# YangHai-1218/RADet

Hardware: AMD Instinct MI355X
Metric: images/sec train-step, r50_ycbv_pbr 640x480 bs=4/GPU (higher is better)
Workload: dtype f32

## Files before the change

include/radet_hip.h:

```cpp
#ifndef RADET_HIP_H
#define RADET_HIP_H
#include <stdint.h>

#ifdef __cplusplus
extern "C" {
#endif


typedef struct RadetConvDesc {
    const float* w;
    const float* bias;
    const float* bn_gamma;
    const float* bn_beta;
    const float* bn_mean;
    const float* bn_var;
    float* wf;
    float* wft;
    float* bias_f;
    const float* dwf_slabs;
    const float* dbias_partials;
    float* dw;
    float* dbias;
    float* dgamma;
    float* dbeta;
// ... 8 lines not shown
    float* w_l1;
    float* bias_amax;
    float* w_l1t;
} RadetConvDesc;

#define RADET_AMAX_WORDS 64
typedef struct RadetScales {
    const void* x_amax;
    const void* w_amax;
    void* y_amax;
    const void* x1_amax;
    const void* w1_amax;
    void* y1_amax;
    void* yq;
    void* yq_amax;
    const void* x_true_amax;
    const void* w_l1;
    const void* bias_amax;
    const void* addend_amax;
} RadetScales;

int radet_gather_table_rows(int M);
int radet_build_gather_table(int* table, int B, int KH, int KW, int so, int sr, int off, int div, const int* seg_desc,
                             int nseg, void* stream);
enum {
    RADET_TILE_ID_MASK = 0xFF,
    RADET_TILE_SYMBOL = 0x100,
    RADET_TILE_BK32 = 0x200,
    RADET_TILE_MATH_BF16 = 0x400,
    RADET_TILE_STORE_BF16 = 0x800,
    RADET_TILE_SPLITK = 0x1000,
    RADET_TILE_SPLITK_MASK = 0xF000,
    RADET_TILE_OUT_F32 = 0x10000,
    RADET_TILE_STAGES3 = 0x20000,
    RADET_TILE_STAGES4 = 0x40000,
    RADET_TILE_ROWPAIRS = 0x80000,
    RADET_TILE_STREAMK = 0x100000,
    RADET_TILE_STREAMK_MASK = 0x700000,
    RADET_TILE_X3 = 0x1000000,
    RADET_TILE_P3 = 0x2000000,
    RADET_TILE_H2 = 0x8000000,
    RADET_TILE_MASKQ = 0x10000000
};
int radet_conv2d_igemm(const float* x, const float* w, const float* bias, const float* addend, const float* mask,
                       float* y, const int* gather_table, int M, int Cin, int Cout, int KH, int KW, int relu,
                       int tile_override, float* splitk_ws, size_t splitk_ws_floats, void* stream);
int radet_conv2d_igemm_s(const float* x, const float* w, const float* bias, const float* addend, const float* mask,
                         float* y, const int* gather_table, int M, int Cin, int Cout, int KH, int KW, int relu,
                         int tile_override, float* splitk_ws, size_t splitk_ws_floats, void* stream, const RadetScales* sc);
int radet_conv2d_igemm_pair_s(const float* x0, const float* w0, const float* bias0, const float* addend0,
                              const float* mask0, float* y0, const float* x1, const float* w1, const float* bias1,
                              const float* addend1, const float* mask1, float* y1, const int* gather_table, int M,
                              int Cin, int Cout, int KH, int KW, int relu, int tile_override, float* splitk_ws,
                              size_t splitk_ws_floats, void* stream, const RadetScales* sc);
int radet_conv2d_igemm_taps_s(const float* x, const float* w, const float* addend, const float* mask, float* y,
                              const int* gather_table, const int* out_rows, const int* tap_ids_host, int ntaps, int kt_w,
                              int M, int Cin, int Cout, int tile_override, float* splitk_ws, size_t splitk_ws_floats,
                              void* stream, const RadetScales* sc);
int radet_conv2d_igemm_classes_s(const float* x, const float* w, const float* addend, const float* mask, float* y,
                                 const int* gather_table, const int* out_rows, const int* tap_ids_host,
                                 const int* cls_ntaps, const int* cls_start, int ncls, int kt_w, int M, int Cin, int Cout,
                                 int tile_override, float* splitk_ws, size_t splitk_ws_floats, void* stream,
                                 const RadetScales* sc);
int radet_conv2d_igemm_pair(const float* x0, const float* w0, const float* bias0, const float* addend0,
                            const float* mask0, float* y0, const float* x1, const float* w1, const float* bias1,
                            const float* addend1, const float* mask1, float* y1, const int* gather_table, int M, int Cin,
                            int Cout, int KH, int KW, int relu, int tile_override, float* splitk_ws,
                            size_t splitk_ws_floats, void* stream);
int radet_conv2d_igemm_taps(const float* x, const float* w, const float* addend, const float* mask, float* y,
                            const int* gather_table, const int* out_rows, const int* tap_ids_host, int ntaps, int kt_w,
                            int M, int Cin, int Cout, int tile_override, float* splitk_ws, size_t splitk_ws_floats,
                            void* stream);
int radet_conv2d_igemm_classes(const float* x, const float* w, const float* addend, const float* mask, float* y,
                               const int* gather_table, const int* out_rows, const int* tap_ids_host, const int* cls_ntaps,
                               const int* cls_start, int ncls, int kt_w, int M, int Cin, int Cout, int tile_override,
                               float* splitk_ws, size_t splitk_ws_floats, void* stream);
int radet_pred3x3_patch(const float* x, int Cin, const int* tiles_dev, int ntiles, const float* w0, const float* bias0,
                        float* y0, int c0, const float* w1, const float* bias1, float* y1, int c1, void* stream);
enum {
    RADET_WGRAD_MATH_BF16 = 0x1,
    RADET_WGRAD_STORE_BF16 = 0x2,
    RADET_WGRAD_TILE = 0x10,
    RADET_WGRAD_TILE_MASK = 0x30,
    RADET_WGRAD_ONE_TAP = 0x40,
    RADET_WGRAD_PX32 = 0x80,
    RADET_WGRAD_X3 = 0x100,
    RADET_WGRAD_P3 = 0x200,
    RADET_WGRAD_KDIV4 = 0x400,
    RADET_WGRAD_KDIV2 = 0x800,
    RADET_WGRAD_H2 = 0x1000,
    RADET_WGRAD_DEEP = 0x2000,
    RADET_WGRAD_WINDOWS = 0x4000
};
int radet_conv2d_wgrad_splits(int M, int Cin, int Cout, int KH, int KW);
int radet_conv2d_wgrad(const float* dy, const float* x, float* slabs, float* dbias_partials, const int* gather_table,
                       int M, int Cin, int Cout, int ld_dy, int KH, int KW, int S, int flags, void* stream);
int radet_conv2d_wgrad_s(const float* dy, const float* x, float* slabs, float* dbias_partials, const int* gather_table,
                         int M, int Cin, int Cout, int ld_dy, int KH, int KW, int S, int flags, void* stream,
                         const RadetScales* sc);
typedef struct RadetWgradJob {
    const float* dy;
    const float* x;
    float* slabs;
    float* dbias_partials;
    const int* gather_table;
    int M, Cin, Cout, ld_dy, KH, KW, S;
// ... 302 lines not shown
```

radet_amd/_lib.py:

```python
import ctypes as C
import os

_HERE = os.path.dirname(os.path.abspath(__file__))
LIB_PATH = os.path.join(_HERE, os.environ.get("RADET_LIB", "libradet_hip.so"))

_p = C.c_void_p
_i = C.c_int
_f = C.c_float
_sz = C.c_size_t


class RadetConvDesc(C.Structure):
    _fields_ = [("w", _p), ("bias", _p), ("bn_gamma", _p), ("bn_beta", _p), ("bn_mean", _p), ("bn_var", _p),
                ("wf", _p), ("wft", _p), ("bias_f", _p), ("dwf_slabs", _p), ("dbias_partials", _p),
                ("dw", _p), ("dbias", _p), ("dgamma", _p), ("dbeta", _p),
                ("cout", _i), ("cin", _i), ("kh", _i), ("kw", _i), ("nsplit", _i), ("eps", _f),
                ("wft_ld", _i), ("wft_off", _i), ("w16", _i), ("w_amax", _p), ("wfq", _p), ("w_l1", _p), ("bias_amax", _p),
                ("w_l1t", _p)]


class RadetScales(C.Structure):
    _fields_ = [("x_amax", _p), ("w_amax", _p), ("y_amax", _p), ("x1_amax", _p), ("w1_amax", _p), ("y1_amax", _p),
                ("yq", _p), ("yq_amax", _p), ("x_true_amax", _p), ("w_l1", _p), ("bias_amax", _p), ("addend_amax", _p)]


class RadetWgradJob(C.Structure):
    _fields_ = [("dy", _p), ("x", _p), ("slabs", _p), ("dbias_partials", _p), ("gather_table", _p),
                ("M", _i), ("Cin", _i), ("Cout", _i), ("ld_dy", _i), ("KH", _i), ("KW", _i), ("S", _i)]


class RadetTapeOp(C.Structure):
    _fields_ = [("kind", C.c_int32), ("fn", C.c_int32), ("stream", _p), ("event", _p), ("args", C.c_uint64 * 32)]


SIGNATURES = {
    "radet_gather_table_rows": (_i, [_i]),
    "radet_build_gather_table": (_i, [_p, _i, _i, _i, _i, _i, _i, _i, _p, _i, _p]),
    "radet_conv2d_igemm": (_i, [_p, _p, _p, _p, _p, _p, _p, _i, _i, _i, _i, _i, _i, _i, _p, _sz, _p]),
    "radet_conv2d_igemm_pair": (_i, [_p] * 13 + [_i, _i, _i, _i, _i, _i, _i, _p, _sz, _p]),
    "radet_conv2d_igemm_taps": (_i, [_p, _p, _p, _p, _p, _p, _p, _p, _i, _i, _i, _i, _i, _i, _p, _sz, _p]),
    "radet_conv2d_igemm_classes": (_i, [_p, _p, _p, _p, _p, _p, _p, _p, _p, _p, _i, _i, _i, _i, _i, _i, _p, _sz, _p]),
    "radet_conv2d_igemm_s": (_i, [_p, _p, _p, _p, _p, _p, _p, _i, _i, _i, _i, _i, _i, _i, _p, _sz, _p, _p]),
    "radet_conv2d_igemm_pair_s": (_i, [_p] * 13 + [_i, _i, _i, _i, _i, _i, _i, _p, _sz, _p, _p]),
    "radet_conv2d_igemm_taps_s": (_i, [_p, _p, _p, _p, _p, _p, _p, _p, _i, _i, _i, _i, _i, _i, _p, _sz, _p, _p]),
    "radet_conv2d_igemm_classes_s": (_i, [_p, _p, _p, _p, _p, _p, _p, _p, _p, _p, _i, _i, _i, _i, _i, _i, _p, _sz, _p, _p]),
    "radet_conv2d_wgrad_s": (_i, [_p, _p, _p, _p, _p, _i, _i, _i, _i, _i, _i, _i, _i, _p, _p]),
    "radet_split_pairs": (_i, [_p, _p, _sz, _i, _i, _p, _p, _p]),
    "radet_merge_pairs": (_i, [_p, _p, _sz, _i, _i, _p, _p]),
    "radet_gn_relu_fwd_q": (_i, [_p, _p, _p, _p, _p, _p, _p, _i, _i, _i, _f, _i, _p, _i, _p, _p, _p, _p]),
    "radet_gn_relu_fwd_pair_q": (_i, [_p] * 20 + [_i, _i, _i, _f, _i, _p, _i, _p]),
    "radet_gn_relu_bwd_q": (_i, [_p, _p, _p, _p, _p, _p, _p, _p, _p, _p, _i, _i, _i, _i, _p, _i, _p, _p, _p, _p]),
    "radet_maxpool3x3s2_a": (_i, [_p, _p, _i, _i, _i, _i, _p, _p]),
    "radet_maxpool3x3s2_q": (_i, [_p, _p, _i, _i, _i, _i, _p, _p, _p, _p, _p]),
    "radet_stem_conv_bn_relu_a": (_i, [_p, _p, _p, _p, _i, _i, _i, _p, _p]),
    "radet_upsample_add_a": (_i, [_p, _p, _i, _i, _i, _i, _i, _i, _p, _p]),
    "radet_upsample_add_bwd_a": (_i, [_p, _p, _i, _i, _i, _i, _i, _i, _p, _p]),
    "radet_relu_bwd_a": (_i, [_p, _p, _p, _p, _sz, _p, _p]),
    "radet_absmax": (_i, [_p, _sz, _p, _p]),
    "radet_amax_slot_words": (_i, []),
    "radet_pred3x3_patch": (_i, [_p, _i, _p, _i, _p, _p, _p, _i, _p, _p, _p, _i, _p]),
    "radet_conv2d_wgrad_splits": (_i, [_i, _i, _i, _i, _i]),
    "radet_conv2d_wgrad": (_i, [_p, _p, _p, _p, _p, _i, _i, _i, _i, _i, _i, _i, _i, _p]),
    "radet_conv2d_wgrad_group": (_i, [_p, _i, _i, _p]),
    "radet_fold_weights": (_i, [_p, _i, _p]),
    "radet_unfold_grads": (_i, [_p, _i, _i, _p]),
    "radet_stem_conv_bn_relu": (_i, [_p, _p, _p, _p, _i, _i, _i, _p]),
    "radet_maxpool3x3s2": (_i, [_p, _p, _i, _i, _i, _i, _p]),
    "radet_maxpool3x3s2_bwd_relu": (_i, [_p, _p, _p, _i, _i, _i, _i, _p]),
    "radet_stem_wgrad_splits": (_i, [_i, _i, _i]),
    "radet_stem_wgrad": (_i, [_p, _p, _p, _p, _i, _i, _i, _i, _p]),
    "radet_gn_workspace_floats": (_i, [_i, _p, _i]),
    "radet_gn_relu_fwd": (_i, [_p, _p, _p, _p, _p, _p, _i, _i, _i, _f, _i, _p, _i, _p]),
    "radet_gn_relu_fwd_pair": (_i, [_p] * 12 + [_i, _i, _i, _f, _i, _p, _i, _p]),
    "radet_gn_relu_fwd_pair_h": (_i, [_p] * 12 + [_i, _i, _i, _f, _i, _p, _i, _p]),
    "radet_gn_relu_bwd": (_i, [_p, _p, _p, _p, _p, _p, _p, _p, _p, _i, _i, _i, _i, _p, _i, _p]),
    "radet_upsample_add": (_i, [_p, _p, _i, _i, _i, _i, _i, _i, _p]),
    "radet_upsample_add_bwd": (_i, [_p, _p, _i, _i, _i, _i, _i, _i, _p]),
    "radet_relu_bwd": (_i, [_p, _p, _p, _p, _sz, _p]),
    "radet_nchw_to_nhwc": (_i, [_p, _p, _i, _i, _i, _i, _p]),
    "radet_nhwc_to_nchw": (_i, [_p, _p, _i, _i, _i, _i, _p]),
    "radet_head_loss_ws_ints": (_i, [_i]),
    "radet_head_loss": (_i, [_p, _p, _p, _p, _p, _p, _p, _p, _p, _p, _i, _i, _i, _f, _f, _f, _f, _p, _p, _p, _i, _p,
                             _i, _p, _i, _p, _p, _p, _i, _p, _p]),
    "radet_scale_relu": (_i, [_p, _p, _p, _p, _i, _i, _p]),
    "radet_decode_ws_bytes": (_sz, [_i, _i, _i]),
    "radet_decode_candidates": (_i, [_p, _p, _p, _p, _p, _i, _i, _i, _f, _i, _p, _p, _p, _p, _p, _p, _p, _p, _p]),
    "radet_nms_ws_bytes": (_sz, [_i, _i]),
    "radet_nms": (_i, [_p, _p, _p, _p, _p, _i, _i, _i, _f, _i, _f, _i, _p, _p, _p, _p, _p, _p, _p, _p]),
    "radet_assign_ws_bytes": (_sz, [_i, _i]),
    "radet_assign_points": (_i, [_p, _p, _p, _i, _i, _p, _i, _p, _p, _i, _i, _i, _i, _f, _p, _p, _p, _p, _p]),
    "radet_assign_points_f": (_i, [_p, _p, _p, _i, _i, _p, _i, _p, _p, _i, _i, _i, _i, _f, _p, _p, _p, _p, _p]),
    "radet_resize_linear_u8": (_i, [_p, _p, _p, _p, _p, _i, _i, _i, _p]),
    "radet_resize_linear_f": (_i, [_p, _p, _p, _p, _i, _i, _i, _p]),
    "radet_warp_affine_u8": (_i, [_p, _sz, _p, _sz, _p, _i, _i, _i, _p]),
    "radet_cutout_u8": (_i, [_p, _sz, _p, _i, _p, _i, _i, _i, _i, _p]),
    "radet_cutout_f32": (_i, [_p, _i, _i, _i, _p, _i, _p, _i, _i, _i, _f, _f, _f, _f, _f, _f, _p]),
# ... 112 lines not shown
```

radet_amd/csrc/conv_common.h:

```cpp
#pragma once
#include "common.h"
#include "../../include/radet_hip.h"
#include <stdlib.h>
#include <type_traits>

#define RADET_SPLIT_COUNTERS 16384
#ifndef RADET_P3_DBG
#define RADET_P3_DBG 0
#endif

struct ConvPtrs {
    const float* x;
    const float* w;
    const float* bias;
    const float* addend;
    const float* mask;
    float* y;
    const unsigned* xs;
    const unsigned* ws;
    unsigned* ys;
    _Float16* yq;
    unsigned* yqs;
    const unsigned* xt;
    const unsigned* wl1;
    const unsigned* bs;
    const unsigned* as;
};

struct ConvArgs {
    ConvPtrs p[2];
    int groups;
    const int* rowtab;
    float* partial;
    int* counters;
    const int* out_rows;
    int tap_ids[16];
    int KTw;
    int M, Mp, Cin, Cout, KH, KW;
    int relu;
    int sk, it_per_split;
    int n_full, sk_tail, it_per_tail;
    int io;
    int sk_wgs, sk_base, sk_rem;
    int cls_nt, cls_b[3];
    int dbg;
    int maskq;
};

__device__ __forceinline__ float ld_act(const float* p, size_t o, int io) {
    return io ? (float)reinterpret_cast<const __bf16*>(p)[o] : p[o];
}
__device__ __forceinline__ void st_out(float* p, size_t o, float v, int io) {
    if (io == 1) reinterpret_cast<__bf16*>(p)[o] = (__bf16)v;
    else p[o] = v;
}


typedef const __attribute__((address_space(1))) void* gptr_t;
typedef __attribute__((address_space(3))) void* lptr_t;

#ifndef RADET_BUFLDS
#define RADET_BUFLDS 1
#endif
__device__ __forceinline__ __amdgpu_buffer_rsrc_t radet_rsrc(const void* base) {
    return __builtin_amdgcn_make_buffer_rsrc(const_cast<void*>(base), 0, 0xFFFFFF00u, 0x00020000);
}
#if RADET_BUFLDS
#define radet_lds_load16(base, ok, elem_off, dst) \
    __builtin_amdgcn_raw_ptr_buffer_load_lds(radet_rsrc(base), (dst), 16, \
        (int)((ok) ? (unsigned)((elem_off) * sizeof(*(base))) : 0xFFFFFFFFu), 0, 0, 0)
#else
#define radet_lds_load16(base, ok, elem_off, dst) \
    __builtin_amdgcn_global_load_lds((gptr_t)((ok) ? (const void*)((base) + (elem_off)) : (const void*)(radet_zero_page + (threadIdx.x & 63) * 4)), \
                                     (dst), 16, 0, 0)
#endif

__device__ __forceinline__ void radet_pipe_barrier() {
    asm volatile("s_waitcnt lgkmcnt(0)" ::: "memory");
    __builtin_amdgcn_s_barrier();
    asm volatile("" ::: "memory");
}

__device__ __forceinline__ int find_seg(const RadetSegs& s, int m) {
    int l = 0;
#pragma unroll
    for (int i = 0; i < RADET_MAX_SEG - 1; ++i)
        if (i < s.nseg - 1 && m >= s.s[i].row_end) l = i + 1;
    return l;
}

struct PixCtx {
    int by, bx;
    int Hi, Wi;
    int base;
};

__device__ __forceinline__ PixCtx decode_pixel(const RadetSegs& segs, int m, int M, int so, int off) {
    PixCtx p;
    p.Hi = 0; p.Wi = 0; p.by = 0; p.bx = 0; p.base = 0;
    if (m < M) {
        const int l = find_seg(segs, m);
        const RadetSeg& sg = segs.s[l];
        const int local = m - sg.row_begin;
        const int hw = sg.Ho * sg.Wo;
        const int n = local / hw;
        const int rem = local - n * hw;
        const int oy = rem / sg.Wo;
        const int ox = rem - oy * sg.Wo;
        p.by = oy * so + off;
        p.bx = ox * so + off;
        p.Hi = sg.Hi;
        p.Wi = sg.Wi;
        p.base = sg.in_row_off + n * sg.Hi * sg.Wi;
    }
    return p;
}

__device__ __forceinline__ int gather_row(const PixCtx& p, int r, int q, int sr, int div) {
    int iy = p.by + r * sr, ix = p.bx + q * sr;
    if (div > 1) {
        if ((iy % div) != 0 || (ix % div) != 0) return -1;
        iy /= div;
        ix /= div;
    }
    if (iy < 0 || iy >= p.Hi || ix < 0 || ix >= p.Wi) return -1;
    return p.base + iy * p.Wi + ix;
}

template <int IO>
__device__ __forceinline__ float ld_act_t(const float* p, size_t o) {
    if constexpr (IO != 0) return (float)reinterpret_cast<const __bf16*>(p)[o];
    else return p[o];
}
template <int IO>
__device__ __forceinline__ void st_out_t(float* p, size_t o, float v) {
    if constexpr (IO == 1) reinterpret_cast<__bf16*>(p)[o] = (__bf16)v;
    else p[o] = v;
}

struct EpiArgs {
    float qs, qs2;
    int M, Cout, relu, io;
    int maskq;
    const int* out_rows;
    float* partial;
    int* counters;
    int sk_base, sk_rem;
};
template <class T>
__device__ __forceinline__ T pin_sgpr(T v) {
    asm volatile("" : "+s"(v));
    return v;
}

template <int BM, int BN, int WM, int WN, int IO>
__device__ __forceinline__ void igemm_epilogue(const EpiArgs& a, const ConvPtrs& P,
                                               f32x16 (&acc)[BM / (WM * 32)][BN / (WN * 32)], int m0, int n0, int wm, int wn,
                                               int li, int lh) {
    constexpr int TM = BM / (WM * 32), TN = BN / (WN * 32);
    const bool has_add = P.addend != nullptr, has_mask = P.mask != nullptr, has_rows = a.out_rows != nullptr;
    const bool interior = !has_rows && m0 + BM <= a.M && n0 + BN <= a.Cout;
    float amax = 0.f;
#pragma unroll
    for (int i = 0; i < TM; ++i) {
        size_t obase[16];
        bool rvalid[16];
        if (has_rows) {
            int orow[16];
#pragma unroll
            for (int r = 0; r < 16; ++r) {
                const int row = m0 + (wm * TM + i) * 32 + (r & 3) + 8 * (r >> 2) + 4 * lh;
                orow[r] = a.out_rows[row < a.M ? row : 0];
                rvalid[r] = row < a.M && orow[r] >= 0;
                if (orow[r] < 0) orow[r] = 0;
            }
#pragma unroll
            for (int r = 0; r < 16; ++r) obase[r] = (size_t)orow[r] * a.Cout;
        } else {
#pragma unroll
            for (int r = 0; r < 16; ++r) {
                const int row = m0 + (wm * TM + i) * 32 + (r & 3) + 8 * (r >> 2) + 4 * lh;
                rvalid[r] = row < a.M;
                obase[r] = (size_t)(rvalid[r] ? row : 0) * a.Cout;
            }
        }
#pragma unroll
        for (int j = 0; j < TN; ++j) {
            const int col = n0 + (wn * TN + j) * 32 + li;
            const bool cvalid = col < a.Cout;
            const int cc = cvalid ? col : 0;
            const float bv = P.bias ? P.bias[cc] : 0.f;
            float av[16], mv[16];
            if (has_add) {
#pragma unroll
                for (int r = 0; r < 16; ++r) av[r] = ld_act_t<IO>(P.addend, obase[r] + cc);
            }
            if (has_mask) {
                if (IO == 0 && a.maskq) {
                    const unsigned short* mq = reinterpret_cast<const unsigned short*>(P.mask) + radet_pair_off(cc);
                    unsigned short mh[16], ml[16];
#pragma unroll
                    for (int r = 0; r < 16; ++r) { mh[r] = mq[2 * obase[r]]; ml[r] = mq[2 * obase[r] + 32]; }
#pragma unroll
                    for (int r = 0; r < 16; ++r) {
                        const unsigned sel = (mh[r] & 0x7FFFu) ? mh[r] : ml[r];
                        mv[r] = ((sel & 0x7FFFu) != 0u && (sel & 0x8000u) == 0u) ? 1.f : 0.f;
                    }
                } else {
#pragma unroll
                    for (int r = 0; r < 16; ++r) mv[r] = ld_act_t<IO>(P.mask, obase[r] + cc);
                }
            }
            float out[16];
#pragma unroll
            for (int r = 0; r < 16; ++r) {
                float v = acc[i][j][r] + bv;
                if (has_add) v += av[r];
                if (a.relu) v = fmaxf(v, 0.f);
                if (has_mask) v = mv[r] > 0.f ? v : 0.f;
                out[r] = v;
            }
            if constexpr (IO == 0) {
                if (P.yq) {
                    const bool odd = li & 1;
                    unsigned* const q = reinterpret_cast<unsigned*>(reinterpret_cast<unsigned short*>(P.yq) +
                                                                    radet_pair_off(cc & ~1) + (odd ? 32 : 0));
#pragma unroll
                    for (int r = 0; r < 16; r += 2) {
                        unsigned h, l;
                        radet_split2(out[r], out[r + 1], a.qs, a.qs2, h, l);
                        const unsigned send = odd ? h : l;
                        const unsigned recv = (unsigned)__builtin_amdgcn_mov_dpp((int)send, 0xB1, 0xF, 0xF, true);
                        const unsigned lo_ch = odd ? recv : h, hi_ch = odd ? l : recv;
                        const unsigned w0 = __builtin_amdgcn_perm(hi_ch, lo_ch, 0x05040100u);
                        const unsigned w1 = __builtin_amdgcn_perm(hi_ch, lo_ch, 0x07060302u);
                        if (interior || (cvalid && rvalid[r])) q[obase[r]] = w0;
                        if (interior || (cvalid && rvalid[r + 1])) q[obase[r + 1]] = w1;
                    }
                }
            }
            const bool has_y = P.y != nullptr;
            if (interior) {
                if (has_y) {
#pragma unroll
// ... 43 lines not shown
#pragma unroll
    for (int i = 0; i < TM; ++i)
#pragma unroll
        for (int j = 0; j < TN; ++j) {
            const float4* src = reinterpret_cast<const float4*>(pz + (((wave * TM + i) * TN + j) * 64 + lane) * 16);
#pragma unroll
            for (int q = 0; q < 4; ++q) {
                const float4 v = src[q];
                acc[i][j][4 * q] += v.x; acc[i][j][4 * q + 1] += v.y; acc[i][j][4 * q + 2] += v.z; acc[i][j][4 * q + 3] += v.w;
            }
        }
}

template <class A>
__device__ __forceinline__ int streamk_start(const A& a, int v) { return v * a.sk_base + (v < a.sk_rem ? v : a.sk_rem); }
template <class A>
__device__ __forceinline__ int streamk_owner(const A& a, int it) {
    const int big = (a.sk_base + 1) * a.sk_rem;
    return it < big ? it / (a.sk_base + 1) : a.sk_rem + (it - big) / a.sk_base;
}

template <int BM, int BN, int WM, int WN>
__device__ __forceinline__ bool streamk_publish(const EpiArgs& a, f32x16 (&acc)[BM / (WM * 32)][BN / (WN * 32)],
                                                int tile, int nseg, int nKs, int v, int slot, volatile int* ws) {
    constexpr int TM = BM / (WM * 32), TN = BN / (WN * 32);
    partial_write<BM, BN, WM, WN>(a.partial + (size_t)(2 * v + slot) * BM * BN, acc);
    asm volatile("s_waitcnt vmcnt(0)" ::: "memory");
    __syncthreads();
    if (threadIdx.x == 0)
        ws[0] = __hip_atomic_fetch_add(&a.counters[tile], nseg, __ATOMIC_RELAXED, __HIP_MEMORY_SCOPE_AGENT);
    __syncthreads();
    const bool last = ws[0] + nseg == nKs;
    __syncthreads();
    if (!last) return false;
    __builtin_amdgcn_fence(__ATOMIC_ACQUIRE, "agent");
    if (threadIdx.x == 0)
        __hip_atomic_store(&a.counters[tile], 0, __ATOMIC_RELAXED, __HIP_MEMORY_SCOPE_AGENT);
    __syncthreads();
#pragma unroll
    for (int i = 0; i < TM; ++i)
#pragma unroll
        for (int j = 0; j < TN; ++j)
#pragma unroll
            for (int r = 0; r < 16; ++r) acc[i][j][r] = 0.f;
    const int t0 = tile * nKs;
    const int v0 = streamk_owner(a, t0), v1 = streamk_owner(a, t0 + nKs - 1);
    for (int u = v0; u <= v1; ++u) {
        const int sl = streamk_start(a, u) >= t0 ? 0 : 1;
        partial_add<BM, BN, WM, WN>(a.partial + (size_t)(2 * u + sl) * BM * BN, acc);
    }
    return true;
}

template <int BM, int BN, int WM, int WN>
__device__ __forceinline__ void igemm_store(const EpiArgs& e, const ConvPtrs& P,
                                            f32x16 (&acc)[BM / (WM * 32)][BN / (WN * 32)], int m0, int n0, int nsplit,
                                            int ctile, int z, int wm, int wn, int li, int lh, volatile int* ws) {
    constexpr int TM = BM / (WM * 32), TN = BN / (WN * 32);
    if (nsplit > 1) {
        float* base = e.partial + (size_t)ctile * nsplit * BM * BN;
        partial_write<BM, BN, WM, WN>(base + (size_t)z * BM * BN, acc);
        asm volatile("s_waitcnt vmcnt(0)" ::: "memory");
        __syncthreads();
        if (threadIdx.x == 0)
            ws[0] = __hip_atomic_fetch_add(&e.counters[ctile], 1, __ATOMIC_RELAXED, __HIP_MEMORY_SCOPE_AGENT);
        __syncthreads();
        if (ws[0] != nsplit - 1) return;
        __builtin_amdgcn_fence(__ATOMIC_ACQUIRE, "agent");
        if (threadIdx.x == 0)
            __hip_atomic_store(&e.counters[ctile], 0, __ATOMIC_RELAXED, __HIP_MEMORY_SCOPE_AGENT);
        __syncthreads();
#pragma unroll
        for (int i = 0; i < TM; ++i)
#pragma unroll
            for (int j = 0; j < TN; ++j)
#pragma unroll
                for (int r = 0; r < 16; ++r) acc[i][j][r] = 0.f;
        for (int zz = 0; zz < nsplit; ++zz) partial_add<BM, BN, WM, WN>(base + (size_t)zz * BM * BN, acc);
    }
    if (e.io == 0) igemm_epilogue<BM, BN, WM, WN, 0>(e, P, acc, m0, n0, wm, wn, li, lh);
    else if (e.io == 1) igemm_epilogue<BM, BN, WM, WN, 1>(e, P, acc, m0, n0, wm, wn, li, lh);
    else igemm_epilogue<BM, BN, WM, WN, 2>(e, P, acc, m0, n0, wm, wn, li, lh);
}

typedef float f32x4 __attribute__((ext_vector_type(4)));
template <int OFF>
__device__ __forceinline__ void lds_read128(f32x4& d, unsigned addr) {
    asm volatile("ds_read_b128 %0, %1 offset:%2" : "=v"(d) : "v"(addr), "n"(OFF) : "memory");
}
typedef short s16x4 __attribute__((ext_vector_type(4)));
typedef unsigned u32x2 __attribute__((ext_vector_type(2)));
typedef float f32x2 __attribute__((ext_vector_type(2)));
typedef __bf16 bf16x2 __attribute__((ext_vector_type(2)));
typedef __bf16 bf16x8 __attribute__((ext_vector_type(8)));
__device__ __forceinline__ unsigned cvt_pk_bf16(float lo, float hi) {
    const f32x2 v = {lo, hi};
    return __builtin_bit_cast(unsigned, __builtin_convertvector(v, bf16x2));
}
__device__ __forceinline__ s16x4 cvt_bf16x4(float a, float b, float c, float d) {
    const u32x2 r = {cvt_pk_bf16(a, b), cvt_pk_bf16(c, d)};
    return __builtin_bit_cast(s16x4, r);
}

template <int OFF>
__device__ __forceinline__ void lds_read32(float& d, unsigned addr) {
    asm volatile("ds_read_b32 %0, %1 offset:%2" : "=v"(d) : "v"(addr), "n"(OFF) : "memory");
}
template <int OFF>
__device__ __forceinline__ void lds_read_u16(unsigned& d, unsigned addr) {
    asm volatile("ds_read_u16 %0, %1 offset:%2" : "=v"(d) : "v"(addr), "n"(OFF) : "memory");
}
template <int OFF>
__device__ __forceinline__ void lds_read_i16(int& d, unsigned addr) {
    asm volatile("ds_read_i16 %0, %1 offset:%2" : "=v"(d) : "v"(addr), "n"(OFF) : "memory");
}
template <int N>
__device__ __forceinline__ void vm_wait() {
    asm volatile("s_waitcnt vmcnt(%0)" ::"n"(N) : "memory");
}
template <int I, int N, class F>
__device__ __forceinline__ void static_for(F&& f) {
    if constexpr (I < N) {
        f(std::integral_constant<int, I>{});
        static_for<I + 1, N>(f);
    }
}
typedef short s16x4v_ __attribute__((ext_vector_type(4)));
template <int OFF>
__device__ __forceinline__ void lds_read_tr16(s16x4v_& d, unsigned addr) {
    asm volatile("ds_read_b64_tr_b16 %0, %1 offset:%2" : "=v"(d) : "v"(addr), "n"(OFF) : "memory");
}
template <int N>
__device__ __forceinline__ void lds_wait() {
// ... 4 lines not shown
__device__ __forceinline__ void split3_bf16(const float (&a)[8], bf16x8& hi, bf16x8& mid, bf16x8& lo) {
    typedef float f32x2_ __attribute__((ext_vector_type(2)));
    u32x4_ h, m, l;
#pragma unroll
    for (int q = 0; q < 4; ++q) {
        const f32x2_ a2 = {a[2 * q], a[2 * q + 1]};
        const unsigned ua0 = __float_as_uint(a2.x), ua1 = __float_as_uint(a2.y);
        const f32x2_ h2 = {__uint_as_float(ua0 & 0xFFFF0000u), __uint_as_float(ua1 & 0xFFFF0000u)};
        const f32x2_ r2 = a2 - h2;
        const unsigned ur0 = __float_as_uint(r2.x), ur1 = __float_as_uint(r2.y);
        const f32x2_ m2 = {__uint_as_float(ur0 & 0xFFFF0000u), __uint_as_float(ur1 & 0xFFFF0000u)};
        const f32x2_ l2 = r2 - m2;
        h[q] = __builtin_amdgcn_perm(ua1, ua0, 0x07060302u);
        m[q] = __builtin_amdgcn_perm(ur1, ur0, 0x07060302u);
        l[q] = __builtin_amdgcn_perm(__float_as_uint(l2.y), __float_as_uint(l2.x), 0x07060302u);
    }
    hi = __builtin_bit_cast(bf16x8, h);
    mid = __builtin_bit_cast(bf16x8, m);
    lo = __builtin_bit_cast(bf16x8, l);
}
__device__ __forceinline__ void split3_bf16(const f32x4& f0, const f32x4& f1, bf16x8& hi, bf16x8& mid, bf16x8& lo) {
    const float a[8] = {f0.x, f0.y, f0.z, f0.w, f1.x, f1.y, f1.z, f1.w};
    split3_bf16(a, hi, mid, lo);
}
__device__ __forceinline__ void mfma_x3(f32x16& acc, const bf16x8& ah, const bf16x8& am, const bf16x8& al,
                                        const bf16x8& bh, const bf16x8& bm, const bf16x8& bl) {
    acc = __builtin_amdgcn_mfma_f32_32x32x16_bf16(ah, bh, acc, 0, 0, 0);
    acc = __builtin_amdgcn_mfma_f32_32x32x16_bf16(am, bh, acc, 0, 0, 0);
    acc = __builtin_amdgcn_mfma_f32_32x32x16_bf16(ah, bm, acc, 0, 0, 0);
    acc = __builtin_amdgcn_mfma_f32_32x32x16_bf16(am, bm, acc, 0, 0, 0);
    acc = __builtin_amdgcn_mfma_f32_32x32x16_bf16(al, bh, acc, 0, 0, 0);
    acc = __builtin_amdgcn_mfma_f32_32x32x16_bf16(ah, bl, acc, 0, 0, 0);
}


typedef _Float16 f16x8 __attribute__((ext_vector_type(8)));
struct H2Scale {
    float s, s2, inv;
};
__device__ __forceinline__ H2Scale h2_scale_bits(unsigned amax_bits) {
    const int e = radet_h2_exp(amax_bits);
    H2Scale r;
    r.s = radet_pow2(e); r.s2 = radet_pow2(e + 11); r.inv = radet_pow2(-e);
    return r;
}
__device__ __forceinline__ H2Scale h2_scale(const unsigned* slot) {
    return h2_scale_bits(radet_amax_read(slot));
}
__device__ __forceinline__ unsigned h2_scale_load(const unsigned* slot) { return radet_amax_load(slot); }
__device__ __forceinline__ H2Scale h2_scale_finish(unsigned raw) {
    asm volatile("" : "+v"(raw));
    return h2_scale_bits(radet_amax_reduce(raw));
}
__device__ __forceinline__ void split2_f16(const float (&a)[8], const H2Scale& sc, f16x8& hi, f16x8& lo) {
    u32x4_ h, l;
#pragma unroll
    for (int q = 0; q < 4; ++q) {
        unsigned hq, lq;
        radet_split2(a[2 * q], a[2 * q + 1], sc.s, sc.s2, hq, lq);
        h[q] = hq; l[q] = lq;
    }
    hi = __builtin_bit_cast(f16x8, h);
    lo = __builtin_bit_cast(f16x8, l);
}
__device__ __forceinline__ void split2_f16(const f32x4& f0, const f32x4& f1, const H2Scale& sc, f16x8& hi, f16x8& lo) {
    const float a[8] = {f0.x, f0.y, f0.z, f0.w, f1.x, f1.y, f1.z, f1.w};
    split2_f16(a, sc, hi, lo);
}
__device__ __forceinline__ void mfma_h2(f32x16& acc0, f32x16& acc1, const f16x8& ah, const f16x8& al, const f16x8& bh,
                                        const f16x8& bl) {
    acc0 = __builtin_amdgcn_mfma_f32_32x32x16_f16(ah, bh, acc0, 0, 0, 0);
    acc1 = __builtin_amdgcn_mfma_f32_32x32x16_f16(ah, bl, acc1, 0, 0, 0);
    acc1 = __builtin_amdgcn_mfma_f32_32x32x16_f16(al, bh, acc1, 0, 0, 0);
}
struct PairScaleRaw { unsigned xt, wl1, bs, as; };
__device__ __forceinline__ PairScaleRaw igemm_pair_scale_load(const ConvPtrs& P) {
    PairScaleRaw r;
    r.xt = radet_amax_load(P.xt); r.wl1 = radet_amax_load(P.wl1);
    r.bs = P.bs ? radet_amax_load(P.bs) : 0u;
    r.as = P.as ? radet_amax_load(P.as) : 0u;
    return r;
}
__device__ __forceinline__ void igemm_pair_scale(const ConvPtrs& P, PairScaleRaw r, bool store, float& qs, float& qs2) {
    asm volatile("" : "+v"(r.xt), "+v"(r.wl1), "+v"(r.bs), "+v"(r.as));
    float bound = __uint_as_float(radet_amax_reduce(r.xt)) * __uint_as_float(radet_amax_reduce(r.wl1));
    bound += __uint_as_float(radet_amax_reduce(r.bs));
    bound += __uint_as_float(radet_amax_reduce(r.as));
    bound *= 1.0001f;
    const unsigned bits = __float_as_uint(bound);
    if (store && threadIdx.x == 0) radet_amax_store(P.yqs, bits);
    const int e = radet_h2_exp(bits);
    qs = radet_pow2(e);
    qs2 = radet_pow2(e + 11);
}

__device__ __forceinline__ void h2_combine(f32x16& acc0, const f32x16& acc1, float inv_a, float inv_b) {
#pragma unroll
    for (int r = 0; r < 16; ++r) acc0[r] = (fmaf(acc1[r], 1.0f / 2048.0f, acc0[r]) * inv_a) * inv_b;
}

struct TileWord {
    int id;
    int splitk;
    int stages;
    int streamk;
    bool symbol, bk32, math_bf16, store_bf16, out_f32, rowpairs, x3, p3, h2, maskq;
// ... 31 lines not shown
```

radet_amd/csrc/conv_igemm.hip:

```cpp
#include "common.h"
#include "../../include/radet_hip.h"
#include <stdlib.h>
#include <type_traits>

#include "conv_common.h"

#include "conv_igemm_kernel.h"
#include "conv_wgrad_kernel.h"

struct PredTile { int base_row, H, W, yx; };
struct PredArgs {
    const float* x;
    const float* w[2];
    const float* bias[2];
    float* y[2];
    int c[2];
    const PredTile* tiles;
    int Cin;
};

__global__ __launch_bounds__(512) void pred3x3_patch_kernel(const PredArgs a) {
    constexpr int TH = 8, TW = 16, PW = TW + 2, PP = (TH + 2) * PW;
    constexpr int PROWS = 192, WROWS = 9 * 32;
    constexpr int A_BYTES = PROWS * 64, BUF_BYTES = (PROWS + WROWS) * 64;
// ... 888 lines not shown
                      const RadetScales* sc) {
    const TileWord tw = decode_tile(tile_override);
    const bool h16 = tw.store_bf16;
    const bool p3 = tw.p3 && !h16;
    if (h16 || p3) {
        if (Cin % 32 != 0) return RADET_ERR_ARG;
        Cin /= 2;
    }
    if (Cin % 16 != 0 || Cin <= 0 || Cout <= 0 || M <= 0 || KH * KW > 16 ||
        (gather_table == nullptr && (KH * KW != 1 || out_rows != nullptr || cls != nullptr)))
        return RADET_ERR_ARG;
    ConvArgs a;
    a.io = h16 ? (tw.out_f32 ? 2 : 1) : 0;
    a.out_rows = out_rows;
    for (int t = 0; t < 16; ++t) a.tap_ids[t] = tap_ids ? (t < KH * KW ? tap_ids[t] : 0) : t;
    a.cls_nt = 0; a.cls_b[0] = a.cls_b[1] = a.cls_b[2] = 0x7fffffff;
    if (cls != nullptr) {
        for (int t = 0; t < 16; ++t) a.tap_ids[t] = tap_ids[t];
        for (int c = 0; c < cls[0]; ++c) {
            a.cls_nt |= cls[1 + c] << (4 * c);
            if (c > 0) a.cls_b[c - 1] = cls[5 + c];
        }
    }
    a.KTw = kt_w > 0 ? kt_w : KH * KW;
    { static const int dbg = getenv("RADET_DBG_IGEMM") ? atoi(getenv("RADET_DBG_IGEMM")) : 0; a.dbg = dbg; }
    a.maskq = tw.maskq && mask != nullptr;
    if (a.maskq && (h16 || Cout % 32 != 0 || second != nullptr)) return RADET_ERR_ARG;
    if (y == nullptr && (sc == nullptr || sc->yq == nullptr)) return RADET_ERR_ARG;
    a.p[0].x = x; a.p[0].w = w; a.p[0].bias = bias; a.p[0].addend = addend; a.p[0].mask = mask; a.p[0].y = y;
    a.p[0].xs = sc ? (const unsigned*)sc->x_amax : nullptr;
    a.p[0].ws = sc ? (const unsigned*)sc->w_amax : nullptr;
    a.p[0].ys = sc ? (unsigned*)sc->y_amax : nullptr;
    a.p[0].yq = sc ? (_Float16*)sc->yq : nullptr;
    a.p[0].yqs = sc ? (unsigned*)sc->yq_amax : nullptr;
    a.p[0].xt = sc ? (const unsigned*)sc->x_true_amax : nullptr;
    a.p[0].wl1 = sc ? (const unsigned*)sc->w_l1 : nullptr;
    a.p[0].bs = (sc && bias) ? (const unsigned*)sc->bias_amax : nullptr;
    a.p[0].as = (sc && addend) ? (const unsigned*)sc->addend_amax : nullptr;
    if (a.p[0].yq != nullptr) {
        if (h16 || Cout % 32 != 0 || a.p[0].yqs == nullptr || a.p[0].xt == nullptr || a.p[0].wl1 == nullptr ||
            (bias && a.p[0].bs == nullptr) || (addend && a.p[0].as == nullptr) || second != nullptr)
            return RADET_ERR_ARG;
    }
    a.p[1] = a.p[0];
    a.groups = 1;
    if (second != nullptr) {
        a.p[1] = *second;
        a.p[1].yq = nullptr; a.p[1].yqs = nullptr; a.p[1].xt = a.p[1].wl1 = a.p[1].bs = a.p[1].as = nullptr;
        a.p[1].xs = sc ? (const unsigned*)sc->x1_amax : nullptr;
        a.p[1].ws = sc ? (const unsigned*)sc->w1_amax : nullptr;
        a.p[1].ys = sc ? (unsigned*)sc->y1_amax : nullptr;
        a.groups = 2;
    }
    a.rowtab = gather_table;
    a.Cin = Cin; a.Cout = Cout; a.KH = KH; a.KW = KW;
    a.relu = relu;
    a.M = M;
    a.Mp = radet_gather_table_rows(M);
    hipStream_t st = (hipStream_t)stream;
    const int sym = tw.symbol ? TAG_SYMBOL : 0;
    int tag = sym | (h16 ? TAG_H16 : (tw.math_bf16 ? TAG_BF16_MATH : 0));
    int bk = tw.bk32 ? 32 : 16;
    if (Cin % 32 != 0) bk = 16;
    const bool x3 = tw.x3 && !h16 && !p3 && !tw.math_bf16 && Cin % 32 == 0;
    if (x3) { bk = 32; tag |= TAG_X3; }
    if (p3) { tag = TAG_P3 | sym; bk = 16; }
    const bool h2 = tw.h2 && (x3 || p3);
    if (h2) {
        for (int g = 0; g < a.groups; ++g)
            if (a.p[g].xs == nullptr || a.p[g].ws == nullptr) return RADET_ERR_ARG;
        tag |= TAG_H2;
    }
    int choice = tw.id;
    if (p3 && h2 && tw.rowpairs && (choice == 5 || choice == 6)) {
        Cin *= 2;
        a.Cin = Cin;
        if (Cin % 32 != 0) return RADET_ERR_ARG;
        tag |= TAG_PAIRS; bk = 32;
    }
    if (choice == 7 && p3 && h2) {
        Cin *= 2;
        a.Cin = Cin;
        if (Cin % 64 != 0 || tw.streamk || a.groups != 1) return RADET_ERR_ARG;
        tag = TAG_X3 | TAG_KDIV | TAG_H2 | TAG_PAIRS; bk = 64;
    } else
    if (choice == 7 || choice == 8) {
        const int kbk = choice == 7 ? 64 : 32;
        if (!x3 || Cin % kbk != 0 || tw.streamk) return RADET_ERR_ARG;
        tag |= TAG_KDIV; bk = kbk;
    } else
    if (choice > 4 && !p3) return RADET_ERR_ARG;
    if (choice == 6 && cls != nullptr) return RADET_ERR_ARG;
    if (choice <= 0) {
        if (Cout <= 32) choice = 4;
        else {
            const double s1 = tile_score(a.M, Cout, 128, 128, 1.00);
            const double s2 = tile_score(a.M, Cout, 128, 64, 0.96);
            const double s3 = tile_score(a.M, Cout, 64, 64, 0.90);
            choice = 1;
            double best = s1;
            if (s2 > best) { best = s2; choice = 2; }
            if (s3 > best) { best = s3; choice = 3; }
        }
    }
    const int nK = KH * KW * (Cin / bk);
    int sk = 1;
// ... 237 lines not shown
```

radet_amd/csrc/conv_igemm_kernel.h:

```cpp
#pragma once
#include "conv_common.h"
static __device__ __attribute__((aligned(16))) float radet_zero_page[512];

constexpr int TAG_SYMBOL = 1;
constexpr int TAG_BF16_MATH = 2;
constexpr int TAG_H16 = 4;
constexpr int TAG_X3 = 8;
constexpr int TAG_P3 = 16;
constexpr int TAG_KDIV = 32;
constexpr int TAG_H2 = 64;
constexpr int TAG_PAIRS = 128;
template <int BM, int BN, int WM, int WN, int TAG, int BK, int NSTG = 2, bool SK = false>
__global__ __launch_bounds__(WM * WN * 64) void conv_igemmg_kernel(const ConvArgs a) {
    constexpr int NW = WM * WN;
    constexpr int F4 = BK / 4;
    constexpr int RPI = 64 / F4;
    constexpr int RPB = 64 / BK;
    constexpr int TM = BM / (WM * 32), TN = BN / (WN * 32);
    constexpr int A_INSTR = BM / RPI, B_INSTR = BN / RPI;
    constexpr int A_PW = (A_INSTR + NW - 1) / NW, B_PW = (B_INSTR + NW - 1) / NW;
    constexpr int NS = ((TAG & TAG_PAIRS) && (TAG & TAG_P3)) ? 2 : BK / 8;
    constexpr bool BF16 = (TAG & TAG_BF16_MATH) != 0;
    constexpr bool H16 = (TAG & TAG_H16) != 0;
    constexpr bool X3 = (TAG & TAG_X3) != 0;
    constexpr bool P3 = (TAG & TAG_P3) != 0;
    constexpr bool H2 = (TAG & TAG_H2) != 0;
    static_assert(!H2 || X3 || P3, "fp16 hi / lo arithmetic: in-register split (TAG_X3) or plane pairs (TAG_P3)");
    constexpr bool RI = P3 && (TAG & TAG_PAIRS) != 0;
    static_assert(!RI || (H2 && BK == 32), "row-interleaved pairs: fp16 hi / lo planes, 128-byte tile rows");
    constexpr int NPLC = P3 ? (H2 ? 2 : 3) : 1;
    constexpr int NPL = RI ? 1 : NPLC;
    constexpr bool KW = (TAG & TAG_KDIV) != 0;
    constexpr bool PQ = (TAG & TAG_PAIRS) != 0 && (TAG & TAG_KDIV) != 0;
    static_assert(!PQ || (KW && H2 && BK == 64), "pair operands in the K-divided tile: 64-channel stages");
    constexpr int KD = KW ? BK / 16 : 1;
    constexpr int WNK = NW / KD;
    constexpr int TMA = KW ? BM / 32 : TM, TNA = KW ? BN / (32 * WNK) : TN;
    static_assert(!KW || (X3 && !SK && NW == 4 && KD * WNK == NW && TM == 1 && TN == 1 && TMA * TNA == KD && NSTG >= 2 && NSTG <= 4),
                  "K-divided tile: one 32 x 32 block per wave after the reduction");
    static_assert(NW == 4 || NW == 8, "4 or 8 waves");
    static_assert(!P3 || BK == 16 || RI, "plane rows are laid out in 32-channel groups: one group per K stage");
    __shared__ __attribute__((aligned(16))) float As[NSTG][NPL * BM * BK];
    __shared__ __attribute__((aligned(16))) float Bs[NSTG][NPL * BN * BK];

    radet_kernarg_warm<sizeof(ConvArgs)>();
    const int tid = threadIdx.x;
    const int lane = tid & 63, wave = __builtin_amdgcn_readfirstlane(tid >> 6);
    const int wm = wave / WN, wn = wave % WN;
    const int li = lane & 31, lh = lane >> 5;
    const int xld = NPL * a.Cin;

    const int tilesN = (a.Cout + BN - 1) / BN;
    const int tilesG = ((a.M + BM - 1) / BM) * tilesN;
    const int KT = a.KH * a.KW;
    const int cpt = a.Cin / BK;
    constexpr bool streamk = SK;
    const int vwg = streamk ? ((int)blockIdx.x & 7) * (a.sk_wgs >> 3) + ((int)blockIdx.x >> 3) : 0;
    int cur = streamk ? streamk_start(a, vwg) : 0;
    const int end_it = streamk ? cur + a.sk_base + (vwg < a.sk_rem ? 1 : 0) : 1;
    const int first_tile = cur / (KT * cpt);
  do {
    const bool tail = !streamk && (int)blockIdx.x >= a.n_full;
    const int tail_slot = tail ? (int)blockIdx.x - a.n_full : 0;
    int id = streamk ? cur / (KT * cpt)
                     : (tail ? a.n_full + tail_slot / a.sk_tail : (a.cls_nt ? (int)blockIdx.x : xcd_remap(blockIdx.x, a.n_full)));
    const int sk_tile = id;
    const int grp = id >= tilesG ? 1 : 0;
    id -= grp * tilesG;
    ConvPtrs P = a.p[grp];
    P.y = pin_sgpr(P.y); P.bias = pin_sgpr(P.bias); P.addend = pin_sgpr(P.addend); P.mask = pin_sgpr(P.mask);
    EpiArgs epi;
    epi.M = pin_sgpr(a.M); epi.Cout = pin_sgpr(a.Cout); epi.relu = pin_sgpr(a.relu); epi.io = pin_sgpr(a.io);
    epi.out_rows = pin_sgpr(a.out_rows); epi.maskq = pin_sgpr(a.maskq);
    epi.partial = pin_sgpr(a.partial); epi.counters = pin_sgpr(a.counters);
    epi.sk_base = pin_sgpr(a.sk_base); epi.sk_rem = pin_sgpr(a.sk_rem);
    epi.qs = 1.f; epi.qs2 = 2048.f;
    unsigned raw_xs = 0u, raw_ws = 0u;
    if constexpr ((TAG & TAG_H2) != 0) { raw_xs = h2_scale_load(P.xs); raw_ws = h2_scale_load(P.ws); }
    PairScaleRaw raw_q = {0u, 0u, 0u, 0u};
    const bool pair_copy = P.yq != nullptr;
    if (pair_copy) raw_q = igemm_pair_scale_load(P);
    const bool pair_store = id == 0 && (int)blockIdx.y == 0 && !SK;
    const int nsplit = pin_sgpr(tail ? a.sk_tail : a.sk);
    const int ctile = pin_sgpr(tail ? tail_slot / a.sk_tail : sk_tile);
    const int zsplit = pin_sgpr(tail ? tail_slot % a.sk_tail : (int)blockIdx.y);
    const int m0 = (id / tilesN) * BM;
    const int n0 = (id % tilesN) * BN;
    int KTt = KT, tbase = 0;
    if (!streamk && a.cls_nt) {
        const int cls = (m0 >= a.cls_b[0] ? 1 : 0) + (m0 >= a.cls_b[1] ? 1 : 0) + (m0 >= a.cls_b[2] ? 1 : 0);
        KTt = (a.cls_nt >> (4 * cls)) & 15;
        tbase = 4 * cls;
    }

    const int per = tail ? a.it_per_tail : a.it_per_split;
    const int it0 = streamk ? cur - sk_tile * KT * cpt : (tail ? tail_slot % a.sk_tail : (int)blockIdx.y) * per;
    int nK = KTt * cpt - it0;
    if (streamk) {
        if (nK > end_it - cur) nK = end_it - cur;
    } else if (nK > per) {
        nK = per;
    }

    const int lrow = lane / F4;
    const bool cmaj = P3 && (!RADET_P3_DBG || !(a.dbg & 8));
    int ld_tap = cmaj ? it0 % KTt : it0 / cpt, ld_c0 = cmaj ? (it0 / KTt) * BK : (it0 - ld_tap * cpt) * BK;
    int arow[A_PW], akq[A_PW];
    const float* wp[B_PW];
#pragma unroll
    for (int k = 0; k < A_PW; ++k) {
        const int r = (wave + NW * k) * RPI + lrow;
        akq[k] = 4 * ((lane % F4) ^ ((r / RPB) % F4));
    }
    {
        int araw[A_PW];
        if (a.rowtab) {
            const int* const tab = a.rowtab + (size_t)(nK > 0 ? ld_tap : 0) * a.Mp;
#pragma unroll
            for (int k = 0; k < A_PW; ++k) {
                const int m = m0 + (wave + NW * k) * RPI + lrow;
                araw[k] = tab[m < a.Mp ? m : a.Mp - 1];
            }
        } else {
#pragma unroll
            for (int k = 0; k < A_PW; ++k) {
                const int m = m0 + (wave + NW * k) * RPI + lrow;
                araw[k] = m < a.M ? m : -1;
            }
        }
#pragma unroll
        for (int k = 0; k < A_PW; ++k) arow[k] = (nK > 0 && (A_INSTR % NW == 0 || wave + NW * k < A_INSTR)) ? araw[k] : -1;
    }
#pragma unroll
    for (int k = 0; k < B_PW; ++k) {
        const int r = (wave + NW * k) * RPI + lrow;
        const int n = n0 + r;
        wp[k] = (wave + NW * k < B_INSTR && n < a.Cout)
                    ? P.w + (size_t)n * a.KTw * xld + 4 * ((lane % F4) ^ ((r / RPB) % F4)) : nullptr;
    }
    constexpr bool A_FULL = A_INSTR % NW == 0, B_FULL = B_INSTR % NW == 0;
    int wtap = nK > 0 ? a.tap_ids[tbase + ld_tap] : 0;
    constexpr int NPIECE = NPL * (A_PW + B_PW);
    const float* abase[A_PW];
    const float* wbase[B_PW];
    unsigned amask[A_PW], wmask[B_PW];
    constexpr bool BMASK = P3 || KW;
    constexpr bool BL = RADET_BUFLDS != 0;
    __amdgpu_buffer_rsrc_t rs_x, rs_w;
    unsigned aoffb[A_PW], woffb[B_PW];
    if constexpr (BL) {
        rs_x = radet_rsrc(P.x);
        rs_w = radet_rsrc(P.w);
    }
    int pc0 = 0, pwt = 0;
    auto set_abase = [&]() {
        pc0 = ld_c0; pwt = wtap;
        if constexpr (BL) {
#pragma unroll
            for (int k = 0; k < A_PW; ++k) {
                amask[k] = arow[k] >= 0 ? 0xFFFFFFFFu : 0u;
                aoffb[k] = ((unsigned)(arow[k] & (int)amask[k]) * (unsigned)xld + (unsigned)akq[k]) * 4u;
            }
        } else
        if constexpr (BMASK) {
#pragma unroll
            for (int k = 0; k < A_PW; ++k) {
                amask[k] = arow[k] >= 0 ? 0xFFFFFFFFu : 0u;
                const unsigned long long real = (unsigned long long)(P.x + (size_t)(arow[k] & (int)amask[k]) * xld + akq[k]);
                const unsigned long long zero = (unsigned long long)(radet_zero_page + lane * 4);
                const unsigned long long m = (unsigned long long)(long long)(int)amask[k];
                abase[k] = (const float*)((real & m) | (zero & ~m));
            }
        }
    };
    if constexpr (BMASK || BL) {
#pragma unroll
        for (int k = 0; k < B_PW; ++k) {
            wmask[k] = wp[k] ? 0xFFFFFFFFu : 0u;
            wbase[k] = wp[k] ? wp[k] : radet_zero_page + lane * 4;
            if constexpr (BL) woffb[k] = wp[k] ? (unsigned)((const char*)wp[k] - (const char*)P.w) : 0u;
        }
    }
    set_abase();
    auto issue_piece = [&](int buf, auto qc) {
        constexpr int q = decltype(qc)::value;
        if constexpr (q < NPL * A_PW) {
            constexpr int k = q / NPL, p = q % NPL;
            const int ins = wave + NW * k;
            if (A_FULL || ins < A_INSTR) {
                if constexpr (BL) {
                    const unsigned voff = (aoffb[k] + 4u * (unsigned)(NPL * pc0 + p * BK)) | ~amask[k];
                    __builtin_amdgcn_raw_ptr_buffer_load_lds(rs_x, (lptr_t)(&As[buf][p * BM * BK + ins * 256]), 16, (int)voff, 0, 0, 0);
                } else {
                const float* src;
                if constexpr (BMASK) src = abase[k] + ((unsigned)(NPL * pc0 + p * BK) & amask[k]);
                else src = arow[k] >= 0 ? P.x + (size_t)arow[k] * xld + NPL * pc0 + akq[k] + p * BK : radet_zero_page + lane * 4;
                __builtin_amdgcn_global_load_lds((gptr_t)src, (lptr_t)(&As[buf][p * BM * BK + ins * 256]), 16, 0, 0);
                }
            }
        } else {
            constexpr int k = (q - NPL * A_PW) / NPL, p = (q - NPL * A_PW) % NPL;
            const int ins = wave + NW * k;
            if (B_FULL || ins < B_INSTR) {
                if constexpr (BL) {
                    const unsigned voff = (woffb[k] + 4u * (unsigned)(pwt * xld + NPL * pc0 + p * BK)) | ~wmask[k];
                    __builtin_amdgcn_raw_ptr_buffer_load_lds(rs_w, (lptr_t)(&Bs[buf][p * BN * BK + ins * 256]), 16, (int)voff, 0, 0, 0);
                } else {
                const float* src;
                if constexpr (BMASK) src = wbase[k] + ((unsigned)(pwt * xld + NPL * pc0 + p * BK) & wmask[k]);
                else src = wp[k] ? wp[k] + pwt * xld + NPL * pc0 + p * BK : radet_zero_page + lane * 4;
                __builtin_amdgcn_global_load_lds((gptr_t)src, (lptr_t)(&Bs[buf][p * BN * BK + ins * 256]), 16, 0, 0);
                }
            }
        }
    };
    auto advance_stage = [&]() {
        if (cmaj) {
            if (++ld_tap == KTt) { ld_tap = 0; ld_c0 += BK; }
            wtap = a.tap_ids[tbase + ld_tap];
            if (a.rowtab) {
#pragma unroll
                for (int k = 0; k < A_PW; ++k)
                    if (A_FULL || wave + NW * k < A_INSTR)
                        arow[k] = a.rowtab[(size_t)ld_tap * a.Mp + m0 + (wave + NW * k) * RPI + lrow];
            }
            return;
        }
        ld_c0 += BK;
        if (ld_c0 == a.Cin) {
            ld_c0 = 0;
            ++ld_tap;
            if (ld_tap < KTt) {
                wtap = a.tap_ids[tbase + ld_tap];
#pragma unroll
                for (int k = 0; k < A_PW; ++k)
                    if (A_FULL || wave + NW * k < A_INSTR)
                        arow[k] = a.rowtab[(size_t)ld_tap * a.Mp + m0 + (wave + NW * k) * RPI + lrow];
            }
        }
    };
    auto issue_stage = [&](int buf) {
        set_abase();
        static_for<0, NPIECE>([&](auto qc) { issue_piece(buf, qc); });
        advance_stage();
    };

    f32x16 acc[TMA][TNA];
    f32x16 acc1[H2 ? TMA : 1][H2 ? TNA : 1];
#pragma unroll
    for (int i = 0; i < TMA; ++i)
#pragma unroll
        for (int j = 0; j < TNA; ++j)
#pragma unroll
            for (int r = 0; r < 16; ++r) acc[i][j][r] = 0.f;
    if constexpr (H2) {
#pragma unroll
        for (int i = 0; i < TMA; ++i)
#pragma unroll
            for (int j = 0; j < TNA; ++j)
#pragma unroll
                for (int r = 0; r < 16; ++r) acc1[i][j][r] = 0.f;
    }
    H2Scale sx = {1.f, 1.f, 1.f}, sw = {1.f, 1.f, 1.f};

    constexpr int LOADS = (A_FULL && B_FULL) ? NPL * (A_PW + B_PW) : 0;
    if (nK > 0) issue_stage(0);
    if (NSTG >= 3 && nK >= NSTG - 1) {
        issue_stage(1);
        if constexpr (NSTG >= 4) issue_stage(2);
        asm volatile("s_waitcnt vmcnt(%0)" ::"n"(LOADS * (NSTG - 2)) : "memory");
    } else {
        if (NSTG >= 3 && nK > 1) issue_stage(1);
        asm volatile("s_waitcnt vmcnt(0)" ::: "memory");
    }
    __syncthreads();
    if constexpr (H2) { sx = h2_scale_finish(raw_xs); sw = h2_scale_finish(raw_ws); }
    if (pair_copy) {
        float qs, qs2;
        igemm_pair_scale(P, raw_q, pair_store, qs, qs2);
        epi.qs = pin_sgpr(qs); epi.qs2 = pin_sgpr(qs2);
    }

    const int rswz = (li / RPB) % F4;
    unsigned aaddr[NS], baddr[NS];
    unsigned aaddr_lo[RI ? NS : 1], baddr_lo[RI ? NS : 1];
    {
        const unsigned a_lds = (unsigned)(size_t)(lptr_t)(&As[0][0]) + (unsigned)((wm * TM * 32 + li) * BK * 4);
        const unsigned b_lds = (unsigned)(size_t)(lptr_t)(&Bs[0][0]) + (unsigned)((wn * TN * 32 + li) * BK * 4);
#pragma unroll
        for (int s = 0; s < NS; ++s) {
            aaddr[s] = a_lds + 16u * (unsigned)((2 * s + lh) ^ rswz);
            baddr[s] = b_lds + 16u * (unsigned)((2 * s + lh) ^ rswz);
            if constexpr (RI) {
                aaddr_lo[s] = a_lds + 16u * (unsigned)((4 + 2 * s + lh) ^ rswz);
                baddr_lo[s] = b_lds + 16u * (unsigned)((4 + 2 * s + lh) ^ rswz);
            }
        }
    }
    auto stage = [&](auto bufc, int it) {
        constexpr int BUF = decltype(bufc)::value;
        constexpr int AO = BUF * BM * BK * 4, BO = BUF * BN * BK * 4, RO = 32 * BK * 4;
        if (it + NSTG - 1 < nK) issue_stage((BUF + NSTG - 1) % NSTG);
        f32x4 af[X3 ? NS : 2][TM], bf[X3 ? NS : 2][TN];
        auto read_s = [&](int s, int pp) {
            lds_read128<AO>(af[pp][0], aaddr[s]);
            if constexpr (TM > 1) lds_read128<AO + RO>(af[pp][TM - 1], aaddr[s]);
            lds_read128<BO>(bf[pp][0], baddr[s]);
            if constexpr (TN > 1) lds_read128<BO + RO>(bf[pp][TN - 1], baddr[s]);
        };
        if constexpr (X3) {
#pragma unroll
            for (int s = 0; s < NS; ++s) read_s(s, s);
            static_for<0, NS / 2>([&](auto gc) {
                constexpr int g = decltype(gc)::value;
                lds_wait<(NS - 2 * g - 2) * (TM + TN)>();
#pragma unroll
                for (int i = 0; i < TM; ++i) asm volatile("" : "+v"(af[2 * g][i]), "+v"(af[2 * g + 1][i]));
#pragma unroll
                for (int j = 0; j < TN; ++j) asm volatile("" : "+v"(bf[2 * g][j]), "+v"(bf[2 * g + 1][j]));
                if constexpr (H2) {
                    f16x8 ah[TM], al[TM], bh[TN], bl[TN];
#pragma unroll
                    for (int i = 0; i < TM; ++i) split2_f16(af[2 * g][i], af[2 * g + 1][i], sx, ah[i], al[i]);
#pragma unroll
                    for (int j = 0; j < TN; ++j) split2_f16(bf[2 * g][j], bf[2 * g + 1][j], sw, bh[j], bl[j]);
#pragma unroll
                    for (int i = 0; i < TM; ++i)
#pragma unroll
                        for (int j = 0; j < TN; ++j) mfma_h2(acc[i][j], acc1[i][j], ah[i], al[i], bh[j], bl[j]);
                } else {
                bf16x8 ah[TM], am[TM], al[TM], bh[TN], bm[TN], bl[TN];
#pragma unroll
                for (int i = 0; i < TM; ++i) split3_bf16(af[2 * g][i], af[2 * g + 1][i], ah[i], am[i], al[i]);
#pragma unroll
                for (int j = 0; j < TN; ++j) split3_bf16(bf[2 * g][j], bf[2 * g + 1][j], bh[j], bm[j], bl[j]);
#pragma unroll
                for (int i = 0; i < TM; ++i)
#pragma unroll
                    for (int j = 0; j < TN; ++j) mfma_x3(acc[i][j], ah[i], am[i], al[i], bh[j], bm[j], bl[j]);
                }
                __builtin_amdgcn_sched_barrier(0);
            });
        } else {
        read_s(0, 0);
#pragma unroll
        for (int s = 0; s < NS; ++s) {
            const int pp = s & 1;
            if (s + 1 < NS) {
                read_s(s + 1, pp ^ 1);
                lds_wait<TM + TN>();
            } else {
                lds_wait<0>();
            }
#pragma unroll
            for (int i = 0; i < TM; ++i) asm volatile("" : "+v"(af[pp][i]));
#pragma unroll
            for (int j = 0; j < TN; ++j) asm volatile("" : "+v"(bf[pp][j]));
            if constexpr (H16) {
#pragma unroll
                for (int i = 0; i < TM; ++i)
#pragma unroll
                    for (int j = 0; j < TN; ++j)
                        acc[i][j] = __builtin_amdgcn_mfma_f32_32x32x16_bf16(__builtin_bit_cast(bf16x8, af[pp][i]),
                                                                            __builtin_bit_cast(bf16x8, bf[pp][j]), acc[i][j], 0, 0, 0);
            } else if constexpr (BF16) {
                s16x4 ab[TM], bb[TN];
#pragma unroll
                for (int i = 0; i < TM; ++i) ab[i] = cvt_bf16x4(af[pp][i].x, af[pp][i].y, af[pp][i].z, af[pp][i].w);
#pragma unroll
                for (int j = 0; j < TN; ++j) bb[j] = cvt_bf16x4(bf[pp][j].x, bf[pp][j].y, bf[pp][j].z, bf[pp][j].w);
#pragma unroll
                for (int i = 0; i < TM; ++i)
#pragma unroll
                    for (int j = 0; j < TN; ++j)
                        acc[i][j] = __builtin_amdgcn_mfma_f32_32x32x8bf16_1k(ab[i], bb[j], acc[i][j], 0, 0, 0);
            } else {
#pragma unroll
                for (int i = 0; i < TM; ++i)
// ... 6 lines not shown
                    }
            }
            __builtin_amdgcn_sched_barrier(0);
        }
        }
        if (NSTG >= 3 && it + NSTG - 1 < nK) asm volatile("s_waitcnt vmcnt(%0)" ::"n"(LOADS * (NSTG - 2)) : "memory");
        else asm volatile("s_waitcnt vmcnt(0)" ::: "memory");
        radet_pipe_barrier();
    };
    if constexpr (KW) {
        const int kg = wave % KD, nh = wave / KD;
        const unsigned ka = (unsigned)(size_t)(lptr_t)(&As[0][0]) + (unsigned)(li * BK * 4);
        const unsigned kb = (unsigned)(size_t)(lptr_t)(&Bs[0][0]) + (unsigned)((nh * TNA * 32 + li) * BK * 4);
        unsigned kaa[2], kba[2];
#pragma unroll
        for (int h = 0; h < 2; ++h) {
            const int slot = PQ ? (8 * (kg >> 1) + 4 * h + 2 * (kg & 1) + lh) : (4 * kg + 2 * h + lh);
            kaa[h] = ka + 16u * (unsigned)(slot ^ rswz);
            kba[h] = kb + 16u * (unsigned)(slot ^ rswz);
        }
        f32x4 fa[2][2][TMA], fb[2][2][TNA];
        constexpr int NRD = 2 * (TMA + TNA);
        auto read_one = [&](int buf, auto ppc, auto rc) {
            constexpr int PP = decltype(ppc)::value, r = decltype(rc)::value;
            constexpr int RO = 32 * BK * 4;
            constexpr int h = r / (TMA + TNA), e = r % (TMA + TNA);
            if constexpr (e < TMA) lds_read128<e * RO>(fa[PP][h][e], kaa[h] + (unsigned)(buf * (BM * BK * 4)));
            else lds_read128<(e - TMA) * RO>(fb[PP][h][e - TMA], kba[h] + (unsigned)(buf * (BN * BK * 4)));
        };
        auto pin = [&](auto ppc) {
            constexpr int PP = decltype(ppc)::value;
            (void)fa; (void)fb;
#pragma unroll
            for (int h = 0; h < 2; ++h) {
#pragma unroll
                for (int i = 0; i < TMA; ++i) asm volatile("" : "+v"(fa[PP][h][i]));
#pragma unroll
                for (int j = 0; j < TNA; ++j) asm volatile("" : "+v"(fb[PP][h][j]));
            }
        };
        auto stage_kw = [&](int buf, auto ppc, int it) {
            constexpr int PP = decltype(ppc)::value;
            if (it + NSTG - 1 < nK) issue_stage(buf + NSTG - 1 >= NSTG ? buf - 1 : buf + NSTG - 1);
            lds_wait<0>();
            pin(ppc);
            if constexpr (H2) {
                f16x8 ah[TMA], al[TMA], bh[TNA], bl[TNA];
                if constexpr (PQ) {
#pragma unroll
                    for (int i = 0; i < TMA; ++i) { ah[i] = __builtin_bit_cast(f16x8, fa[PP][0][i]); al[i] = __builtin_bit_cast(f16x8, fa[PP][1][i]); }
#pragma unroll
                    for (int j = 0; j < TNA; ++j) { bh[j] = __builtin_bit_cast(f16x8, fb[PP][0][j]); bl[j] = __builtin_bit_cast(f16x8, fb[PP][1][j]); }
                } else {
#pragma unroll
                for (int i = 0; i < TMA; ++i) split2_f16(fa[PP][0][i], fa[PP][1][i], sx, ah[i], al[i]);
#pragma unroll
                for (int j = 0; j < TNA; ++j) split2_f16(fb[PP][0][j], fb[PP][1][j], sw, bh[j], bl[j]);
                }
#pragma unroll
                for (int i = 0; i < TMA; ++i)
#pragma unroll
                    for (int j = 0; j < TNA; ++j) mfma_h2(acc[i][j], acc1[i][j], ah[i], al[i], bh[j], bl[j]);
            } else {
            bf16x8 ah[TMA], am[TMA], al[TMA], bh[TNA], bm[TNA], bl[TNA];
#pragma unroll
            for (int i = 0; i < TMA; ++i) split3_bf16(fa[PP][0][i], fa[PP][1][i], ah[i], am[i], al[i]);
#pragma unroll
            for (int j = 0; j < TNA; ++j) split3_bf16(fb[PP][0][j], fb[PP][1][j], bh[j], bm[j], bl[j]);
#pragma unroll
            for (int i = 0; i < TMA; ++i)
#pragma unroll
                for (int j = 0; j < TNA; ++j) mfma_x3(acc[i][j], ah[i], am[i], al[i], bh[j], bm[j], bl[j]);
            }
            __builtin_amdgcn_sched_barrier(0);
            if (NSTG >= 3 && it + NSTG - 1 < nK) asm volatile("s_waitcnt vmcnt(%0)" ::"n"(LOADS * (NSTG - 2)) : "memory");
            else asm volatile("s_waitcnt vmcnt(0)" ::: "memory");
            radet_pipe_barrier();
        };
        static_assert(NSTG == 2 || LOADS > 0, "deep K-divided pipelines count on every wave owning the same loads per stage");
        int buf = 0;
        auto next_buf = [&]() { buf = buf + 1 == NSTG ? 0 : buf + 1; };
        if (nK > 0) static_for<0, NRD>([&](auto rc) { read_one(0, std::integral_constant<int, 0>{}, rc); });
        for (int it = 0; it < nK; it += 2) {
            stage_kw(buf, std::integral_constant<int, 0>{}, it);
            next_buf();
            if (it + 1 < nK) {
                static_for<0, NRD>([&](auto rc) { read_one(buf, std::integral_constant<int, 1>{}, rc); });
                stage_kw(buf, std::integral_constant<int, 1>{}, it + 1);
                next_buf();
                if (it + 2 < nK) static_for<0, NRD>([&](auto rc) { read_one(buf, std::integral_constant<int, 0>{}, rc); });
            }
        }
    } else if constexpr (P3) {
        f32x4 fa[2][NPLC][TM], fb[2][NPLC][TN];
        constexpr int NRD = NPLC * (TM + TN);
        constexpr int NT = H2 ? 3 : 6;
        auto read_one = [&](auto bufc, auto sc, auto ppc, auto rc) {
            constexpr int BUF = decltype(bufc)::value, s = decltype(sc)::value, pp = decltype(ppc)::value, r = decltype(rc)::value;
            constexpr int AO = BUF * NPL * BM * BK * 4, BO = BUF * NPL * BN * BK * 4, RO = 32 * BK * 4;
            constexpr int pl = r / (TM + TN), e = (H2 && pl == 1) ? (r % (TM + TN) + TM) % (TM + TN) : r % (TM + TN);
            if constexpr (RI) {
                if constexpr (e < TM) lds_read128<e * RO>(fa[pp][pl][e], (pl ? aaddr_lo[s] : aaddr[s]) + (unsigned)AO);
                else lds_read128<(e - TM) * RO>(fb[pp][pl][e - TM], (pl ? baddr_lo[s] : baddr[s]) + (unsigned)BO);
            } else
            if constexpr (e < TM) lds_read128<pl * BM * BK * 4 + e * RO>(fa[pp][pl][e], aaddr[s] + (unsigned)AO);
            else lds_read128<pl * BN * BK * 4 + (e - TM) * RO>(fb[pp][pl][e - TM], baddr[s] + (unsigned)BO);
        };
        auto slice = [&](auto ppc, auto rbufc, auto rsc, bool do_read, auto ldc, int ld_buf, bool do_load) {
            constexpr int PP = decltype(ppc)::value;
            constexpr bool LD = decltype(ldc)::value;
// ... 45 lines not shown
                    if (do_read)
                        static_for<t * NRD / (NT - 1), (t + 1) * NRD / (NT - 1)>([&](auto rc) { read_one(rbufc, rsc, std::integral_constant<int, PP ^ 1>{}, rc); });
                }
                __builtin_amdgcn_sched_barrier(0);
            });
        };
        auto stage_p3 = [&](auto bufc, int it) {
            constexpr int BUF = decltype(bufc)::value;
            static_for<0, NS>([&](auto sc) {
                constexpr int s = decltype(sc)::value;
                constexpr int PP = s & 1;
                if constexpr (H2 && s + 1 < NS) lds_wait<NRD / 2>(); else lds_wait<0>();
                if constexpr (s + 1 < NS) {
                    slice(std::integral_constant<int, PP>{}, bufc, std::integral_constant<int, s + 1>{},
                          !RADET_P3_DBG || !(a.dbg & 4), std::false_type{}, 0, false);
                } else {
                    if (NSTG >= 3 && it + NSTG - 1 < nK) asm volatile("s_waitcnt vmcnt(%0)" ::"n"(LOADS * (NSTG - 2)) : "memory");
                    else asm volatile("s_waitcnt vmcnt(0)" ::: "memory");
                    radet_pipe_barrier();
                    slice(std::integral_constant<int, PP>{}, std::integral_constant<int, (BUF + 1) % NSTG>{},
                          std::integral_constant<int, 0>{}, it + 1 < nK && (!RADET_P3_DBG || !(a.dbg & 4)), std::true_type{}, BUF,
                          it + NSTG < nK && (!RADET_P3_DBG || !(a.dbg & 1)));
                }
            });
        };
        static_assert(NS % 2 == 0, "fragment double buffer: compile-time slice parity");
        if (nK > 0) {
            if (NSTG - 1 < nK) issue_stage(NSTG - 1);
            static_for<0, NRD>([&](auto rc) {
                read_one(std::integral_constant<int, 0>{}, std::integral_constant<int, 0>{}, std::integral_constant<int, 0>{}, rc);
            });
        }
        for (int it = 0; it < nK; it += NSTG) {
            stage_p3(std::integral_constant<int, 0>{}, it);
            if (it + 1 < nK) stage_p3(std::integral_constant<int, 1>{}, it + 1);
            if constexpr (NSTG >= 3)
                if (it + 2 < nK) stage_p3(std::integral_constant<int, 2>{}, it + 2);
            if constexpr (NSTG >= 4)
                if (it + 3 < nK) stage_p3(std::integral_constant<int, 3>{}, it + 3);
        }
    } else
    for (int it = 0; it < nK; it += NSTG) {
        stage(std::integral_constant<int, 0>{}, it);
        if (it + 1 < nK) stage(std::integral_constant<int, 1>{}, it + 1);
        if constexpr (NSTG >= 3)
            if (it + 2 < nK) stage(std::integral_constant<int, 2>{}, it + 2);
        if constexpr (NSTG >= 4)
            if (it + 3 < nK) stage(std::integral_constant<int, 3>{}, it + 3);
    }
    if constexpr (H2) {
#pragma unroll
        for (int i = 0; i < TMA; ++i)
#pragma unroll
            for (int j = 0; j < TNA; ++j) h2_combine(acc[i][j], acc1[i][j], sx.inv, sw.inv);
    }
    if constexpr (SK) {
        cur += nK;
        bool fin = nK == KT * cpt;
        if (!fin)
            fin = streamk_publish<BM, BN, WM, WN>(epi, acc, sk_tile, nK, KT * cpt, vwg, sk_tile == first_tile ? 0 : 1,
                                                  reinterpret_cast<volatile int*>(&As[0][0]));
        if (fin) igemm_store<BM, BN, WM, WN>(epi, P, acc, m0, n0, 1, 0, 0, wm, wn, li, lh, nullptr);
    } else if constexpr (KW) {
        constexpr int SLOTS_A = NSTG * BM * BK / 1024, SLOTS_B = NSTG * BN * BK / 1024;
        static_assert(NW * (KD - 1) <= SLOTS_A + SLOTS_B, "partial blocks fit the stage buffers");
        const int kg = wave % KD, nh = wave / KD;
        float* const pa = &As[0][0];
        float* const pb = &Bs[0][0];
        auto slot_ptr = [&](int sender_wave, int blk) {
            const int sk_ = sender_wave % KD;
            const int slot = sender_wave * (KD - 1) + blk - (blk > sk_ ? 1 : 0);
            return reinterpret_cast<f32x4*>(slot < SLOTS_A ? pa + slot * 1024 : pb + (slot - SLOTS_A) * 1024) + lane;
        };
        f32x16 out[1][1];
        static_for<0, KD>([&](auto bc) {
            constexpr int b = decltype(bc)::value;
            const f32x16& v = acc[b / TNA][b % TNA];
            if (kg == b) {
                out[0][0] = v;
            } else {
                f32x4* d = slot_ptr(wave, b);
#pragma unroll
                for (int q = 0; q < 4; ++q) d[q * 64] = f32x4{v[4 * q], v[4 * q + 1], v[4 * q + 2], v[4 * q + 3]};
            }
        });
        __syncthreads();
#pragma unroll
        for (int sg = 0; sg < KD; ++sg) {
            if (sg != kg) {
                const f32x4* d = slot_ptr(nh * KD + sg, kg);
#pragma unroll
                for (int q = 0; q < 4; ++q) {
                    const f32x4 t = d[q * 64];
                    out[0][0][4 * q] += t.x; out[0][0][4 * q + 1] += t.y; out[0][0][4 * q + 2] += t.z; out[0][0][4 * q + 3] += t.w;
                }
            }
        }
        __syncthreads();
        igemm_store<BM, BN, WM, WN>(epi, P, out, m0, n0, nsplit, ctile, zsplit, kg / TNA, nh * TNA + kg % TNA, li, lh,
                                    reinterpret_cast<volatile int*>(&As[0][0]));
        cur = end_it;
    } else {
        igemm_store<BM, BN, WM, WN>(epi, P, acc, m0, n0, nsplit, ctile, zsplit, wm, wn, li, lh,
                                    reinterpret_cast<volatile int*>(&As[0][0]));
        cur = end_it;
    }
  } while (SK && cur < end_it);
}


template <int BM, int BN>
static int igemm_plan(ConvArgs& a, int tag, int bk, size_t ws_floats, int skw, bool no_tail_split) {
    const int sk_in = a.sk;
    const int T = a.groups * ((a.M + BM - 1) / BM) * ((a.Cout + BN - 1) / BN);
    a.sk_wgs = a.sk_base = a.sk_rem = 0;
    if (skw > 0 && a.partial != nullptr && tag == 0 && BM * BN <= 128 * 64) {
        const long I = (long)T * a.KH * a.KW * (a.Cin / bk);
        const int G = 256 * skw;
        if (I >= G && T <= RADET_SPLIT_COUNTERS && (size_t)G * 2 * BM * BN <= ws_floats && T % G != 0) {
            a.sk = 1;
            a.it_per_split = a.KH * a.KW * (a.Cin / bk);
            a.sk_wgs = G;
            a.sk_base = (int)(I / G);
            a.sk_rem = (int)(I % G);
        }
    }
    while (a.sk > 1 && ((size_t)T * a.sk * BM * BN > ws_floats || T > RADET_SPLIT_COUNTERS)) --a.sk;
    if (a.sk != sk_in) {
        const int nKs0 = a.KH * a.KW * (a.Cin / bk);
        a.it_per_split = (nKs0 + a.sk - 1) / a.sk;
    }
    a.n_full = T; a.sk_tail = 1; a.it_per_tail = a.it_per_split;
    const int nKs = a.KH * a.KW * (a.Cin / bk);
    const int rem = T % 256;
    if (a.sk_wgs == 0 && a.cls_nt == 0 && a.sk == 1 && a.partial != nullptr && T > 256 && rem > 0 && rem <= 160 && nKs * bk >= 512 &&
        !no_tail_split) {
        int skt = 256 / rem;
        if (skt > 8) skt = 8;
        if (skt > nKs / 8) skt = nKs / 8;
        while (skt > 1 && ((size_t)rem * skt * BM * BN > ws_floats || rem > RADET_SPLIT_COUNTERS)) --skt;
        if (skt >= 2) {
            a.n_full = T - rem;
            a.sk_tail = skt;
            a.it_per_tail = (nKs + skt - 1) / skt;
        }
    }
    return a.sk_wgs > 0 ? a.sk_wgs : a.n_full + (T - a.n_full) * a.sk_tail;
}
```

radet_amd/csrc/tape_thunks.c:

```c
#include <stdint.h>
#include <stddef.h>
#include <string.h>
#include "radet_hip.h"

static float f32(uint64_t w) { uint32_t u = (uint32_t)w; float f; memcpy(&f, &u, 4); return f; }

static int t_radet_absmax(const uint64_t* a) { return radet_absmax((void*)(uintptr_t)a[0], (size_t)a[1], (void*)(uintptr_t)a[2], (void*)(uintptr_t)a[3]); }
static int t_radet_adamw_step(const uint64_t* a) { return radet_adamw_step((void*)(uintptr_t)a[0], (void*)(uintptr_t)a[1], (void*)(uintptr_t)a[2], (void*)(uintptr_t)a[3], (size_t)a[4], f32(a[5]), f32(a[6]), f32(a[7]), f32(a[8]), f32(a[9]), (int)(int64_t)a[10], f32(a[11]), f32(a[12]), (void*)(uintptr_t)a[13], (int)(int64_t)a[14], (void*)(uintptr_t)a[15], (void*)(uintptr_t)a[16]); }
static int t_radet_adamw_step_runs(const uint64_t* a) { return radet_adamw_step_runs((void*)(uintptr_t)a[0], (void*)(uintptr_t)a[1], (void*)(uintptr_t)a[2], (void*)(uintptr_t)a[3], (size_t)a[4], f32(a[5]), f32(a[6]), f32(a[7]), f32(a[8]), f32(a[9]), (int)(int64_t)a[10], f32(a[11]), f32(a[12]), (void*)(uintptr_t)a[13], (int)(int64_t)a[14], (void*)(uintptr_t)a[15], (void*)(uintptr_t)a[16], (int)(int64_t)a[17], (void*)(uintptr_t)a[18]); }
static int t_radet_amax_slot_words(const uint64_t* a) { (void)a; return radet_amax_slot_words(); }
static int t_radet_assign_points(const uint64_t* a) { return radet_assign_points((void*)(uintptr_t)a[0], (void*)(uintptr_t)a[1], (void*)(uintptr_t)a[2], (int)(int64_t)a[3], (int)(int64_t)a[4], (void*)(uintptr_t)a[5], (int)(int64_t)a[6], (void*)(uintptr_t)a[7], (void*)(uintptr_t)a[8], (int)(int64_t)a[9], (int)(int64_t)a[10], (int)(int64_t)a[11], (int)(int64_t)a[12], f32(a[13]), (void*)(uintptr_t)a[14], (void*)(uintptr_t)a[15], (void*)(uintptr_t)a[16], (void*)(uintptr_t)a[17], (void*)(uintptr_t)a[18]); }
static int t_radet_assign_points_f(const uint64_t* a) { return radet_assign_points_f((void*)(uintptr_t)a[0], (void*)(uintptr_t)a[1], (void*)(uintptr_t)a[2], (int)(int64_t)a[3], (int)(int64_t)a[4], (void*)(uintptr_t)a[5], (int)(int64_t)a[6], (void*)(uintptr_t)a[7], (void*)(uintptr_t)a[8], (int)(int64_t)a[9], (int)(int64_t)a[10], (int)(int64_t)a[11], (int)(int64_t)a[12], f32(a[13]), (void*)(uintptr_t)a[14], (void*)(uintptr_t)a[15], (void*)(uintptr_t)a[16], (void*)(uintptr_t)a[17], (void*)(uintptr_t)a[18]); }
static int t_radet_augment_box(const uint64_t* a) { return radet_augment_box((void*)(uintptr_t)a[0], (void*)(uintptr_t)a[1], (void*)(uintptr_t)a[2], (size_t)a[3], (int)(int64_t)a[4], (int)(int64_t)a[5], (int)(int64_t)a[6], (void*)(uintptr_t)a[7]); }
static int t_radet_augment_finish(const uint64_t* a) { return radet_augment_finish((void*)(uintptr_t)a[0], (void*)(uintptr_t)a[1], (void*)(uintptr_t)a[2], (void*)(uintptr_t)a[3], (int)(int64_t)a[4], (int)(int64_t)a[5], (int)(int64_t)a[6], f32(a[7]), f32(a[8]), f32(a[9]), f32(a[10]), f32(a[11]), f32(a[12]), (void*)(uintptr_t)a[13]); }
static int t_radet_augment_hsv_noise(const uint64_t* a) { return radet_augment_hsv_noise((void*)(uintptr_t)a[0], (void*)(uintptr_t)a[1], (void*)(uintptr_t)a[2], (int)(int64_t)a[3], (int)(int64_t)a[4], (void*)(uintptr_t)a[5]); }
static int t_radet_augment_merge_hblur(const uint64_t* a) { return radet_augment_merge_hblur((void*)(uintptr_t)a[0], (void*)(uintptr_t)a[1], (void*)(uintptr_t)a[2], (void*)(uintptr_t)a[3], (int)(int64_t)a[4], (int)(int64_t)a[5], (int)(int64_t)a[6], (void*)(uintptr_t)a[7]); }
static int t_radet_augment_sharp(const uint64_t* a) { return radet_augment_sharp((void*)(uintptr_t)a[0], (void*)(uintptr_t)a[1], (void*)(uintptr_t)a[2], (void*)(uintptr_t)a[3], (int)(int64_t)a[4], (int)(int64_t)a[5], (void*)(uintptr_t)a[6]); }
static int t_radet_augment_vblur(const uint64_t* a) { return radet_augment_vblur((void*)(uintptr_t)a[0], (void*)(uintptr_t)a[1], (void*)(uintptr_t)a[2], (int)(int64_t)a[3], (int)(int64_t)a[4], (int)(int64_t)a[5], (void*)(uintptr_t)a[6]); }
static int t_radet_bbox_overlaps(const uint64_t* a) { return radet_bbox_overlaps((void*)(uintptr_t)a[0], (void*)(uintptr_t)a[1], (void*)(uintptr_t)a[2], (int)(int64_t)a[3], (int)(int64_t)a[4], (int)(int64_t)a[5], (int)(int64_t)a[6], (int)(int64_t)a[7], f32(a[8]), (void*)(uintptr_t)a[9]); }
static int t_radet_bce_logits_loss(const uint64_t* a) { return radet_bce_logits_loss((void*)(uintptr_t)a[0], (void*)(uintptr_t)a[1], (void*)(uintptr_t)a[2], (int)(int64_t)a[3], (size_t)a[4], (int)(int64_t)a[5], (void*)(uintptr_t)a[6], f32(a[7]), (void*)(uintptr_t)a[8], (void*)(uintptr_t)a[9]); }
static int t_radet_bce_logits_loss_bwd(const uint64_t* a) { return radet_bce_logits_loss_bwd((void*)(uintptr_t)a[0], (void*)(uintptr_t)a[1], (void*)(uintptr_t)a[2], (int)(int64_t)a[3], (size_t)a[4], (int)(int64_t)a[5], (void*)(uintptr_t)a[6], (void*)(uintptr_t)a[7], (void*)(uintptr_t)a[8], f32(a[9]), (void*)(uintptr_t)a[10], (void*)(uintptr_t)a[11]); }
static int t_radet_box_loss(const uint64_t* a) { return radet_box_loss((int)(int64_t)a[0], (void*)(uintptr_t)a[1], (void*)(uintptr_t)a[2], (void*)(uintptr_t)a[3], (size_t)a[4], f32(a[5]), f32(a[6]), (void*)(uintptr_t)a[7], f32(a[8]), (void*)(uintptr_t)a[9], (void*)(uintptr_t)a[10]); }
static int t_radet_box_loss_bwd(const uint64_t* a) { return radet_box_loss_bwd((int)(int64_t)a[0], (void*)(uintptr_t)a[1], (void*)(uintptr_t)a[2], (void*)(uintptr_t)a[3], (size_t)a[4], f32(a[5]), f32(a[6]), (void*)(uintptr_t)a[7], (void*)(uintptr_t)a[8], (void*)(uintptr_t)a[9], f32(a[10]), (void*)(uintptr_t)a[11], (void*)(uintptr_t)a[12]); }
static int t_radet_build_gather_table(const uint64_t* a) { return radet_build_gather_table((void*)(uintptr_t)a[0], (int)(int64_t)a[1], (int)(int64_t)a[2], (int)(int64_t)a[3], (int)(int64_t)a[4], (int)(int64_t)a[5], (int)(int64_t)a[6], (int)(int64_t)a[7], (void*)(uintptr_t)a[8], (int)(int64_t)a[9], (void*)(uintptr_t)a[10]); }
static int t_radet_coco_accumulate(const uint64_t* a) { return radet_coco_accumulate((void*)(uintptr_t)a[0], (void*)(uintptr_t)a[1], (void*)(uintptr_t)a[2], (void*)(uintptr_t)a[3], (void*)(uintptr_t)a[4], (void*)(uintptr_t)a[5], (void*)(uintptr_t)a[6], (void*)(uintptr_t)a[7], (int)(int64_t)a[8], (int)(int64_t)a[9], (int)(int64_t)a[10], (int)(int64_t)a[11], (int)(int64_t)a[12], (void*)(uintptr_t)a[13], (void*)(uintptr_t)a[14], (void*)(uintptr_t)a[15], (void*)(uintptr_t)a[16]); }
static int t_radet_coco_match(const uint64_t* a) { return radet_coco_match((void*)(uintptr_t)a[0], (void*)(uintptr_t)a[1], (void*)(uintptr_t)a[2], (void*)(uintptr_t)a[3], (void*)(uintptr_t)a[4], (void*)(uintptr_t)a[5], (int)(int64_t)a[6], (int)(int64_t)a[7], (void*)(uintptr_t)a[8], (int)(int64_t)a[9], (void*)(uintptr_t)a[10], (int)(int64_t)a[11], (void*)(uintptr_t)a[12], (void*)(uintptr_t)a[13], (void*)(uintptr_t)a[14], (void*)(uintptr_t)a[15], (void*)(uintptr_t)a[16]); }
static int t_radet_conv2d_igemm(const uint64_t* a) { return radet_conv2d_igemm((void*)(uintptr_t)a[0], (void*)(uintptr_t)a[1], (void*)(uintptr_t)a[2], (void*)(uintptr_t)a[3], (void*)(uintptr_t)a[4], (void*)(uintptr_t)a[5], (void*)(uintptr_t)a[6], (int)(int64_t)a[7], (int)(int64_t)a[8], (int)(int64_t)a[9], (int)(int64_t)a[10], (int)(int64_t)a[11], (int)(int64_t)a[12], (int)(int64_t)a[13], (void*)(uintptr_t)a[14], (size_t)a[15], (void*)(uintptr_t)a[16]); }
static int t_radet_conv2d_igemm_classes(const uint64_t* a) { return radet_conv2d_igemm_classes((void*)(uintptr_t)a[0], (void*)(uintptr_t)a[1], (void*)(uintptr_t)a[2], (void*)(uintptr_t)a[3], (void*)(uintptr_t)a[4], (void*)(uintptr_t)a[5], (void*)(uintptr_t)a[6], (void*)(uintptr_t)a[7], (void*)(uintptr_t)a[8], (void*)(uintptr_t)a[9], (int)(int64_t)a[10], (int)(int64_t)a[11], (int)(int64_t)a[12], (int)(int64_t)a[13], (int)(int64_t)a[14], (int)(int64_t)a[15], (void*)(uintptr_t)a[16], (size_t)a[17], (void*)(uintptr_t)a[18]); }
static int t_radet_conv2d_igemm_classes_s(const uint64_t* a) { return radet_conv2d_igemm_classes_s((void*)(uintptr_t)a[0], (void*)(uintptr_t)a[1], (void*)(uintptr_t)a[2], (void*)(uintptr_t)a[3], (void*)(uintptr_t)a[4], (void*)(uintptr_t)a[5], (void*)(uintptr_t)a[6], (void*)(uintptr_t)a[7], (void*)(uintptr_t)a[8], (void*)(uintptr_t)a[9], (int)(int64_t)a[10], (int)(int64_t)a[11], (int)(int64_t)a[12], (int)(int64_t)a[13], (int)(int64_t)a[14], (int)(int64_t)a[15], (void*)(uintptr_t)a[16], (size_t)a[17], (void*)(uintptr_t)a[18], (void*)(uintptr_t)a[19]); }
static int t_radet_conv2d_igemm_pair(const uint64_t* a) { return radet_conv2d_igemm_pair((void*)(uintptr_t)a[0], (void*)(uintptr_t)a[1], (void*)(uintptr_t)a[2], (void*)(uintptr_t)a[3], (void*)(uintptr_t)a[4], (void*)(uintptr_t)a[5], (void*)(uintptr_t)a[6], (void*)(uintptr_t)a[7], (void*)(uintptr_t)a[8], (void*)(uintptr_t)a[9], (void*)(uintptr_t)a[10], (void*)(uintptr_t)a[11], (void*)(uintptr_t)a[12], (int)(int64_t)a[13], (int)(int64_t)a[14], (int)(int64_t)a[15], (int)(int64_t)a[16], (int)(int64_t)a[17], (int)(int64_t)a[18], (int)(int64_t)a[19], (void*)(uintptr_t)a[20], (size_t)a[21], (void*)(uintptr_t)a[22]); }
static int t_radet_conv2d_igemm_pair_s(const uint64_t* a) { return radet_conv2d_igemm_pair_s((void*)(uintptr_t)a[0], (void*)(uintptr_t)a[1], (void*)(uintptr_t)a[2], (void*)(uintptr_t)a[3], (void*)(uintptr_t)a[4], (void*)(uintptr_t)a[5], (void*)(uintptr_t)a[6], (void*)(uintptr_t)a[7], (void*)(uintptr_t)a[8], (void*)(uintptr_t)a[9], (void*)(uintptr_t)a[10], (void*)(uintptr_t)a[11], (void*)(uintptr_t)a[12], (int)(int64_t)a[13], (int)(int64_t)a[14], (int)(int64_t)a[15], (int)(int64_t)a[16], (int)(int64_t)a[17], (int)(int64_t)a[18], (int)(int64_t)a[19], (void*)(uintptr_t)a[20], (size_t)a[21], (void*)(uintptr_t)a[22], (void*)(uintptr_t)a[23]); }
static int t_radet_conv2d_igemm_s(const uint64_t* a) { return radet_conv2d_igemm_s((void*)(uintptr_t)a[0], (void*)(uintptr_t)a[1], (void*)(uintptr_t)a[2], (void*)(uintptr_t)a[3], (void*)(uintptr_t)a[4], (void*)(uintptr_t)a[5], (void*)(uintptr_t)a[6], (int)(int64_t)a[7], (int)(int64_t)a[8], (int)(int64_t)a[9], (int)(int64_t)a[10], (int)(int64_t)a[11], (int)(int64_t)a[12], (int)(int64_t)a[13], (void*)(uintptr_t)a[14], (size_t)a[15], (void*)(uintptr_t)a[16], (void*)(uintptr_t)a[17]); }
static int t_radet_conv2d_igemm_taps(const uint64_t* a) { return radet_conv2d_igemm_taps((void*)(uintptr_t)a[0], (void*)(uintptr_t)a[1], (void*)(uintptr_t)a[2], (void*)(uintptr_t)a[3], (void*)(uintptr_t)a[4], (void*)(uintptr_t)a[5], (void*)(uintptr_t)a[6], (void*)(uintptr_t)a[7], (int)(int64_t)a[8], (int)(int64_t)a[9], (int)(int64_t)a[10], (int)(int64_t)a[11], (int)(int64_t)a[12], (int)(int64_t)a[13], (void*)(uintptr_t)a[14], (size_t)a[15], (void*)(uintptr_t)a[16]); }
static int t_radet_conv2d_igemm_taps_s(const uint64_t* a) { return radet_conv2d_igemm_taps_s((void*)(uintptr_t)a[0], (void*)(uintptr_t)a[1], (void*)(uintptr_t)a[2], (void*)(uintptr_t)a[3], (void*)(uintptr_t)a[4], (void*)(uintptr_t)a[5], (void*)(uintptr_t)a[6], (void*)(uintptr_t)a[7], (int)(int64_t)a[8], (int)(int64_t)a[9], (int)(int64_t)a[10], (int)(int64_t)a[11], (int)(int64_t)a[12], (int)(int64_t)a[13], (void*)(uintptr_t)a[14], (size_t)a[15], (void*)(uintptr_t)a[16], (void*)(uintptr_t)a[17]); }
static int t_radet_conv2d_wgrad(const uint64_t* a) { return radet_conv2d_wgrad((void*)(uintptr_t)a[0], (void*)(uintptr_t)a[1], (void*)(uintptr_t)a[2], (void*)(uintptr_t)a[3], (void*)(uintptr_t)a[4], (int)(int64_t)a[5], (int)(int64_t)a[6], (int)(int64_t)a[7], (int)(int64_t)a[8], (int)(int64_t)a[9], (int)(int64_t)a[10], (int)(int64_t)a[11], (int)(int64_t)a[12], (void*)(uintptr_t)a[13]); }
static int t_radet_conv2d_wgrad_group(const uint64_t* a) { return radet_conv2d_wgrad_group((void*)(uintptr_t)a[0], (int)(int64_t)a[1], (int)(int64_t)a[2], (void*)(uintptr_t)a[3]); }
static int t_radet_conv2d_wgrad_s(const uint64_t* a) { return radet_conv2d_wgrad_s((void*)(uintptr_t)a[0], (void*)(uintptr_t)a[1], (void*)(uintptr_t)a[2], (void*)(uintptr_t)a[3], (void*)(uintptr_t)a[4], (int)(int64_t)a[5], (int)(int64_t)a[6], (int)(int64_t)a[7], (int)(int64_t)a[8], (int)(int64_t)a[9], (int)(int64_t)a[10], (int)(int64_t)a[11], (int)(int64_t)a[12], (void*)(uintptr_t)a[13], (void*)(uintptr_t)a[14]); }
static int t_radet_conv2d_wgrad_splits(const uint64_t* a) { return radet_conv2d_wgrad_splits((int)(int64_t)a[0], (int)(int64_t)a[1], (int)(int64_t)a[2], (int)(int64_t)a[3], (int)(int64_t)a[4]); }
static int t_radet_convert_rows(const uint64_t* a) { return radet_convert_rows((void*)(uintptr_t)a[0], (void*)(uintptr_t)a[1], (size_t)a[2], (int)(int64_t)a[3], (int)(int64_t)a[4], (int)(int64_t)a[5], (int)(int64_t)a[6], (int)(int64_t)a[7], (int)(int64_t)a[8], (void*)(uintptr_t)a[9]); }
static int t_radet_copy_d2d(const uint64_t* a) { return radet_copy_d2d((void*)(uintptr_t)a[0], (void*)(uintptr_t)a[1], (size_t)a[2], (void*)(uintptr_t)a[3]); }
static int t_radet_copy_segments(const uint64_t* a) { return radet_copy_segments((void*)(uintptr_t)a[0], (int)(int64_t)a[1], (int)(int64_t)a[2], (void*)(uintptr_t)a[3]); }
static int t_radet_crop_canvases(const uint64_t* a) { return radet_crop_canvases((void*)(uintptr_t)a[0], (size_t)a[1], (void*)(uintptr_t)a[2], (void*)(uintptr_t)a[3], (int)(int64_t)a[4], (void*)(uintptr_t)a[5], (int)(int64_t)a[6], (int)(int64_t)a[7], (void*)(uintptr_t)a[8], (size_t)a[9], (void*)(uintptr_t)a[10]); }
static int t_radet_cutout_f32(const uint64_t* a) { return radet_cutout_f32((void*)(uintptr_t)a[0], (int)(int64_t)a[1], (int)(int64_t)a[2], (int)(int64_t)a[3], (void*)(uintptr_t)a[4], (int)(int64_t)a[5], (void*)(uintptr_t)a[6], (int)(int64_t)a[7], (int)(int64_t)a[8], (int)(int64_t)a[9], f32(a[10]), f32(a[11]), f32(a[12]), f32(a[13]), f32(a[14]), f32(a[15]), (void*)(uintptr_t)a[16]); }
static int t_radet_cutout_u8(const uint64_t* a) { return radet_cutout_u8((void*)(uintptr_t)a[0], (size_t)a[1], (void*)(uintptr_t)a[2], (int)(int64_t)a[3], (void*)(uintptr_t)a[4], (int)(int64_t)a[5], (int)(int64_t)a[6], (int)(int64_t)a[7], (int)(int64_t)a[8], (void*)(uintptr_t)a[9]); }
static int t_radet_decode_candidates(const uint64_t* a) { return radet_decode_candidates((void*)(uintptr_t)a[0], (void*)(uintptr_t)a[1], (void*)(uintptr_t)a[2], (void*)(uintptr_t)a[3], (void*)(uintptr_t)a[4], (int)(int64_t)a[5], (int)(int64_t)a[6], (int)(int64_t)a[7], f32(a[8]), (int)(int64_t)a[9], (void*)(uintptr_t)a[10], (void*)(uintptr_t)a[11], (void*)(uintptr_t)a[12], (void*)(uintptr_t)a[13], (void*)(uintptr_t)a[14], (void*)(uintptr_t)a[15], (void*)(uintptr_t)a[16], (void*)(uintptr_t)a[17], (void*)(uintptr_t)a[18]); }
static int t_radet_fill_zero(const uint64_t* a) { return radet_fill_zero((void*)(uintptr_t)a[0], (size_t)a[1], (void*)(uintptr_t)a[2]); }
static int t_radet_fold_weights(const uint64_t* a) { return radet_fold_weights((void*)(uintptr_t)a[0], (int)(int64_t)a[1], (void*)(uintptr_t)a[2]); }
static int t_radet_gather_table_rows(const uint64_t* a) { return radet_gather_table_rows((int)(int64_t)a[0]); }
static int t_radet_gaussian_blur9_u8(const uint64_t* a) { return radet_gaussian_blur9_u8((void*)(uintptr_t)a[0], (void*)(uintptr_t)a[1], (void*)(uintptr_t)a[2], (void*)(uintptr_t)a[3], (void*)(uintptr_t)a[4], (int)(int64_t)a[5], (int)(int64_t)a[6], (void*)(uintptr_t)a[7]); }
static int t_radet_gdt(const uint64_t* a) { return radet_gdt((void*)(uintptr_t)a[0], (void*)(uintptr_t)a[1], (int)(int64_t)a[2], (void*)(uintptr_t)a[3], (void*)(uintptr_t)a[4], (void*)(uintptr_t)a[5], (void*)(uintptr_t)a[6], (void*)(uintptr_t)a[7]); }
static int t_radet_giou_loss(const uint64_t* a) { return radet_giou_loss((void*)(uintptr_t)a[0], (void*)(uintptr_t)a[1], (void*)(uintptr_t)a[2], (size_t)a[3], f32(a[4]), (void*)(uintptr_t)a[5], f32(a[6]), (void*)(uintptr_t)a[7], (void*)(uintptr_t)a[8]); }
static int t_radet_giou_loss_bwd(const uint64_t* a) { return radet_giou_loss_bwd((void*)(uintptr_t)a[0], (void*)(uintptr_t)a[1], (void*)(uintptr_t)a[2], (size_t)a[3], f32(a[4]), (void*)(uintptr_t)a[5], (void*)(uintptr_t)a[6], (void*)(uintptr_t)a[7], f32(a[8]), (void*)(uintptr_t)a[9], (void*)(uintptr_t)a[10]); }
static int t_radet_gn_relu_bwd(const uint64_t* a) { return radet_gn_relu_bwd((void*)(uintptr_t)a[0], (void*)(uintptr_t)a[1], (void*)(uintptr_t)a[2], (void*)(uintptr_t)a[3], (void*)(uintptr_t)a[4], (void*)(uintptr_t)a[5], (void*)(uintptr_t)a[6], (void*)(uintptr_t)a[7], (void*)(uintptr_t)a[8], (int)(int64_t)a[9], (int)(int64_t)a[10], (int)(int64_t)a[11], (int)(int64_t)a[12], (void*)(uintptr_t)a[13], (int)(int64_t)a[14], (void*)(uintptr_t)a[15]); }
static int t_radet_gn_relu_bwd_h(const uint64_t* a) { return radet_gn_relu_bwd_h((void*)(uintptr_t)a[0], (void*)(uintptr_t)a[1], (void*)(uintptr_t)a[2], (void*)(uintptr_t)a[3], (void*)(uintptr_t)a[4], (void*)(uintptr_t)a[5], (void*)(uintptr_t)a[6], (void*)(uintptr_t)a[7], (void*)(uintptr_t)a[8], (int)(int64_t)a[9], (int)(int64_t)a[10], (int)(int64_t)a[11], (int)(int64_t)a[12], (void*)(uintptr_t)a[13], (int)(int64_t)a[14], (void*)(uintptr_t)a[15]); }
static int t_radet_gn_relu_bwd_p(const uint64_t* a) { return radet_gn_relu_bwd_p((void*)(uintptr_t)a[0], (void*)(uintptr_t)a[1], (void*)(uintptr_t)a[2], (void*)(uintptr_t)a[3], (void*)(uintptr_t)a[4], (void*)(uintptr_t)a[5], (void*)(uintptr_t)a[6], (void*)(uintptr_t)a[7], (void*)(uintptr_t)a[8], (void*)(uintptr_t)a[9], (int)(int64_t)a[10], (int)(int64_t)a[11], (int)(int64_t)a[12], (int)(int64_t)a[13], (void*)(uintptr_t)a[14], (int)(int64_t)a[15], (void*)(uintptr_t)a[16]); }
static int t_radet_gn_relu_bwd_q(const uint64_t* a) { return radet_gn_relu_bwd_q((void*)(uintptr_t)a[0], (void*)(uintptr_t)a[1], (void*)(uintptr_t)a[2], (void*)(uintptr_t)a[3], (void*)(uintptr_t)a[4], (void*)(uintptr_t)a[5], (void*)(uintptr_t)a[6], (void*)(uintptr_t)a[7], (void*)(uintptr_t)a[8], (void*)(uintptr_t)a[9], (int)(int64_t)a[10], (int)(int64_t)a[11], (int)(int64_t)a[12], (int)(int64_t)a[13], (void*)(uintptr_t)a[14], (int)(int64_t)a[15], (void*)(uintptr_t)a[16], (void*)(uintptr_t)a[17], (void*)(uintptr_t)a[18], (void*)(uintptr_t)a[19]); }
static int t_radet_gn_relu_fwd(const uint64_t* a) { return radet_gn_relu_fwd((void*)(uintptr_t)a[0], (void*)(uintptr_t)a[1], (void*)(uintptr_t)a[2], (void*)(uintptr_t)a[3], (void*)(uintptr_t)a[4], (void*)(uintptr_t)a[5], (int)(int64_t)a[6], (int)(int64_t)a[7], (int)(int64_t)a[8], f32(a[9]), (int)(int64_t)a[10], (void*)(uintptr_t)a[11], (int)(int64_t)a[12], (void*)(uintptr_t)a[13]); }
static int t_radet_gn_relu_fwd_h(const uint64_t* a) { return radet_gn_relu_fwd_h((void*)(uintptr_t)a[0], (void*)(uintptr_t)a[1], (void*)(uintptr_t)a[2], (void*)(uintptr_t)a[3], (void*)(uintptr_t)a[4], (void*)(uintptr_t)a[5], (int)(int64_t)a[6], (int)(int64_t)a[7], (int)(int64_t)a[8], f32(a[9]), (int)(int64_t)a[10], (void*)(uintptr_t)a[11], (int)(int64_t)a[12], (void*)(uintptr_t)a[13]); }
static int t_radet_gn_relu_fwd_p(const uint64_t* a) { return radet_gn_relu_fwd_p((void*)(uintptr_t)a[0], (void*)(uintptr_t)a[1], (void*)(uintptr_t)a[2], (void*)(uintptr_t)a[3], (void*)(uintptr_t)a[4], (void*)(uintptr_t)a[5], (void*)(uintptr_t)a[6], (int)(int64_t)a[7], (int)(int64_t)a[8], (int)(int64_t)a[9], f32(a[10]), (int)(int64_t)a[11], (void*)(uintptr_t)a[12], (int)(int64_t)a[13], (void*)(uintptr_t)a[14]); }
static int t_radet_gn_relu_fwd_pair(const uint64_t* a) { return radet_gn_relu_fwd_pair((void*)(uintptr_t)a[0], (void*)(uintptr_t)a[1], (void*)(uintptr_t)a[2], (void*)(uintptr_t)a[3], (void*)(uintptr_t)a[4], (void*)(uintptr_t)a[5], (void*)(uintptr_t)a[6], (void*)(uintptr_t)a[7], (void*)(uintptr_t)a[8], (void*)(uintptr_t)a[9], (void*)(uintptr_t)a[10], (void*)(uintptr_t)a[11], (int)(int64_t)a[12], (int)(int64_t)a[13], (int)(int64_t)a[14], f32(a[15]), (int)(int64_t)a[16], (void*)(uintptr_t)a[17], (int)(int64_t)a[18], (void*)(uintptr_t)a[19]); }
static int t_radet_gn_relu_fwd_pair_h(const uint64_t* a) { return radet_gn_relu_fwd_pair_h((void*)(uintptr_t)a[0], (void*)(uintptr_t)a[1], (void*)(uintptr_t)a[2], (void*)(uintptr_t)a[3], (void*)(uintptr_t)a[4], (void*)(uintptr_t)a[5], (void*)(uintptr_t)a[6], (void*)(uintptr_t)a[7], (void*)(uintptr_t)a[8], (void*)(uintptr_t)a[9], (void*)(uintptr_t)a[10], (void*)(uintptr_t)a[11], (int)(int64_t)a[12], (int)(int64_t)a[13], (int)(int64_t)a[14], f32(a[15]), (int)(int64_t)a[16], (void*)(uintptr_t)a[17], (int)(int64_t)a[18], (void*)(uintptr_t)a[19]); }
static int t_radet_gn_relu_fwd_pair_p(const uint64_t* a) { return radet_gn_relu_fwd_pair_p((void*)(uintptr_t)a[0], (void*)(uintptr_t)a[1], (void*)(uintptr_t)a[2], (void*)(uintptr_t)a[3], (void*)(uintptr_t)a[4], (void*)(uintptr_t)a[5], (void*)(uintptr_t)a[6], (void*)(uintptr_t)a[7], (void*)(uintptr_t)a[8], (void*)(uintptr_t)a[9], (void*)(uintptr_t)a[10], (void*)(uintptr_t)a[11], (void*)(uintptr_t)a[12], (void*)(uintptr_t)a[13], (int)(int64_t)a[14], (int)(int64_t)a[15], (int)(int64_t)a[16], f32(a[17]), (int)(int64_t)a[18], (void*)(uintptr_t)a[19], (int)(int64_t)a[20], (void*)(uintptr_t)a[21]); }
static int t_radet_gn_relu_fwd_pair_q(const uint64_t* a) { return radet_gn_relu_fwd_pair_q((void*)(uintptr_t)a[0], (void*)(uintptr_t)a[1], (void*)(uintptr_t)a[2], (void*)(uintptr_t)a[3], (void*)(uintptr_t)a[4], (void*)(uintptr_t)a[5], (void*)(uintptr_t)a[6], (void*)(uintptr_t)a[7], (void*)(uintptr_t)a[8], (void*)(uintptr_t)a[9], (void*)(uintptr_t)a[10], (void*)(uintptr_t)a[11], (void*)(uintptr_t)a[12], (void*)(uintptr_t)a[13], (void*)(uintptr_t)a[14], (void*)(uintptr_t)a[15], (void*)(uintptr_t)a[16], (void*)(uintptr_t)a[17], (void*)(uintptr_t)a[18], (void*)(uintptr_t)a[19], (int)(int64_t)a[20], (int)(int64_t)a[21], (int)(int64_t)a[22], f32(a[23]), (int)(int64_t)a[24], (void*)(uintptr_t)a[25], (int)(int64_t)a[26], (void*)(uintptr_t)a[27]); }
static int t_radet_gn_relu_fwd_q(const uint64_t* a) { return radet_gn_relu_fwd_q((void*)(uintptr_t)a[0], (void*)(uintptr_t)a[1], (void*)(uintptr_t)a[2], (void*)(uintptr_t)a[3], (void*)(uintptr_t)a[4], (void*)(uintptr_t)a[5], (void*)(uintptr_t)a[6], (int)(int64_t)a[7], (int)(int64_t)a[8], (int)(int64_t)a[9], f32(a[10]), (int)(int64_t)a[11], (void*)(uintptr_t)a[12], (int)(int64_t)a[13], (void*)(uintptr_t)a[14], (void*)(uintptr_t)a[15], (void*)(uintptr_t)a[16], (void*)(uintptr_t)a[17]); }
static int t_radet_gn_workspace_floats(const uint64_t* a) { return radet_gn_workspace_floats((int)(int64_t)a[0], (void*)(uintptr_t)a[1], (int)(int64_t)a[2]); }
static int t_radet_grad_accumulate(const uint64_t* a) { return radet_grad_accumulate((void*)(uintptr_t)a[0], (void*)(uintptr_t)a[1], (size_t)a[2], (int)(int64_t)a[3], (void*)(uintptr_t)a[4]); }
static int t_radet_grid_anchors(const uint64_t* a) { return radet_grid_anchors((void*)(uintptr_t)a[0], (void*)(uintptr_t)a[1], (int)(int64_t)a[2], (int)(int64_t)a[3], (void*)(uintptr_t)a[4]); }
static int t_radet_head_loss(const uint64_t* a) { return radet_head_loss((void*)(uintptr_t)a[0], (void*)(uintptr_t)a[1], (void*)(uintptr_t)a[2], (void*)(uintptr_t)a[3], (void*)(uintptr_t)a[4], (void*)(uintptr_t)a[5], (void*)(uintptr_t)a[6], (void*)(uintptr_t)a[7], (void*)(uintptr_t)a[8], (void*)(uintptr_t)a[9], (int)(int64_t)a[10], (int)(int64_t)a[11], (int)(int64_t)a[12], f32(a[13]), f32(a[14]), f32(a[15]), f32(a[16]), (void*)(uintptr_t)a[17], (void*)(uintptr_t)a[18], (void*)(uintptr_t)a[19], (int)(int64_t)a[20], (void*)(uintptr_t)a[21], (int)(int64_t)a[22], (void*)(uintptr_t)a[23], (int)(int64_t)a[24], (void*)(uintptr_t)a[25], (void*)(uintptr_t)a[26], (void*)(uintptr_t)a[27], (int)(int64_t)a[28], (void*)(uintptr_t)a[29], (void*)(uintptr_t)a[30]); }
static int t_radet_head_loss_ws_ints(const uint64_t* a) { return radet_head_loss_ws_ints((int)(int64_t)a[0]); }
static int t_radet_jpeg_decode(const uint64_t* a) { return radet_jpeg_decode((void*)(uintptr_t)a[0], (void*)(uintptr_t)a[1], (int)(int64_t)a[2], (void*)(uintptr_t)a[3], (int)(int64_t)a[4], (void*)(uintptr_t)a[5], (void*)(uintptr_t)a[6], (void*)(uintptr_t)a[7], (int)(int64_t)a[8], (void*)(uintptr_t)a[9], (void*)(uintptr_t)a[10], (void*)(uintptr_t)a[11], (void*)(uintptr_t)a[12], (int)(int64_t)a[13], (int)(int64_t)a[14], (int)(int64_t)a[15], (void*)(uintptr_t)a[16]); }
static int t_radet_jpeg_index(const uint64_t* a) { return radet_jpeg_index((void*)(uintptr_t)a[0], (int)(int64_t)a[1], (int)(int64_t)a[2], (int)(int64_t)a[3], (void*)(uintptr_t)a[4], (void*)(uintptr_t)a[5], (int)(int64_t)a[6], (int)(int64_t)a[7], (int)(int64_t)a[8], (void*)(uintptr_t)a[9], (int)(int64_t)a[10]); }
static int t_radet_loss_finalize(const uint64_t* a) { return radet_loss_finalize((void*)(uintptr_t)a[0], (int)(int64_t)a[1], (void*)(uintptr_t)a[2], f32(a[3]), (void*)(uintptr_t)a[4], (void*)(uintptr_t)a[5]); }
static int t_radet_loss_partials(const uint64_t* a) { return radet_loss_partials((size_t)a[0]); }
static int t_radet_mask_max(const uint64_t* a) { return radet_mask_max((void*)(uintptr_t)a[0], (void*)(uintptr_t)a[1], (int)(int64_t)a[2], (size_t)a[3], (void*)(uintptr_t)a[4]); }
static int t_radet_mask_transform(const uint64_t* a) { return radet_mask_transform((void*)(uintptr_t)a[0], (void*)(uintptr_t)a[1], (void*)(uintptr_t)a[2], (void*)(uintptr_t)a[3], (int)(int64_t)a[4], (int)(int64_t)a[5], (int)(int64_t)a[6], (int)(int64_t)a[7], (int)(int64_t)a[8], (int)(int64_t)a[9], (int)(int64_t)a[10], (int)(int64_t)a[11], (int)(int64_t)a[12], (void*)(uintptr_t)a[13]); }
static int t_radet_maxpool3x3s2(const uint64_t* a) { return radet_maxpool3x3s2((void*)(uintptr_t)a[0], (void*)(uintptr_t)a[1], (int)(int64_t)a[2], (int)(int64_t)a[3], (int)(int64_t)a[4], (int)(int64_t)a[5], (void*)(uintptr_t)a[6]); }
static int t_radet_maxpool3x3s2_a(const uint64_t* a) { return radet_maxpool3x3s2_a((void*)(uintptr_t)a[0], (void*)(uintptr_t)a[1], (int)(int64_t)a[2], (int)(int64_t)a[3], (int)(int64_t)a[4], (int)(int64_t)a[5], (void*)(uintptr_t)a[6], (void*)(uintptr_t)a[7]); }
static int t_radet_maxpool3x3s2_bwd_relu(const uint64_t* a) { return radet_maxpool3x3s2_bwd_relu((void*)(uintptr_t)a[0], (void*)(uintptr_t)a[1], (void*)(uintptr_t)a[2], (int)(int64_t)a[3], (int)(int64_t)a[4], (int)(int64_t)a[5], (int)(int64_t)a[6], (void*)(uintptr_t)a[7]); }
static int t_radet_maxpool3x3s2_h(const uint64_t* a) { return radet_maxpool3x3s2_h((void*)(uintptr_t)a[0], (void*)(uintptr_t)a[1], (int)(int64_t)a[2], (int)(int64_t)a[3], (int)(int64_t)a[4], (int)(int64_t)a[5], (void*)(uintptr_t)a[6]); }
static int t_radet_maxpool3x3s2_q(const uint64_t* a) { return radet_maxpool3x3s2_q((void*)(uintptr_t)a[0], (void*)(uintptr_t)a[1], (int)(int64_t)a[2], (int)(int64_t)a[3], (int)(int64_t)a[4], (int)(int64_t)a[5], (void*)(uintptr_t)a[6], (void*)(uintptr_t)a[7], (void*)(uintptr_t)a[8], (void*)(uintptr_t)a[9], (void*)(uintptr_t)a[10]); }
static int t_radet_mbd(const uint64_t* a) { return radet_mbd((void*)(uintptr_t)a[0], (void*)(uintptr_t)a[1], (int)(int64_t)a[2], (void*)(uintptr_t)a[3], (void*)(uintptr_t)a[4], f32(a[5]), (int)(int64_t)a[6], (int)(int64_t)a[7], (void*)(uintptr_t)a[8], (size_t)a[9], (void*)(uintptr_t)a[10], (void*)(uintptr_t)a[11]); }
static int t_radet_merge_pairs(const uint64_t* a) { return radet_merge_pairs((void*)(uintptr_t)a[0], (void*)(uintptr_t)a[1], (size_t)a[2], (int)(int64_t)a[3], (int)(int64_t)a[4], (void*)(uintptr_t)a[5], (void*)(uintptr_t)a[6]); }
// ... 11 lines not shown
static int t_radet_resize_linear_u8(const uint64_t* a) { return radet_resize_linear_u8((void*)(uintptr_t)a[0], (void*)(uintptr_t)a[1], (void*)(uintptr_t)a[2], (void*)(uintptr_t)a[3], (void*)(uintptr_t)a[4], (int)(int64_t)a[5], (int)(int64_t)a[6], (int)(int64_t)a[7], (void*)(uintptr_t)a[8]); }
static int t_radet_rle_masks(const uint64_t* a) { return radet_rle_masks((void*)(uintptr_t)a[0], (int)(int64_t)a[1], (void*)(uintptr_t)a[2], (int)(int64_t)a[3], (void*)(uintptr_t)a[4], (void*)(uintptr_t)a[5], (int)(int64_t)a[6], (void*)(uintptr_t)a[7], (void*)(uintptr_t)a[8], (int)(int64_t)a[9], (int)(int64_t)a[10], (int)(int64_t)a[11], (int)(int64_t)a[12], (int)(int64_t)a[13], (void*)(uintptr_t)a[14]); }
static int t_radet_scale_relu(const uint64_t* a) { return radet_scale_relu((void*)(uintptr_t)a[0], (void*)(uintptr_t)a[1], (void*)(uintptr_t)a[2], (void*)(uintptr_t)a[3], (int)(int64_t)a[4], (int)(int64_t)a[5], (void*)(uintptr_t)a[6]); }
static int t_radet_sgd_step(const uint64_t* a) { return radet_sgd_step((void*)(uintptr_t)a[0], (void*)(uintptr_t)a[1], (void*)(uintptr_t)a[2], (size_t)a[3], f32(a[4]), f32(a[5]), f32(a[6]), f32(a[7]), (int)(int64_t)a[8], (int)(int64_t)a[9], f32(a[10]), f32(a[11]), (void*)(uintptr_t)a[12], (int)(int64_t)a[13], (void*)(uintptr_t)a[14], (void*)(uintptr_t)a[15], (int)(int64_t)a[16], (void*)(uintptr_t)a[17]); }
static int t_radet_sigmoid_focal_loss(const uint64_t* a) { return radet_sigmoid_focal_loss((void*)(uintptr_t)a[0], (void*)(uintptr_t)a[1], (void*)(uintptr_t)a[2], (int)(int64_t)a[3], (size_t)a[4], (int)(int64_t)a[5], f32(a[6]), f32(a[7]), (void*)(uintptr_t)a[8], f32(a[9]), (void*)(uintptr_t)a[10], (void*)(uintptr_t)a[11]); }
static int t_radet_sigmoid_focal_loss_bwd(const uint64_t* a) { return radet_sigmoid_focal_loss_bwd((void*)(uintptr_t)a[0], (void*)(uintptr_t)a[1], (void*)(uintptr_t)a[2], (int)(int64_t)a[3], (size_t)a[4], (int)(int64_t)a[5], f32(a[6]), f32(a[7]), (void*)(uintptr_t)a[8], (void*)(uintptr_t)a[9], (void*)(uintptr_t)a[10], f32(a[11]), (void*)(uintptr_t)a[12], (void*)(uintptr_t)a[13]); }
static int t_radet_sobel_edge(const uint64_t* a) { return radet_sobel_edge((void*)(uintptr_t)a[0], (void*)(uintptr_t)a[1], (void*)(uintptr_t)a[2], (void*)(uintptr_t)a[3], (void*)(uintptr_t)a[4], (int)(int64_t)a[5], (int)(int64_t)a[6], (void*)(uintptr_t)a[7]); }
static int t_radet_split_pairs(const uint64_t* a) { return radet_split_pairs((void*)(uintptr_t)a[0], (void*)(uintptr_t)a[1], (size_t)a[2], (int)(int64_t)a[3], (int)(int64_t)a[4], (void*)(uintptr_t)a[5], (void*)(uintptr_t)a[6], (void*)(uintptr_t)a[7]); }
static int t_radet_split_planes(const uint64_t* a) { return radet_split_planes((void*)(uintptr_t)a[0], (void*)(uintptr_t)a[1], (size_t)a[2], (int)(int64_t)a[3], (int)(int64_t)a[4], (void*)(uintptr_t)a[5]); }
static int t_radet_sqnorm_partials(const uint64_t* a) { return radet_sqnorm_partials((void*)(uintptr_t)a[0], (size_t)a[1], (void*)(uintptr_t)a[2], (int)(int64_t)a[3], (void*)(uintptr_t)a[4]); }
static int t_radet_stem_conv_bn_relu(const uint64_t* a) { return radet_stem_conv_bn_relu((void*)(uintptr_t)a[0], (void*)(uintptr_t)a[1], (void*)(uintptr_t)a[2], (void*)(uintptr_t)a[3], (int)(int64_t)a[4], (int)(int64_t)a[5], (int)(int64_t)a[6], (void*)(uintptr_t)a[7]); }
static int t_radet_stem_conv_bn_relu_a(const uint64_t* a) { return radet_stem_conv_bn_relu_a((void*)(uintptr_t)a[0], (void*)(uintptr_t)a[1], (void*)(uintptr_t)a[2], (void*)(uintptr_t)a[3], (int)(int64_t)a[4], (int)(int64_t)a[5], (int)(int64_t)a[6], (void*)(uintptr_t)a[7], (void*)(uintptr_t)a[8]); }
static int t_radet_stem_conv_bn_relu_h(const uint64_t* a) { return radet_stem_conv_bn_relu_h((void*)(uintptr_t)a[0], (void*)(uintptr_t)a[1], (void*)(uintptr_t)a[2], (void*)(uintptr_t)a[3], (int)(int64_t)a[4], (int)(int64_t)a[5], (int)(int64_t)a[6], (void*)(uintptr_t)a[7]); }
static int t_radet_stem_wgrad(const uint64_t* a) { return radet_stem_wgrad((void*)(uintptr_t)a[0], (void*)(uintptr_t)a[1], (void*)(uintptr_t)a[2], (void*)(uintptr_t)a[3], (int)(int64_t)a[4], (int)(int64_t)a[5], (int)(int64_t)a[6], (int)(int64_t)a[7], (void*)(uintptr_t)a[8]); }
static int t_radet_stem_wgrad_splits(const uint64_t* a) { return radet_stem_wgrad_splits((int)(int64_t)a[0], (int)(int64_t)a[1], (int)(int64_t)a[2]); }
static int t_radet_stream_create_cumask(const uint64_t* a) { return radet_stream_create_cumask((void*)(uintptr_t)a[0], (int)(int64_t)a[1], (void*)(uintptr_t)a[2]); }
static int t_radet_tblr_decode(const uint64_t* a) { return radet_tblr_decode((void*)(uintptr_t)a[0], (void*)(uintptr_t)a[1], (void*)(uintptr_t)a[2], (int)(int64_t)a[3], (void*)(uintptr_t)a[4], (int)(int64_t)a[5], f32(a[6]), f32(a[7]), (int)(int64_t)a[8], (void*)(uintptr_t)a[9]); }
static int t_radet_tblr_encode(const uint64_t* a) { return radet_tblr_encode((void*)(uintptr_t)a[0], (void*)(uintptr_t)a[1], (void*)(uintptr_t)a[2], (int)(int64_t)a[3], (void*)(uintptr_t)a[4], (int)(int64_t)a[5], (void*)(uintptr_t)a[6]); }
static int t_radet_threshold_compact(const uint64_t* a) { return radet_threshold_compact((void*)(uintptr_t)a[0], (size_t)a[1], f32(a[2]), (void*)(uintptr_t)a[3], (void*)(uintptr_t)a[4], (void*)(uintptr_t)a[5]); }
static int t_radet_unfold_grads(const uint64_t* a) { return radet_unfold_grads((void*)(uintptr_t)a[0], (int)(int64_t)a[1], (int)(int64_t)a[2], (void*)(uintptr_t)a[3]); }
static int t_radet_upsample_add(const uint64_t* a) { return radet_upsample_add((void*)(uintptr_t)a[0], (void*)(uintptr_t)a[1], (int)(int64_t)a[2], (int)(int64_t)a[3], (int)(int64_t)a[4], (int)(int64_t)a[5], (int)(int64_t)a[6], (int)(int64_t)a[7], (void*)(uintptr_t)a[8]); }
static int t_radet_upsample_add_a(const uint64_t* a) { return radet_upsample_add_a((void*)(uintptr_t)a[0], (void*)(uintptr_t)a[1], (int)(int64_t)a[2], (int)(int64_t)a[3], (int)(int64_t)a[4], (int)(int64_t)a[5], (int)(int64_t)a[6], (int)(int64_t)a[7], (void*)(uintptr_t)a[8], (void*)(uintptr_t)a[9]); }
static int t_radet_upsample_add_bwd(const uint64_t* a) { return radet_upsample_add_bwd((void*)(uintptr_t)a[0], (void*)(uintptr_t)a[1], (int)(int64_t)a[2], (int)(int64_t)a[3], (int)(int64_t)a[4], (int)(int64_t)a[5], (int)(int64_t)a[6], (int)(int64_t)a[7], (void*)(uintptr_t)a[8]); }
static int t_radet_upsample_add_bwd_a(const uint64_t* a) { return radet_upsample_add_bwd_a((void*)(uintptr_t)a[0], (void*)(uintptr_t)a[1], (int)(int64_t)a[2], (int)(int64_t)a[3], (int)(int64_t)a[4], (int)(int64_t)a[5], (int)(int64_t)a[6], (int)(int64_t)a[7], (void*)(uintptr_t)a[8], (void*)(uintptr_t)a[9]); }
static int t_radet_upsample_add_bwd_h(const uint64_t* a) { return radet_upsample_add_bwd_h((void*)(uintptr_t)a[0], (void*)(uintptr_t)a[1], (int)(int64_t)a[2], (int)(int64_t)a[3], (int)(int64_t)a[4], (int)(int64_t)a[5], (int)(int64_t)a[6], (int)(int64_t)a[7], (void*)(uintptr_t)a[8]); }
static int t_radet_upsample_add_h(const uint64_t* a) { return radet_upsample_add_h((void*)(uintptr_t)a[0], (void*)(uintptr_t)a[1], (int)(int64_t)a[2], (int)(int64_t)a[3], (int)(int64_t)a[4], (int)(int64_t)a[5], (int)(int64_t)a[6], (int)(int64_t)a[7], (void*)(uintptr_t)a[8]); }
static int t_radet_warp_affine_u8(const uint64_t* a) { return radet_warp_affine_u8((void*)(uintptr_t)a[0], (size_t)a[1], (void*)(uintptr_t)a[2], (size_t)a[3], (void*)(uintptr_t)a[4], (int)(int64_t)a[5], (int)(int64_t)a[6], (int)(int64_t)a[7], (void*)(uintptr_t)a[8]); }

typedef int (*radet_thunk_fn)(const uint64_t*);
const struct RadetTapeThunk { const char* name; radet_thunk_fn fn; int nargs; } radet_tape_thunks[] = {
    {"radet_absmax", t_radet_absmax, 4},
    {"radet_adamw_step", t_radet_adamw_step, 17},
    {"radet_adamw_step_runs", t_radet_adamw_step_runs, 19},
    {"radet_amax_slot_words", t_radet_amax_slot_words, 0},
    {"radet_assign_points", t_radet_assign_points, 19},
    {"radet_assign_points_f", t_radet_assign_points_f, 19},
    {"radet_augment_box", t_radet_augment_box, 8},
    {"radet_augment_finish", t_radet_augment_finish, 14},
    {"radet_augment_hsv_noise", t_radet_augment_hsv_noise, 6},
    {"radet_augment_merge_hblur", t_radet_augment_merge_hblur, 8},
    {"radet_augment_sharp", t_radet_augment_sharp, 7},
    {"radet_augment_vblur", t_radet_augment_vblur, 7},
    {"radet_bbox_overlaps", t_radet_bbox_overlaps, 10},
    {"radet_bce_logits_loss", t_radet_bce_logits_loss, 10},
    {"radet_bce_logits_loss_bwd", t_radet_bce_logits_loss_bwd, 12},
    {"radet_box_loss", t_radet_box_loss, 11},
    {"radet_box_loss_bwd", t_radet_box_loss_bwd, 13},
    {"radet_build_gather_table", t_radet_build_gather_table, 11},
    {"radet_coco_accumulate", t_radet_coco_accumulate, 17},
    {"radet_coco_match", t_radet_coco_match, 17},
    {"radet_conv2d_igemm", t_radet_conv2d_igemm, 17},
    {"radet_conv2d_igemm_classes", t_radet_conv2d_igemm_classes, 19},
    {"radet_conv2d_igemm_classes_s", t_radet_conv2d_igemm_classes_s, 20},
    {"radet_conv2d_igemm_pair", t_radet_conv2d_igemm_pair, 23},
    {"radet_conv2d_igemm_pair_s", t_radet_conv2d_igemm_pair_s, 24},
    {"radet_conv2d_igemm_s", t_radet_conv2d_igemm_s, 18},
    {"radet_conv2d_igemm_taps", t_radet_conv2d_igemm_taps, 17},
    {"radet_conv2d_igemm_taps_s", t_radet_conv2d_igemm_taps_s, 18},
    {"radet_conv2d_wgrad", t_radet_conv2d_wgrad, 14},
    {"radet_conv2d_wgrad_group", t_radet_conv2d_wgrad_group, 4},
    {"radet_conv2d_wgrad_s", t_radet_conv2d_wgrad_s, 15},
    {"radet_conv2d_wgrad_splits", t_radet_conv2d_wgrad_splits, 5},
    {"radet_convert_rows", t_radet_convert_rows, 10},
    {"radet_copy_d2d", t_radet_copy_d2d, 4},
    {"radet_copy_segments", t_radet_copy_segments, 4},
    {"radet_crop_canvases", t_radet_crop_canvases, 11},
    {"radet_cutout_f32", t_radet_cutout_f32, 17},
    {"radet_cutout_u8", t_radet_cutout_u8, 10},
    {"radet_decode_candidates", t_radet_decode_candidates, 19},
    {"radet_fill_zero", t_radet_fill_zero, 3},
    {"radet_fold_weights", t_radet_fold_weights, 3},
    {"radet_gather_table_rows", t_radet_gather_table_rows, 1},
    {"radet_gaussian_blur9_u8", t_radet_gaussian_blur9_u8, 8},
    {"radet_gdt", t_radet_gdt, 8},
    {"radet_giou_loss", t_radet_giou_loss, 9},
    {"radet_giou_loss_bwd", t_radet_giou_loss_bwd, 11},
    {"radet_gn_relu_bwd", t_radet_gn_relu_bwd, 16},
    {"radet_gn_relu_bwd_h", t_radet_gn_relu_bwd_h, 16},
    {"radet_gn_relu_bwd_p", t_radet_gn_relu_bwd_p, 17},
    {"radet_gn_relu_bwd_q", t_radet_gn_relu_bwd_q, 20},
    {"radet_gn_relu_fwd", t_radet_gn_relu_fwd, 14},
    {"radet_gn_relu_fwd_h", t_radet_gn_relu_fwd_h, 14},
    {"radet_gn_relu_fwd_p", t_radet_gn_relu_fwd_p, 15},
    {"radet_gn_relu_fwd_pair", t_radet_gn_relu_fwd_pair, 20},
    {"radet_gn_relu_fwd_pair_h", t_radet_gn_relu_fwd_pair_h, 20},
    {"radet_gn_relu_fwd_pair_p", t_radet_gn_relu_fwd_pair_p, 22},
    {"radet_gn_relu_fwd_pair_q", t_radet_gn_relu_fwd_pair_q, 28},
    {"radet_gn_relu_fwd_q", t_radet_gn_relu_fwd_q, 18},
    {"radet_gn_workspace_floats", t_radet_gn_workspace_floats, 3},
    {"radet_grad_accumulate", t_radet_grad_accumulate, 5},
    {"radet_grid_anchors", t_radet_grid_anchors, 5},
    {"radet_head_loss", t_radet_head_loss, 31},
    {"radet_head_loss_ws_ints", t_radet_head_loss_ws_ints, 1},
    {"radet_jpeg_decode", t_radet_jpeg_decode, 17},
    {"radet_jpeg_index", t_radet_jpeg_index, 11},
    {"radet_loss_finalize", t_radet_loss_finalize, 6},
    {"radet_loss_partials", t_radet_loss_partials, 1},
    {"radet_mask_max", t_radet_mask_max, 5},
    {"radet_mask_transform", t_radet_mask_transform, 14},
    {"radet_maxpool3x3s2", t_radet_maxpool3x3s2, 7},
    {"radet_maxpool3x3s2_a", t_radet_maxpool3x3s2_a, 8},
    {"radet_maxpool3x3s2_bwd_relu", t_radet_maxpool3x3s2_bwd_relu, 8},
    {"radet_maxpool3x3s2_h", t_radet_maxpool3x3s2_h, 7},
    {"radet_maxpool3x3s2_q", t_radet_maxpool3x3s2_q, 11},
    {"radet_mbd", t_radet_mbd, 12},
    {"radet_merge_pairs", t_radet_merge_pairs, 7},
    {"radet_merge_planes", t_radet_merge_planes, 6},
    {"radet_nchw_to_nhwc", t_radet_nchw_to_nhwc, 7},
    {"radet_nhwc_to_nchw", t_radet_nhwc_to_nchw, 7},
    {"radet_nms", t_radet_nms, 20},
    {"radet_paste_maps", t_radet_paste_maps, 9},
    {"radet_pred3x3_patch", t_radet_pred3x3_patch, 13},
    {"radet_preprocess_frames", t_radet_preprocess_frames, 12},
    {"radet_relu_bwd", t_radet_relu_bwd, 6},
    {"radet_relu_bwd_a", t_radet_relu_bwd_a, 7},
    {"radet_relu_bwd_h", t_radet_relu_bwd_h, 6},
    {"radet_resize_linear_f", t_radet_resize_linear_f, 8},
    {"radet_resize_linear_u8", t_radet_resize_linear_u8, 9},
    {"radet_rle_masks", t_radet_rle_masks, 15},
    {"radet_scale_relu", t_radet_scale_relu, 7},
    {"radet_sgd_step", t_radet_sgd_step, 18},
    {"radet_sigmoid_focal_loss", t_radet_sigmoid_focal_loss, 12},
    {"radet_sigmoid_focal_loss_bwd", t_radet_sigmoid_focal_loss_bwd, 14},
    {"radet_sobel_edge", t_radet_sobel_edge, 8},
    {"radet_split_pairs", t_radet_split_pairs, 8},
    {"radet_split_planes", t_radet_split_planes, 6},
    {"radet_sqnorm_partials", t_radet_sqnorm_partials, 5},
    {"radet_stem_conv_bn_relu", t_radet_stem_conv_bn_relu, 8},
    {"radet_stem_conv_bn_relu_a", t_radet_stem_conv_bn_relu_a, 9},
    {"radet_stem_conv_bn_relu_h", t_radet_stem_conv_bn_relu_h, 8},
    {"radet_stem_wgrad", t_radet_stem_wgrad, 9},
    {"radet_stem_wgrad_splits", t_radet_stem_wgrad_splits, 3},
    {"radet_stream_create_cumask", t_radet_stream_create_cumask, 3},
    {"radet_tblr_decode", t_radet_tblr_decode, 10},
    {"radet_tblr_encode", t_radet_tblr_encode, 7},
    {"radet_threshold_compact", t_radet_threshold_compact, 6},
    {"radet_unfold_grads", t_radet_unfold_grads, 4},
    {"radet_upsample_add", t_radet_upsample_add, 9},
    {"radet_upsample_add_a", t_radet_upsample_add_a, 10},
    {"radet_upsample_add_bwd", t_radet_upsample_add_bwd, 9},
    {"radet_upsample_add_bwd_a", t_radet_upsample_add_bwd_a, 10},
    {"radet_upsample_add_bwd_h", t_radet_upsample_add_bwd_h, 9},
    {"radet_upsample_add_h", t_radet_upsample_add_h, 9},
    {"radet_warp_affine_u8", t_radet_warp_affine_u8, 9},
};
const int radet_tape_nthunks = 114;
```

radet_amd/engine.py:

```python
import contextlib
import ctypes as C
import os

import torch

from . import _lib
from . import kernels as K
from .kernels import ConvGeom, Levels

ARCH = {50: (3, 4, 6, 3), 101: (3, 4, 23, 3)}


def conv_out_hw(h, w, k, s, p):
    return (h + 2 * p - k) // s + 1, (w + 2 * p - k) // s + 1


class _StemSplits:

    def __init__(self, nsplit):
        self.nsplit = nsplit


class Conv:

    def __init__(self, name, cin, cout, k, stride, pad, bn=None, bias=False, trainable=True, dgrad=True):
        self.name, self.cin, self.cout, self.k, self.stride, self.pad = name, cin, cout, k, stride, pad
        self.bn, self.bias, self.trainable, self.need_dgrad = bn, bias, trainable, dgrad
        self.wft_ld, self.wft_off, self.wft_shared = 0, 0, None
        self.grouped = False
        self.geom = None
        self.wf = self.wft = self.bias_f = self.slabs = self.dbias_partials = None

    @property
    def wsize(self):
        return self.cout * self.cin * self.k * self.k


class Engine:
    def __init__(self, params, grads, depth=50, num_classes=21, frozen_stages=1, strides=(8, 16, 32, 64, 128),
                 stacked_convs=4, feat=256, math=None, watch=None):
        math = math or os.environ.get("RADET_MATH", "fp32")
        assert math in ("fp32", "fp32-mfma", "bf16", "bf16-storage"), math
        self.watch = watch or {}
        self._watched = {}
        self.math = 1 if math == "bf16" else 0
        self.h16 = math == "bf16-storage"
        x3mode = os.environ.get("RADET_X3", "h2")
        self.x3 = math == "fp32" and x3mode != "0"
        self.h2 = self.x3 and x3mode not in ("bf16", "b3")
        self.pairs = self.h2 and os.environ.get("RADET_PAIRS", "0") == "1"
        self.po = self.h2 and not self.pairs and os.environ.get("RADET_PAIRS_ONLY", "0") == "1"
        self.po_max_planes = int(os.environ.get("RADET_PAIRS_ONLY_MAX", "512"))
        self.pairs_from = int(os.environ.get("RADET_PAIRS_FROM", "2"))
        if self.x3 and "RADET_TOWER_MODE" not in os.environ:
            self.tower_mode = "pairbwd"
        self.p3 = self.x3 and self.tower_mode == "pairbwd" and feat % 32 == 0 and os.environ.get("RADET_P3", "1") != "0"
        self.math_name = math
        self.act_dtype = torch.bfloat16 if self.h16 else torch.float32
        self.p, self.g = params, grads
        self.depth, self.num_classes, self.frozen_stages = depth, num_classes, frozen_stages
        self.strides, self.stacked_convs, self.feat = tuple(strides), stacked_convs, feat
        self.dev = next(iter(params.values())).device
        self.convs = []
        self._build_layers()
        self._alloc_folded()
        self.geo_key = None
        self.table = None

    TOWER_TAG = K.SYMBOL | K.BK32 | 3
    TOWER_TAG_FWD = K.SYMBOL | K.BK32 | 2

    tower_stages = K.STAGES3 if os.environ.get("RADET_TOWER_STAGES3", "0") == "1" else 0
    tower_tile = int(os.environ.get("RADET_TOWER_TILE", "6"))
    if os.environ.get("RADET_TOWER_ROWPAIRS", "0") == "1":
        tower_tile |= K.ROWPAIRS

    def _ttile(self, c, bwd=False, tag=True, pair=True):
        fp32 = not self.math and not self.h16
        if self.p3:
            return (6 if pair else 5) | (K.SYMBOL if tag else 0) | self.tower_stages
        if fp32 and self.x3:
            t = K.BK32 | 1
        elif bwd:
            t = (self.TOWER_TAG & ~K.SYMBOL) if fp32 else (self.tower_bwd_tile_h16 or c.geom.bwd_tile)
        else:
            t = (self.TOWER_TAG_FWD & ~K.SYMBOL) | (K.STAGES3 if fp32 else 0)
            if not fp32 and self.tower_fwd_tile_h16:
                t = self.tower_fwd_tile_h16
        return t | (K.SYMBOL if tag else 0)
    tower_fwd_tile_h16 = int(os.environ.get("RADET_TOWER_FWD_TILE", "0"), 0)
    tower_bwd_tile_h16 = int(os.environ.get("RADET_TOWER_BWD_TILE", str(K.BK32 | 1)), 0)
    tower_events = None
    _pfx_ready = None

    def _tower_launch(self, fn, *args, **kw):
        ev = self.tower_events
        if ev is None:
            return fn(*args, **kw)
        s, e = torch.cuda.Event(enable_timing=True), torch.cuda.Event(enable_timing=True)
        s.record()
        fn(*args, **kw)
        e.record()
        ev.append((s, e))

    def tower_gemm_flops(self):
        return 2.0 * self.R * self.feat * 9 * self.feat

    def _add(self, conv):
        self.convs.append(conv)
        return conv

    def _build_layers(self):
        fs = self.frozen_stages
        if fs < 0 and self.h16:
            raise NotImplementedError("ResNet(frozen_stages=-1) (trainable stem) with bf16 storage is not implemented on MI355X: "
                                      "every RADet config freezes the stem (frozen_stages >= 0; the BOP configs use 1)")
        self.stem = self._add(Conv("backbone.conv1", 3, 64, 7, 2, 3, bn="backbone.bn1", trainable=fs < 0, dgrad=False))
        self.stages = []
        inpl = 64
        for li, nb in enumerate(ARCH[self.depth]):
            planes = 64 * 2 ** li
            train = (li + 1) > fs
            blocks = []
            for b in range(nb):
                pfx = f"backbone.layer{li + 1}.{b}"
                stride = 2 if (b == 0 and li > 0) else 1
                in_dgrad = train and not (b == 0 and li <= fs)
                blk = dict(
                    c1=self._add(Conv(pfx + ".conv1", inpl, planes, 1, 1, 0, bn=pfx + ".bn1", trainable=train, dgrad=in_dgrad)),
                    c2=self._add(Conv(pfx + ".conv2", planes, planes, 3, stride, 1, bn=pfx + ".bn2", trainable=train, dgrad=train)),
                    c3=self._add(Conv(pfx + ".conv3", planes, planes * 4, 1, 1, 0, bn=pfx + ".bn3", trainable=train, dgrad=train)),
                    ds=None, stride=stride, train=train,
                    po=self.po and stride == 1 and planes % 32 == 0 and planes <= self.po_max_planes)
                if b == 0:
                    blk["ds"] = self._add(Conv(pfx + ".downsample.0", inpl, planes * 4, 1, stride, 0, bn=pfx + ".downsample.1",
                                               trainable=train, dgrad=in_dgrad))
                inpl = planes * 4
                blocks.append(blk)
            self.stages.append(blocks)
        f = self.feat
        self.lat = [self._add(Conv(f"neck.lateral_convs.{i}.conv", c, f, 1, 1, 0, bias=True)) for i, c in enumerate((512, 1024, 2048))]
        self.fpn = [self._add(Conv(f"neck.fpn_convs.{i}.conv", f, f, 3, 1 if i < 3 else 2, 1, bias=True)) for i in range(5)]
        self.cls_tower = [self._add(Conv(f"bbox_head.cls_convs.{i}.conv", f, f, 3, 1, 1)) for i in range(self.stacked_convs)]
        self.reg_tower = [self._add(Conv(f"bbox_head.reg_convs.{i}.conv", f, f, 3, 1, 1)) for i in range(self.stacked_convs)]
        self.pred_cls = self._add(Conv("bbox_head.atss_cls", f, self.num_classes, 3, 1, 1, bias=True))
        self.pred_reg = self._add(Conv("bbox_head.atss_reg", f, 4, 3, 1, 1, bias=True))
        self.pred_iou = self._add(Conv("bbox_head.atss_centerness", f, 1, 3, 1, 1, bias=True))
        kq = 32 if self.h16 else 16
        self.cls_pad = ((self.num_classes + kq - 1) // kq) * kq
        self.ri_pad = kq
        self.iou_col = 8 if self.h16 else 4
        self.pred_cls.wft_ld, self.pred_cls.wft_off = self.cls_pad, 0
        self.pred_reg.wft_ld, self.pred_reg.wft_off = self.ri_pad, 0
        self.pred_iou.wft_ld, self.pred_iou.wft_off = self.ri_pad, self.iou_col
        self.pred_iou.wft_shared = self.pred_reg

    def _alloc_folded(self):
        dev = self.dev
        n_wf = sum(c.wsize for c in self.convs)
        n_b = sum(c.cout for c in self.convs)
        self.wf_arena = torch.zeros(n_wf, device=dev, dtype=self.act_dtype)
        self.stem_wf = torch.zeros(self.convs[0].wsize, device=dev)
        self.bias_arena = torch.zeros(n_b, device=dev)
        n_wft = 0
        for c in self.convs:
            if c.need_dgrad and c.wft_shared is None:
                ld = c.wft_ld or c.cout
                n_wft += c.cin * c.k * c.k * ld
        self.wft_arena = torch.zeros(n_wft, device=dev, dtype=self.act_dtype)
        self.w_amax = K.new_amax(dev, len(self.convs))
        self.w_l1 = K.new_amax(dev, len(self.convs)) if (self.pairs or self.po) else None
        self.b_amax = K.new_amax(dev, len(self.convs)) if (self.pairs or self.po) else None
        self.w_l1t = K.new_amax(dev, len(self.convs)) if self.po else None
        self._w_amax_keys = []
        o_w = o_b = o_t = 0
        towers = (self.cls_tower + self.reg_tower) if self.p3 else []
        po_c1 = [blk["c1"] for st in self.stages for blk in st if blk["po"]]
        po_c2 = [blk["c2"] for st in self.stages for blk in st if blk["po"]]
        po_c3 = [blk["c3"] for st in self.stages for blk in st if blk["po"] and blk["train"]]
        towers = towers + po_c2
        pkind = "h2" if self.h2 else "b3"
        for ci, c in enumerate(self.convs):
            c.w_amax = self.w_amax[ci]
            c.wfq = None
            c.wmeta = (self.w_l1[ci], self.b_amax[ci] if (c.bn or c.bias) else None) if (self.pairs or c in po_c1) else None
            c.wmeta_t = (self.w_l1t[ci], None) if c in po_c3 else None
            c.w16 = (3 if self.h2 else 2) if c in towers else (1 if (self.h16 and c is not self.convs[0]) else 0)
            c.wf = self.wf_arena[o_w:o_w + c.wsize] if c is not self.convs[0] else self.stem_wf
            o_w += c.wsize
# ... 85 lines not shown
            if only:
                q = K.Planes(rows, ch, device=dev, kind="h2")
                if prefix:
                    assert n_pfx[0] < self.amax_pfx[0].shape[0], "frozen prefix: more buffers than amax slots"
                    q.true_amax = self.amax_pfx[0][n_pfx[0]]
                    n_pfx[0] += 1
                    self._pfx_shapes[name] = (rows, ch, "pairs-only", False)
                    self._pfx_sets[0][name] = q
                else:
                    q.true_amax = slot()
                self.buf[name] = q
                return q
            t = torch.empty(rows, ch, device=dev, dtype=dtype or self.act_dtype)
            self.buf[name] = t
            if prefix:
                self._pfx_shapes[name] = (rows, ch, t.dtype, twin and self.pairs)
                self._pfx_sets[0][name] = t
            sl_ = None
            if self.h2 and t.dtype == torch.float32:
                if prefix:
                    assert n_pfx[0] < self.amax_pfx[0].shape[0], "frozen prefix: more buffers than amax slots"
                    sl_ = self.amax_pfx[0][n_pfx[0]]
                    n_pfx[0] += 1
                else:
                    sl_ = slot()
                self._amax_keys.append(K.register_amax(t, sl_, by_storage=True))
            if twin and self.pairs and ch % 32 == 0:
                q = K.Planes(rows, ch, device=dev, kind="h2")
                q.true_amax = sl_
                self.buf[name + "@q"] = q
                if prefix:
                    self._pfx_sets[0][name + "@q"] = q
            return t

        frozen_prefix = not self.stem.trainable
        new("stem", B * h1 * w1, 64, prefix=frozen_prefix)
        new("pool", B * h2 * w2, 64, prefix=frozen_prefix, twin=self.pairs_from <= 1)
        if self.stem.trainable:
            new("d_pool", B * h2 * w2, 64)
            new("d_stem", B * h1 * w1, 64)
            self.stem.geom = _StemSplits(K.stem_wgrad_splits(B, H, W))
        lv = Levels([(h2, w2)], B)
        for li, blocks in enumerate(self.stages):
            for b, blk in enumerate(blocks):
                pfx = f"l{li + 1}.{b}"
                blk["lin"] = lv
                fz = frozen_prefix and not blk["train"] and all(not bb["train"] for st in self.stages[:li] for bb in st)
                blk["c1"].geom = ConvGeom(lv, blk["c1"].cin, blk["c1"].cout, 1, 1, 0)
                blk["c2"].geom = ConvGeom(lv, blk["c2"].cin, blk["c2"].cout, 3, blk["stride"], 1)
                lo = blk["c2"].geom.lout
                blk["c3"].geom = ConvGeom(lo, blk["c3"].cin, blk["c3"].cout, 1, 1, 0)
                if blk["ds"] is not None:
                    blk["ds"].geom = ConvGeom(lv, blk["ds"].cin, blk["ds"].cout, 1, blk["stride"], 0)
                    new(pfx + ".idt", lo.rows, blk["ds"].cout, prefix=fz)
                blk["lout"] = lo
                tw = li + 1 >= self.pairs_from
                new(pfx + ".o1", lv.rows, blk["c1"].cout, prefix=fz, twin=tw, only=blk["po"])
                new(pfx + ".o2", lo.rows, blk["c2"].cout, prefix=fz, twin=tw)
                new(pfx + ".out", lo.rows, blk["c3"].cout, prefix=fz, twin=tw or (li + 2 == self.pairs_from and b == len(blocks) - 1))
                if blk["train"]:
                    new(pfx + ".d_o1", lv.rows, blk["c1"].cout)
                    new(pfx + ".d_o2", lo.rows, blk["c2"].cout, only=blk["po"])
                    new(pfx + ".d_pre", lo.rows, blk["c3"].cout)
                lv = lo
        c_lv = [self.stages[i][-1]["lout"] for i in (1, 2, 3)]
        f = self.feat
        for i in range(3):
            self.lat[i].geom = ConvGeom(c_lv[i], self.lat[i].cin, f, 1, 1, 0)
            new(f"lat{i}", c_lv[i].rows, f)
            new(f"d_lat{i}", c_lv[i].rows, f)
            new(f"d_c{i}", c_lv[i].rows, self.lat[i].cin)
        hw = [c_lv[i].hw[0] for i in range(3)]
        hw.append(conv_out_hw(*hw[-1], 3, 2, 1))
        hw.append(conv_out_hw(*hw[-1], 3, 2, 1))
        self.plv = Levels(hw, B)
        if self.x3:
            K._pred_tiles(self.plv)
        for i in range(3):
            self.fpn[i].geom = ConvGeom(c_lv[i], f, f, 3, 1, 1)
        self.fpn[3].geom = ConvGeom(self.plv.sub(2), f, f, 3, 2, 1)
        self.fpn[4].geom = ConvGeom(self.plv.sub(3), f, f, 3, 2, 1)
        R = self.plv.rows
        self.R = R
        new("P", R, f)
        new("dP", R, f)
        for lvl in (2, 3):
            r0, r1 = self.plv.level_rows(lvl)
            new(f"dP_tmp{lvl}", r1 - r0, f)
        pkind = "h2" if self.h2 else "b3"
        if self.p3:
            self.buf["Pp"] = K.Planes(R, f, device=dev, kind=pkind)
        for t in ("cls", "reg"):
            for i in range(self.stacked_convs):
                new(f"{t}.z{i}", R, f)
                if self.p3 and i < self.stacked_convs - 1:
                    self.buf[f"{t}.y{i}"] = K.Planes(R, f, device=dev, kind=pkind)
                else:
                    new(f"{t}.y{i}", R, f)
                if self.h2:
                    self.buf[f"{t}.zhat{i}"] = slot(aux=True)
                self.buf[f"{t}.stats{i}"] = torch.empty(len(hw) * B * 64, device=dev)
            new(f"{t}.dy", R, f)
            for nm in (f"{t}.dz0", f"{t}.dz1"):
                if self.p3:
                    self.buf[nm] = K.Planes(R, f, device=dev, kind=pkind)
                else:
                    new(nm, R, f)
# ... 9 lines not shown
        new("iou", R, 1, torch.float32)
        self.buf["dcls"] = torch.zeros(R, self.cls_pad, device=dev)
        self.buf["dregiou"] = torch.zeros(R, 16, device=dev)
        if self.h2:
            for nm in ("dcls", "dregiou"):
                self._amax_keys.append(K.register_amax(self.buf[nm], slot(), by_storage=True))
        if self.h16:
            self.buf["dcls16"] = torch.zeros(R, self.cls_pad, device=dev, dtype=torch.bfloat16)
            self.buf["dregiou16"] = torch.zeros(R, self.ri_pad, device=dev, dtype=torch.bfloat16)
        self.gn_ws = torch.empty(K.gn_ws_floats(self.plv), device=dev)
        self.gn_ws2 = torch.empty(K.gn_ws_floats(self.plv), device=dev)
        self.ldesc, self.nlvl = K.level_desc(self.plv, self.strides)
        self.loss_ws = torch.zeros(K.head_loss_ws_ints(R), dtype=torch.int32, device=dev)
        self.losses = torch.zeros(3, device=dev)
        self.dscales = torch.zeros(len(hw), device=dev)
        for c in self.convs:
            if c.geom is not None:
                c.geom.math = self.math
                c.geom.h16 = self.h16
                c.geom.x3 = self.x3
                c.geom.h2 = self.h2
                c.geom.pairs = c.wfq is not None or (self.po and c.w16 == 3 and c.name.startswith("backbone."))
        tune = os.environ.get("RADET_AUTOTUNE", "1") != "0"
        self._plan_wgrad_groups()
        if tune:
            K.load_tune_cache()
            for c in self.convs:
                if c.trainable and c.geom is not None and c.cout > 64 and c.cin > 64 and not c.grouped \
                        and c not in self.cls_tower and c not in self.reg_tower:
                    K.autotune_wgrad(c.geom)
        for c in self.convs:
            if c.geom is not None and hasattr(c.geom, "wgrad_pair_flags") and c not in self.cls_tower + self.reg_tower:
                c.geom.wgrad_pair_flags = K.WG_ONE_TAP | (c.geom.wgrad_flags & K.WG_TILE_MASK)
        n_slab = sum(c.geom.nsplit * c.wsize for c in self.convs if c.trainable)
        n_bp = sum(c.geom.nsplit * c.cout for c in self.convs if c.trainable)
        self.slab_arena = torch.empty(n_slab, device=dev)
        self.bp_arena = torch.zeros(n_bp, device=dev)
        o_s = o_b = 0
        for c in self.convs:
            if c.trainable:
                n = c.geom.nsplit * c.wsize
                c.slabs = self.slab_arena[o_s:o_s + n]
                o_s += n
                n = c.geom.nsplit * c.cout
                c.dbias_partials = self.bp_arena[o_b:o_b + n]
                o_b += n
        self._build_table()
        if tune:
            towers = self.cls_tower + self.reg_tower
            for c in self.convs:
                if c is not self.stem and c.geom is not None and (self.math or c not in towers):
                    K.autotune(c.geom, need_dgrad=c.need_dgrad)
            K.save_tune_cache()

    wgrad_group = os.environ.get("RADET_WGRAD_GROUP", "0") == "1"
    wgrad_group_tile = int(os.environ.get("RADET_WGRAD_GROUP_TILE", "128"))
    wgrad_group_slots = int(os.environ.get("RADET_WGRAD_GROUP_SLOTS", "512"))
    wgrad_flush_blocks = int(os.environ.get("RADET_WGRAD_FLUSH_BLOCKS", "0"))

    def _plan_wgrad_groups(self):
        for c in self.convs:
            c.grouped = False
        self._pending_wgrad = []
        if not self.wgrad_group or self.h16:
            return
        t = self.wgrad_group_tile
        fb = self.wgrad_flush_blocks
        groups = []
        for blocks in self.stages:
            rev = list(reversed(blocks))
            step = fb if fb > 0 else len(rev)
            for i in range(0, len(rev), step):
                groups.append([c for blk in rev[i:i + step] for c in (blk["c1"], blk["c2"], blk["c3"], blk["ds"])
                               if c is not None and c.trainable])
        groups.append(list(self.lat) + list(self.fpn))
        for grp in groups:
            grp = [c for c in grp if c.cout % t == 0 and c.cin % t == 0]
            if not grp:
                continue
            for c, s in zip(grp, K.group_splits([c.geom for c in grp], tile=t, slots=self.wgrad_group_slots)):
                c.grouped = True
                c.geom.nsplit = s

    def flush_wgrads(self):
        jobs, self._pending_wgrad = self._pending_wgrad, []
        if not jobs:
            return
        if not self.use_streams:
            K.conv_wgrad_group(jobs, tile=self.wgrad_group_tile, math=self.math)
            return
        side = self._side()
        self._fork(side)
        with torch.cuda.stream(side):
            K.conv_wgrad_group(jobs, tile=self.wgrad_group_tile, math=self.math)

    def _build_table(self):
        n = len(self.convs)
        arr = (_lib.RadetConvDesc * n)()

        def ptr(t):
            return None if t is None else C.c_void_p(t.data_ptr())

        for d, c in zip(arr, self.convs):
            p, g = self.p, self.g
            d.w = ptr(p[c.name + ".weight"])
            d.bias = ptr(p.get(c.name + ".bias")) if c.bias else None
# ... 74 lines not shown
    def _part_version(self, lo, hi):
        if os.environ.get("RADET_FOLD_EVERY_CALL"):
            return (object(),)
        key = (lo, hi)
        watched = self._watched.get(key)
        if watched is None:
            watched = []
            for c in self.convs[lo:hi]:
                names = [c.name + ".weight"] + ([c.name + ".bias"] if c.bias else [])
                if c.bn:
                    names += [c.bn + sfx for sfx in (".weight", ".bias", ".running_mean", ".running_var")]
                for k in names:
                    if k in self.p:
                        watched += list(self.watch.get(k, (self.p[k],)))
            self._watched[key] = watched
        return (tuple(t._version for t in watched), tuple(t.data_ptr() for t in watched), self.h16, self.math)

    def params_changed(self):
        self._param_epoch += 1

    def invalidate_fold(self):
        self._folded = (None, None)

    def _await_fold(self):
        if self._fold_event is not None:
            K.ev_wait(self._fold_event)
            self._fold_event = None

    def unfold(self):
        K.unfold_grads(self.table, len(self.convs), self.max_cout)

    def _block_forward(self, blk, pfx, x, b, xq=None):
        blk["x"] = x
        o1, o2, out = b[pfx + ".o1"], b[pfx + ".o2"], b[pfx + ".out"]
        c1, c2, c3, ds = blk["c1"], blk["c2"], blk["c3"], blk["ds"]
        if xq is not None and c1.wfq is not None and c2.wfq is not None and c3.wfq is not None and (ds is None or ds.wfq is not None):
            o1q, o2q, outq = b[pfx + ".o1@q"], b[pfx + ".o2@q"], b.get(pfx + ".out@q")
            K.conv_fwd(c1.geom, xq, c1.wfq, c1.bias_f, o1, relu=True, tile=c1.geom.fwd_tile_q, yq=o1q, wmeta=c1.wmeta)
            K.conv_fwd(c2.geom, o1q, c2.wfq, c2.bias_f, o2, relu=True, tile=c2.geom.fwd_tile_q, yq=o2q, wmeta=c2.wmeta)
            if ds is not None:
                idt = b[pfx + ".idt"]
                K.conv_fwd(ds.geom, xq, ds.wfq, ds.bias_f, idt, tile=ds.geom.fwd_tile_q)
            else:
                idt = x
            K.conv_fwd(c3.geom, o2q, c3.wfq, c3.bias_f, out, addend=idt, relu=True, tile=c3.geom.fwd_tile_q, yq=outq,
                       wmeta=c3.wmeta)
            return out
        if blk["po"]:
            K.conv_fwd(c1.geom, x, c1.wf, c1.bias_f, None, relu=True, yq=o1, wmeta=c1.wmeta)
            K.conv_fwd(c2.geom, o1, c2.wf, c2.bias_f, o2, relu=True, tile=c2.geom.fwd_tile_q)
        else:
            K.conv_fwd(blk["c1"].geom, x, blk["c1"].wf, blk["c1"].bias_f, o1, relu=True)
            K.conv_fwd(blk["c2"].geom, o1, blk["c2"].wf, blk["c2"].bias_f, o2, relu=True)
        if blk["ds"] is not None:
            idt = b[pfx + ".idt"]
            K.conv_fwd(blk["ds"].geom, x, blk["ds"].wf, blk["ds"].bias_f, idt)
        else:
            idt = x
        outq = b.get(pfx + ".out@q")
        K.conv_fwd(blk["c3"].geom, o2, blk["c3"].wf, blk["c3"].bias_f, out, addend=idt, relu=True, yq=outq,
                   wmeta=c3.wmeta if outq is not None else None)
        return out

    def _n_frozen_stages(self):
        n = 0
        while n < len(self.stages) and not self.stages[n][0]["train"]:
            n += 1
        return n

    def _prefix_forward(self, img, which):
        B, H, W = self.B, self.H, self.W
        b = self._pfx_sets[which]
        if self.h2:
            K.fill_zero(self.amax_pfx[which])
        K.STAGE = "stem"
        K.stem(img, self.stem.wf, self.stem.bias_f, b["stem"], B, H, W)
        K.maxpool(b["stem"], b["pool"], B, self.stem_hw[0], self.stem_hw[1], 64, yq=b.get("pool@q"))
        x, xq = b["pool"], b.get("pool@q")
        for li in range(self._n_frozen_stages()):
            K.STAGE = f"layer{li + 1}"
            for bi, blk in enumerate(self.stages[li]):
                x = self._block_forward(blk, f"l{li + 1}.{bi}", x, b, xq)
                xq = b.get(f"l{li + 1}.{bi}.out@q")
        return b

    @staticmethod
    def _img_key(img, geo):
        return (img.data_ptr(), img._version, tuple(img.shape), geo)

    def prefetch_prefix(self, next_img):
        if self.stem.trainable or not self.use_streams or next_img is None or self.geo_key is None:
            return False
        if tuple(next_img.shape) != (self.B, 3, self.H, self.W) or not next_img.is_contiguous():
            return False
        other = 1 - self._pfx_active
        if self._pfx_sets[other] is None:
            self._pfx_sets[other] = {}
            if self.h2:
                self.amax_pfx[other] = K.new_amax(self.dev, 128)
            for i, (name, (rows, ch, dt, twin)) in enumerate(self._pfx_shapes.items()):
                if dt == "pairs-only":
                    q = K.Planes(rows, ch, device=self.dev, kind="h2")
                    q.true_amax = self.amax_pfx[other][i]
                    self._pfx_sets[other][name] = q
                    continue
                t = torch.empty(rows, ch, device=self.dev, dtype=dt)
# ... 628 lines not shown
```

radet_amd/kernels.py:

```python
import ctypes as C
import os

import torch

from . import _lib

ID_MASK = 0xFF
SYMBOL = 0x100
BK32 = 0x200
MATH_BF16 = 0x400
STORE_BF16, OUT_F32 = 0x800, 0x10000
SPLITK, SPLITK_MASK = 0x1000, 0xF000
STAGES3 = 0x20000
STAGES4 = 0x40000
ROWPAIRS = 0x80000
STREAMK, STREAMK_MASK = 0x100000, 0x700000
X3 = 0x1000000
P3 = 0x2000000
H2 = 0x8000000
MASKQ = 0x10000000
WG_MATH_BF16, WG_STORE_BF16 = 0x1, 0x2
WG_TILE, WG_TILE_MASK = 0x10, 0x30
WG_ONE_TAP = 0x40
WG_PX32 = 0x80
# ... 702 lines not shown
def split_planes(src, dst, src_amax=None):
    assert src.dim() == 2 and src.dtype == torch.float32 and src.stride(1) == 1 and dst.C == src.shape[1]
    if dst.kind == "h2":
        sa = src_amax if src_amax is not None else amax_slot(src)
        if sa is None:
            sa = new_amax(src.device)
            absmax(src.contiguous(), sa)
        _lib.call("radet_split_pairs", src.data_ptr(), _ptr(dst.t), C.c_size_t(src.shape[0]), src.shape[1], src.stride(0),
                  _ptr(sa), _ptr(dst.amax), _stream())
        return
    _lib.call("radet_split_planes", C.c_void_p(src.data_ptr()), _ptr(dst.t), C.c_size_t(src.shape[0]), src.shape[1],
              src.stride(0), _stream())


def merge_planes(src, dst):
    assert dst.dim() == 2 and dst.dtype == torch.float32 and dst.stride(1) == 1 and src.C == dst.shape[1]
    if src.kind == "h2":
        _lib.call("radet_merge_pairs", _ptr(src.t), dst.data_ptr(), C.c_size_t(dst.shape[0]), dst.shape[1], dst.stride(0),
                  _ptr(src.amax), _stream())
        return
    _lib.call("radet_merge_planes", _ptr(src.t), C.c_void_p(dst.data_ptr()), C.c_size_t(dst.shape[0]), dst.shape[1],
              dst.stride(0), _stream())


def _is16(t):
    return t is not None and not _isp(t) and t.dtype == torch.bfloat16


def _tile(g, tile, default, x=None, y=None):
    t = (tile or default) | (MATH_BF16 if g.math else 0)
    if _isp(x):
        if tile_id(t) == 8:
            t = with_tile(t, 3)
        return (t & ~(MATH_BF16 | BK32)) | P3 | (H2 if x.kind == "h2" else 0)
    if getattr(g, "x3", False) and not g.math and not _is16(x):
        t |= X3 | (H2 if getattr(g, "h2", False) else 0)
    if _is16(x):
        t = (t & ~MATH_BF16) | STORE_BF16 | (OUT_F32 if (y is not None and y.dtype == torch.float32) else 0)
    return t


def conv_fwd(g, x, wf, bias, y, addend=None, mask=None, relu=False, tile=0, splitk=True, yq=None, wmeta=None):
    assert y is not None or yq is not None
    tile = _tile(g, tile, g.fwd_tile, x, y)
    ws = splitk_ws() if splitk else None
    table = g.fwd_table
    sc = _scales(x, wf, y, need=bool(tile & H2), yq=yq, wmeta=wmeta, addend=addend)

    def launch():
        _lib.call("radet_conv2d_igemm_s", _ptr_any(x), _ptr_any(wf), _ptr(bias), _ptr(addend), _ptr(mask), _ptr(y), _ptr(table),
                  g.lout.rows, g.cin, g.cout, g.k, g.k, int(relu), tile, _ptr(ws), C.c_size_t(ws.numel() if splitk else 0),
                  _stream(), sc)
    _timed(lambda: _igemm_key(tile, x), 2.0 * g.lout.rows * g.cout * g.cin * g.k * g.k, launch, _conv_bytes(g), geom=g)


def _pred_tiles(lv):
    import numpy as np
    t = getattr(lv, "_pred_tiles", None)
    if t is None:
        rows = []
        for (h, w), off in zip(lv.hw, lv.offsets):
            for n in range(lv.B):
                for ty in range(-(-h // 8)):
                    for tx in range(-(-w // 16)):
                        rows.append((off + n * h * w, h, w, (ty << 16) | tx))
        t = torch.from_numpy(np.asarray(rows, np.int32)).cuda()
        if not torch.cuda.is_current_stream_capturing():
            torch.cuda.current_stream().synchronize()
        lv._pred_tiles = t
    return t


def pred_conv_patch(lv, x, a, b=None):
    t = _pred_tiles(lv)
    cin = x.shape[1]
    w1, b1, y1, c1 = b if b is not None else (None, None, None, 0)
    _timed("pred3x3_patch_kernel", 2.0 * lv.rows * (a[3] + c1) * cin * 9,
           lambda: _lib.call("radet_pred3x3_patch", _ptr(x), cin, _ptr(t), t.shape[0], _ptr(a[0]), _ptr(a[1]), _ptr(a[2]), a[3],
                             _ptr(w1), _ptr(b1), _ptr(y1), c1, _stream()))


_WTUNE_CACHE = _LRU(8192)


def autotune_wgrad(g, reps=None):
    dev = torch.device("cuda", torch.cuda.current_device())
    reps = reps or TUNE_REPS
    global _TUNE_DIRTY, TUNE_RUNS
    key = (g._key, g.cin, g.cout, g.math, g.h16, "w") + (("x3",) if getattr(g, "x3", False) else ()) + _h2key(g)
    if key not in _WTUNE_CACHE:
        _TUNE_DIRTY = True
        TUNE_RUNS += 1
        M, kk = g.lout.rows, g.k * g.k
        s0 = g.nsplit
        cands = [(0, s0)]
        if g.cout > 64 and g.cin > 64:
            for tid in (1, 2, 3) if getattr(g, "x3", False) else (1, 2):
                tflag, (t, tn) = tid * WG_TILE, WG_TILE_SHAPE[tid]
                tiles = -(-g.cout // t) * -(-g.cin // tn) * kk
                for blocks in (256, 512, 768, 1024):
                    S = max(1, min(64, round(blocks / tiles), (M + 127) // 128))
                    cands.append((tflag | WG_ONE_TAP, S))
                    if not g.math and not g.h16:
                        cands.append((tflag | WG_ONE_TAP | WG_PX32, S))
                    if getattr(g, "x3", False) and t == 64:
                        cands += [(tflag | WG_ONE_TAP | WG_KDIV4, S), (tflag | WG_ONE_TAP | WG_KDIV2, S)]
# ... 837 lines not shown
```

Before: 503.4.

## Fuse bottleneck downsample shortcut into c3 conv via dual-source GEMM kernel

Result: no change. 500.9 (-0.5%).

```diff
diff --git a/include/radet_hip.h b/include/radet_hip.h
--- a/include/radet_hip.h
+++ b/include/radet_hip.h
@@ -84,6 +84,10 @@
                               const float* mask0, float* y0, const float* x1, const float* w1, const float* bias1,
                               const float* addend1, const float* mask1, float* y1, const int* gather_table, int M,
                               int Cin, int Cout, int KH, int KW, int relu, int tile_override, float* splitk_ws,
+                              size_t splitk_ws_floats, void* stream, const RadetScales* sc);
+int radet_conv2d_igemm_dual_s(const float* x0, const float* w0, const float* bias0, const int* table0, int Cin0, int rows0,
+                              const float* x1, const float* w1, const float* bias1, const int* table1, int Cin1, int rows1,
+                              float* y, int M, int Cout, int relu, int tile_override, float* splitk_ws,
                               size_t splitk_ws_floats, void* stream, const RadetScales* sc);
 int radet_conv2d_igemm_taps_s(const float* x, const float* w, const float* addend, const float* mask, float* y,
                               const int* gather_table, const int* out_rows, const int* tap_ids_host, int ntaps, int kt_w,
diff --git a/radet_amd/_lib.py b/radet_amd/_lib.py
--- a/radet_amd/_lib.py
+++ b/radet_amd/_lib.py
@@ -42,6 +42,7 @@
     "radet_conv2d_igemm_classes": (_i, [_p, _p, _p, _p, _p, _p, _p, _p, _p, _p, _i, _i, _i, _i, _i, _i, _p, _sz, _p]),
     "radet_conv2d_igemm_s": (_i, [_p, _p, _p, _p, _p, _p, _p, _i, _i, _i, _i, _i, _i, _i, _p, _sz, _p, _p]),
     "radet_conv2d_igemm_pair_s": (_i, [_p] * 13 + [_i, _i, _i, _i, _i, _i, _i, _p, _sz, _p, _p]),
+    "radet_conv2d_igemm_dual_s": (_i, [_p, _p, _p, _p, _i, _i, _p, _p, _p, _p, _i, _i, _p, _i, _i, _i, _i, _p, _sz, _p, _p]),
     "radet_conv2d_igemm_taps_s": (_i, [_p, _p, _p, _p, _p, _p, _p, _p, _i, _i, _i, _i, _i, _i, _p, _sz, _p, _p]),
     "radet_conv2d_igemm_classes_s": (_i, [_p, _p, _p, _p, _p, _p, _p, _p, _p, _p, _i, _i, _i, _i, _i, _i, _p, _sz, _p, _p]),
     "radet_conv2d_wgrad_s": (_i, [_p, _p, _p, _p, _p, _i, _i, _i, _i, _i, _i, _i, _i, _p, _p]),
diff --git a/radet_amd/csrc/conv_common.h b/radet_amd/csrc/conv_common.h
--- a/radet_amd/csrc/conv_common.h
+++ b/radet_amd/csrc/conv_common.h
@@ -45,6 +45,8 @@
     int cls_nt, cls_b[3];
     int dbg;
     int maskq;
+    int Cin0;
+    const int* rowtab1;
 };
 
 __device__ __forceinline__ float ld_act(const float* p, size_t o, int io) {
@@ -146,6 +148,7 @@
     float* partial;
     int* counters;
     int sk_base, sk_rem;
+    const float* bias1;
 };
 template <class T>
 __device__ __forceinline__ T pin_sgpr(T v) {
@@ -153,7 +156,7 @@
     return v;
 }
 
-template <int BM, int BN, int WM, int WN, int IO>
+template <int BM, int BN, int WM, int WN, int IO, bool B1 = false>
 __device__ __forceinline__ void igemm_epilogue(const EpiArgs& a, const ConvPtrs& P,
                                                f32x16 (&acc)[BM / (WM * 32)][BN / (WN * 32)], int m0, int n0, int wm, int wn,
                                                int li, int lh) {
@@ -189,7 +192,8 @@
             const int col = n0 + (wn * TN + j) * 32 + li;
             const bool cvalid = col < a.Cout;
             const int cc = cvalid ? col : 0;
-            const float bv = P.bias ? P.bias[cc] : 0.f;
+            float bv = P.bias ? P.bias[cc] : 0.f;
+            if constexpr (B1) { if (a.bias1) bv += a.bias1[cc]; }
             float av[16], mv[16];
             if (has_add) {
 #pragma unroll
@@ -339,7 +343,7 @@
     return true;
 }
 
-template <int BM, int BN, int WM, int WN>
+template <int BM, int BN, int WM, int WN, bool B1 = false>
 __device__ __forceinline__ void igemm_store(const EpiArgs& e, const ConvPtrs& P,
                                             f32x16 (&acc)[BM / (WM * 32)][BN / (WN * 32)], int m0, int n0, int nsplit,
                                             int ctile, int z, int wm, int wn, int li, int lh, volatile int* ws) {
@@ -365,7 +369,8 @@
                 for (int r = 0; r < 16; ++r) acc[i][j][r] = 0.f;
         for (int zz = 0; zz < nsplit; ++zz) partial_add<BM, BN, WM, WN>(base + (size_t)zz * BM * BN, acc);
     }
-    if (e.io == 0) igemm_epilogue<BM, BN, WM, WN, 0>(e, P, acc, m0, n0, wm, wn, li, lh);
+    if constexpr (B1) igemm_epilogue<BM, BN, WM, WN, 0, true>(e, P, acc, m0, n0, wm, wn, li, lh);
+    else if (e.io == 0) igemm_epilogue<BM, BN, WM, WN, 0>(e, P, acc, m0, n0, wm, wn, li, lh);
     else if (e.io == 1) igemm_epilogue<BM, BN, WM, WN, 1>(e, P, acc, m0, n0, wm, wn, li, lh);
     else igemm_epilogue<BM, BN, WM, WN, 2>(e, P, acc, m0, n0, wm, wn, li, lh);
 }
@@ -476,6 +481,31 @@
     asm volatile("" : "+v"(raw));
     return h2_scale_bits(radet_amax_reduce(raw));
 }
+struct H2Dual {
+    H2Scale x[2], w[2];
+    float inv_a, inv_b;
+};
+__device__ __forceinline__ H2Scale h2_scale_lowered(int e, int by) {
+    H2Scale r;
+    const int el = e - by;
+    r.s = el >= -126 ? radet_pow2(el) : 0.f;
+    r.s2 = el >= -126 ? radet_pow2(el + 11) : 0.f;
+    r.inv = radet_pow2(-e);
+    return r;
+}
+__device__ __forceinline__ H2Dual h2_dual_scales(unsigned raw_x0, unsigned raw_w0, unsigned raw_x1, unsigned raw_w1) {
+    asm volatile("" : "+v"(raw_x0), "+v"(raw_w0), "+v"(raw_x1), "+v"(raw_w1));
+    const int ex0 = radet_h2_exp(radet_amax_reduce(raw_x0)), ew0 = radet_h2_exp(radet_amax_reduce(raw_w0));
+    const int ex1 = radet_h2_exp(radet_amax_reduce(raw_x1)), ew1 = radet_h2_exp(radet_amax_reduce(raw_w1));
+    const int d = (ex0 + ew0) - (ex1 + ew1);
+    H2Dual r;
+    r.x[0] = h2_scale_lowered(ex0, 0); r.x[1] = h2_scale_lowered(ex1, 0);
+    r.w[0] = h2_scale_lowered(ew0, d > 0 ? d : 0);
+    r.w[1] = h2_scale_lowered(ew1, d < 0 ? -d : 0);
+    r.inv_a = d > 0 ? r.x[1].inv : r.x[0].inv;
+    r.inv_b = d > 0 ? r.w[1].inv : r.w[0].inv;
+    return r;
+}
 __device__ __forceinline__ void split2_f16(const float (&a)[8], const H2Scale& sc, f16x8& hi, f16x8& lo) {
     u32x4_ h, l;
 #pragma unroll
diff --git a/radet_amd/csrc/conv_dual.hip b/radet_amd/csrc/conv_dual.hip
--- /dev/null
+++ b/radet_amd/csrc/conv_dual.hip
@@ -0,0 +1,130 @@
+#include "common.h"
+#include "../../include/radet_hip.h"
+#include <stdlib.h>
+#include <type_traits>
+
+#include "conv_igemm_kernel.h"
+
+constexpr int DUAL_H2 = TAG_H2 | TAG_X3, DUAL_KW = DUAL_H2 | TAG_KDIV;
+
+template <int BM, int BN, int WM, int WN, int MODE>
+static void launch_dual(const ConvArgs& a_in, hipStream_t st, int bk, size_t ws_floats, int stages, bool no_tail_split) {
+    ConvArgs a = a_in;
+    constexpr int TAGV = MODE == 0 ? 0 : (MODE == 1 ? DUAL_H2 : DUAL_KW);
+    const int tiles = igemm_plan<BM, BN>(a, TAGV, bk, ws_floats, 0, no_tail_split);
+#define RADET_DUAL(BKV, NSV) \
+    hipLaunchKernelGGL((conv_igemmg_dual_kernel<BM, BN, WM, WN, TAGV, BKV, NSV>), dim3(tiles, a.sk), dim3(256), 0, st, a)
+    if constexpr (MODE == 0) {
+        if (bk == 32) RADET_DUAL(32, 2); else RADET_DUAL(16, 2);
+    } else if constexpr (MODE == 1) {
+        if (stages >= 3) RADET_DUAL(32, 3); else RADET_DUAL(32, 2);
+    } else {
+        if (bk == 64) RADET_DUAL(64, 2);
+        else if (stages >= 4) RADET_DUAL(32, 4);
+        else if (stages == 3) RADET_DUAL(32, 3);
+        else RADET_DUAL(32, 2);
+    }
+#undef RADET_DUAL
+}
+
+extern "C" int radet_conv2d_igemm_dual_s(const float* x0, const float* w0, const float* bias0, const int* table0, int Cin0,
+                                         int rows0, const float* x1, const float* w1, const float* bias1, const int* table1,
+                                         int Cin1, int rows1, float* y, int M, int Cout, int relu, int tile_override,
+                                         float* splitk_ws, size_t splitk_ws_floats, void* stream, const RadetScales* sc) {
+    const TileWord tw = decode_tile(tile_override);
+    if (x0 == nullptr || w0 == nullptr || x1 == nullptr || w1 == nullptr || y == nullptr || M <= 0 || Cout <= 0 || Cin0 <= 0 ||
+        Cin1 <= 0 || Cin0 % 16 != 0 || Cin1 % 16 != 0 || rows0 <= 0 || rows1 <= 0)
+        return RADET_ERR_ARG;
+    if ((table0 == nullptr && rows0 < M) || (table1 == nullptr && rows1 < M)) return RADET_ERR_ARG;
+    if (tw.p3 || tw.store_bf16 || tw.math_bf16 || tw.out_f32 || tw.rowpairs || tw.maskq || tw.streamk || tw.x3 != tw.h2)
+        return RADET_ERR_ARG;
+    const bool h2 = tw.h2;
+    if (h2 && (Cin0 % 32 != 0 || Cin1 % 32 != 0 || sc == nullptr || sc->x_amax == nullptr || sc->w_amax == nullptr ||
+               sc->x1_amax == nullptr || sc->w1_amax == nullptr))
+        return RADET_ERR_ARG;
+    const unsigned long long lim = 0xFFFFFF00ull;
+    if (4ull * (unsigned long long)rows0 * Cin0 > lim || 4ull * (unsigned long long)rows1 * Cin1 > lim ||
+        4ull * (unsigned long long)Cout * Cin0 > lim || 4ull * (unsigned long long)Cout * Cin1 > lim)
+        return RADET_ERR_ARG;
+    int choice = tw.id, bk = h2 ? 32 : ((tw.bk32 && Cin0 % 32 == 0 && Cin1 % 32 == 0) ? 32 : 16);
+    if (choice == 7 || choice == 8) {
+        bk = choice == 7 ? 64 : 32;
+        if (!h2 || Cin0 % bk != 0 || Cin1 % bk != 0) return RADET_ERR_ARG;
+    } else if (choice > 4) {
+        return RADET_ERR_ARG;
+    }
+    if (choice <= 0) {
+        auto score = [&](int bm, int bn, double intrinsic) {
+            const long tm = (M + bm - 1) / bm, tn = (Cout + bn - 1) / bn, blocks = tm * tn;
+            return (double)blocks / (256.0 * ((blocks + 255) / 256)) * ((double)M * Cout) / ((double)tm * bm * tn * bn) * intrinsic;
+        };
+        choice = 1;
+        double best = score(128, 128, 1.00);
+        if (Cout <= 32) choice = 4;
+        else {
+            if (score(128, 64, 0.96) > best) { best = score(128, 64, 0.96); choice = 2; }
+            if (score(64, 64, 0.90) > best) choice = 3;
+        }
+    }
+    ConvArgs a;
+    a.p[0].x = x0; a.p[0].w = w0; a.p[0].bias = bias0; a.p[0].addend = nullptr; a.p[0].mask = nullptr; a.p[0].y = y;
+    a.p[0].xs = sc ? (const unsigned*)sc->x_amax : nullptr;
+    a.p[0].ws = sc ? (const unsigned*)sc->w_amax : nullptr;
+    a.p[0].ys = sc ? (unsigned*)sc->y_amax : nullptr;
+    a.p[0].yq = nullptr; a.p[0].yqs = nullptr; a.p[0].xt = a.p[0].wl1 = a.p[0].bs = a.p[0].as = nullptr;
+    a.p[1] = a.p[0];
+    a.p[1].x = x1; a.p[1].w = w1; a.p[1].bias = bias1; a.p[1].y = nullptr; a.p[1].ys = nullptr;
+    a.p[1].xs = sc ? (const unsigned*)sc->x1_amax : nullptr;
+    a.p[1].ws = sc ? (const unsigned*)sc->w1_amax : nullptr;
+    a.groups = 1;
+    a.rowtab = table0; a.rowtab1 = table1;
+    a.out_rows = nullptr;
+    for (int t = 0; t < 16; ++t) a.tap_ids[t] = t;
+    a.KTw = 1;
+    a.M = M; a.Mp = radet_gather_table_rows(M);
+    a.Cin = Cin0 + Cin1; a.Cin0 = Cin0; a.Cout = Cout; a.KH = a.KW = 1;
+    a.relu = relu;
+    a.io = 0;
+    a.sk_wgs = a.sk_base = a.sk_rem = 0;
+    a.cls_nt = 0; a.cls_b[0] = a.cls_b[1] = a.cls_b[2] = 0x7fffffff;
+    a.dbg = 0; a.maskq = 0;
+    static const bool no_splitk = getenv("RADET_NO_SPLITK") != nullptr, no_tail_split = getenv("RADET_NO_TAIL_SPLIT") != nullptr;
+    const int nK = a.Cin / bk;
+    const int bm = (choice == 3 || choice >= 7) ? 64 : 128, bn = choice == 1 ? 128 : (choice == 4 ? 32 : 64);
+    const long tiles = (long)((M + bm - 1) / bm) * ((Cout + bn - 1) / bn);
+    int sk = 1;
+    if (splitk_ws != nullptr && !no_splitk) {
+        if (tw.splitk) sk = tw.splitk;
+        else if (tiles < 384) {
+            sk = (int)((512 + tiles - 1) / tiles);
+            if (sk > nK / 8) sk = nK / 8;
+            if (sk > 8) sk = 8;
+        }
+        if (sk < 1) sk = 1;
+    }
+    a.sk = sk;
+    a.it_per_split = (nK + sk - 1) / sk;
+    a.counters = (int*)splitk_ws;
+    a.partial = nullptr;
+    if (splitk_ws != nullptr && splitk_ws_floats > RADET_SPLIT_COUNTERS) {
+        a.partial = splitk_ws + RADET_SPLIT_COUNTERS;
+        splitk_ws_floats -= RADET_SPLIT_COUNTERS;
+    } else {
+        a.sk = 1;
+        a.it_per_split = nK;
+        splitk_ws_floats = 0;
+    }
+    hipStream_t st = (hipStream_t)stream;
+#define RADET_DUAL_TILE(MODE) \
+    switch (choice) { \
+        case 1: launch_dual<128, 128, 2, 2, MODE>(a, st, bk, splitk_ws_floats, tw.stages, no_tail_split); break; \
+        case 2: launch_dual<128, 64, 2, 2, MODE>(a, st, bk, splitk_ws_floats, tw.stages, no_tail_split); break; \
+        case 3: launch_dual<64, 64, 2, 2, MODE>(a, st, bk, splitk_ws_floats, tw.stages, no_tail_split); break; \
+        default: launch_dual<128, 32, 4, 1, MODE>(a, st, bk, splitk_ws_floats, tw.stages, no_tail_split); break; \
+    }
+    if (choice >= 7) launch_dual<64, 64, 2, 2, 2>(a, st, bk, splitk_ws_floats, tw.stages, no_tail_split);
+    else if (h2) { RADET_DUAL_TILE(1) }
+    else { RADET_DUAL_TILE(0) }
+#undef RADET_DUAL_TILE
+    return radet_check_launch();
+}
diff --git a/radet_amd/csrc/conv_igemm.hip b/radet_amd/csrc/conv_igemm.hip
--- a/radet_amd/csrc/conv_igemm.hip
+++ b/radet_amd/csrc/conv_igemm.hip
@@ -964,6 +964,7 @@
         a.p[1].ys = sc ? (unsigned*)sc->y1_amax : nullptr;
         a.groups = 2;
     }
+    a.Cin0 = Cin; a.rowtab1 = nullptr;
     a.rowtab = gather_table;
     a.Cin = Cin; a.Cout = Cout; a.KH = KH; a.KW = KW;
     a.relu = relu;
diff --git a/radet_amd/csrc/conv_igemm_kernel.h b/radet_amd/csrc/conv_igemm_kernel.h
--- a/radet_amd/csrc/conv_igemm_kernel.h
+++ b/radet_amd/csrc/conv_igemm_kernel.h
@@ -10,8 +10,8 @@
 constexpr int TAG_KDIV = 32;
 constexpr int TAG_H2 = 64;
 constexpr int TAG_PAIRS = 128;
-template <int BM, int BN, int WM, int WN, int TAG, int BK, int NSTG = 2, bool SK = false>
-__global__ __launch_bounds__(WM * WN * 64) void conv_igemmg_kernel(const ConvArgs a) {
+template <int BM, int BN, int WM, int WN, int TAG, int BK, int NSTG, bool SK, bool DUAL>
+__device__ __forceinline__ void conv_igemmg_body(const ConvArgs& a) {
     constexpr int NW = WM * WN;
     constexpr int F4 = BK / 4;
     constexpr int RPI = 64 / F4;
@@ -38,6 +38,8 @@
     constexpr int TMA = KW ? BM / 32 : TM, TNA = KW ? BN / (32 * WNK) : TN;
     static_assert(!KW || (X3 && !SK && NW == 4 && KD * WNK == NW && TM == 1 && TN == 1 && TMA * TNA == KD && NSTG >= 2 && NSTG <= 4),
                   "K-divided tile: one 32 x 32 block per wave after the reduction");
+    static_assert(!DUAL || (!P3 && !SK && !H16 && !BF16 && (H2 || !X3) && RADET_BUFLDS != 0),
+                  "two-source GEMM: fp32 tensors, native fp32 or fp16 hi / lo arithmetic, buffer-form tile loads");
     static_assert(NW == 4 || NW == 8, "4 or 8 waves");
     static_assert(!P3 || BK == 16 || RI, "plane rows are laid out in 32-channel groups: one group per K stage");
     __shared__ __attribute__((aligned(16))) float As[NSTG][NPL * BM * BK];
@@ -54,6 +56,7 @@
     const int tilesG = ((a.M + BM - 1) / BM) * tilesN;
     const int KT = a.KH * a.KW;
     const int cpt = a.Cin / BK;
+    const int cin0 = DUAL ? a.Cin0 : a.Cin, cpt0 = cin0 / BK;
     constexpr bool streamk = SK;
     const int vwg = streamk ? ((int)blockIdx.x & 7) * (a.sk_wgs >> 3) + ((int)blockIdx.x >> 3) : 0;
     int cur = streamk ? streamk_start(a, vwg) : 0;
@@ -75,8 +78,11 @@
     epi.partial = pin_sgpr(a.partial); epi.counters = pin_sgpr(a.counters);
     epi.sk_base = pin_sgpr(a.sk_base); epi.sk_rem = pin_sgpr(a.sk_rem);
     epi.qs = 1.f; epi.qs2 = 2048.f;
+    if constexpr (DUAL) epi.bias1 = pin_sgpr(a.p[1].bias);
     unsigned raw_xs = 0u, raw_ws = 0u;
     if constexpr ((TAG & TAG_H2) != 0) { raw_xs = h2_scale_load(P.xs); raw_ws = h2_scale_load(P.ws); }
+    unsigned raw_xs1 = 0u, raw_ws1 = 0u;
+    if constexpr (DUAL && (TAG & TAG_H2) != 0) { raw_xs1 = h2_scale_load(a.p[1].xs); raw_ws1 = h2_scale_load(a.p[1].ws); }
     PairScaleRaw raw_q = {0u, 0u, 0u, 0u};
     const bool pair_copy = P.yq != nullptr;
     if (pair_copy) raw_q = igemm_pair_scale_load(P);
@@ -107,6 +113,7 @@
     int ld_tap = cmaj ? it0 % KTt : it0 / cpt, ld_c0 = cmaj ? (it0 / KTt) * BK : (it0 - ld_tap * cpt) * BK;
     int arow[A_PW], akq[A_PW];
     const float* wp[B_PW];
+    unsigned wrow[DUAL ? B_PW : 1];
 #pragma unroll
     for (int k = 0; k < A_PW; ++k) {
         const int r = (wave + NW * k) * RPI + lrow;
@@ -131,12 +138,25 @@
 #pragma unroll
         for (int k = 0; k < A_PW; ++k) arow[k] = (nK > 0 && (A_INSTR % NW == 0 || wave + NW * k < A_INSTR)) ? araw[k] : -1;
     }
+    int arow1[DUAL ? A_PW : 1];
+    if constexpr (DUAL) {
+        int araw[A_PW];
+#pragma unroll
+        for (int k = 0; k < A_PW; ++k) {
+            const int m = m0 + (wave + NW * k) * RPI + lrow;
+            if (a.rowtab1) araw[k] = a.rowtab1[m < a.Mp ? m : a.Mp - 1];
+            else araw[k] = m < a.M ? m : -1;
+        }
+#pragma unroll
+        for (int k = 0; k < A_PW; ++k) arow1[k] = (nK > 0 && (A_INSTR % NW == 0 || wave + NW * k < A_INSTR)) ? araw[k] : -1;
+    }
 #pragma unroll
     for (int k = 0; k < B_PW; ++k) {
         const int r = (wave + NW * k) * RPI + lrow;
         const int n = n0 + r;
         wp[k] = (wave + NW * k < B_INSTR && n < a.Cout)
-                    ? P.w + (size_t)n * a.KTw * xld + 4 * ((lane % F4) ^ ((r / RPB) % F4)) : nullptr;
+                    ? P.w + (DUAL ? (size_t)0 : (size_t)n * a.KTw * xld) + 4 * ((lane % F4) ^ ((r / RPB) % F4)) : nullptr;
+        if constexpr (DUAL) wrow[k] = (unsigned)n;
     }
     constexpr bool A_FULL = A_INSTR % NW == 0, B_FULL = B_INSTR % NW == 0;
     int wtap = nK > 0 ? a.tap_ids[tbase + ld_tap] : 0;
@@ -148,6 +168,7 @@
     constexpr bool BL = RADET_BUFLDS != 0;
     __amdgpu_buffer_rsrc_t rs_x, rs_w;
     unsigned aoffb[A_PW], woffb[B_PW];
+    unsigned wq[DUAL ? B_PW : 1];
     if constexpr (BL) {
         rs_x = radet_rsrc(P.x);
         rs_w = radet_rsrc(P.w);
@@ -155,6 +176,21 @@
     int pc0 = 0, pwt = 0;
     auto set_abase = [&]() {
         pc0 = ld_c0; pwt = wtap;
+        if constexpr (DUAL) {
+            const bool s1 = ld_c0 >= cin0;
+            const unsigned ld = (unsigned)(s1 ? a.Cin - cin0 : cin0);
+            pc0 = s1 ? ld_c0 - cin0 : ld_c0; pwt = 0;
+            rs_x = radet_rsrc(s1 ? a.p[1].x : P.x);
+            rs_w = radet_rsrc(s1 ? a.p[1].w : P.w);
+#pragma unroll
+            for (int k = 0; k < A_PW; ++k) {
+                const int r = s1 ? arow1[k] : arow[k];
+                amask[k] = r >= 0 ? 0xFFFFFFFFu : 0u;
+                aoffb[k] = ((unsigned)(r & (int)amask[k]) * ld + (unsigned)akq[k]) * 4u;
+            }
+#pragma unroll
+            for (int k = 0; k < B_PW; ++k) woffb[k] = wq[k] + wrow[k] * ld * 4u;
+        } else
         if constexpr (BL) {
 #pragma unroll
             for (int k = 0; k < A_PW; ++k) {
@@ -179,6 +215,7 @@
             wmask[k] = wp[k] ? 0xFFFFFFFFu : 0u;
             wbase[k] = wp[k] ? wp[k] : radet_zero_page + lane * 4;
             if constexpr (BL) woffb[k] = wp[k] ? (unsigned)((const char*)wp[k] - (const char*)P.w) : 0u;
+            if constexpr (DUAL) wq[k] = woffb[k];
         }
     }
     set_abase();
@@ -262,6 +299,8 @@
                 for (int r = 0; r < 16; ++r) acc1[i][j][r] = 0.f;
     }
     H2Scale sx = {1.f, 1.f, 1.f}, sw = {1.f, 1.f, 1.f};
+    H2Scale sx1 = {1.f, 1.f, 1.f}, sw1 = {1.f, 1.f, 1.f};
+    float cinv_a = 1.f, cinv_b = 1.f;
 
     constexpr int LOADS = (A_FULL && B_FULL) ? NPL * (A_PW + B_PW) : 0;
     if (nK > 0) issue_stage(0);
@@ -274,7 +313,12 @@
         asm volatile("s_waitcnt vmcnt(0)" ::: "memory");
     }
     __syncthreads();
-    if constexpr (H2) { sx = h2_scale_finish(raw_xs); sw = h2_scale_finish(raw_ws); }
+    if constexpr (H2 && DUAL) {
+        const H2Dual du = h2_dual_scales(raw_xs, raw_ws, raw_xs1, raw_ws1);
+        sx = du.x[0]; sw = du.w[0]; sx1 = du.x[1]; sw1 = du.w[1];
+        cinv_a = du.inv_a; cinv_b = du.inv_b;
+    } else
+    if constexpr (H2) { sx = h2_scale_finish(raw_xs); sw = h2_scale_finish(raw_ws); cinv_a = sx.inv; cinv_b = sw.inv; }
     if (pair_copy) {
         float qs, qs2;
         igemm_pair_scale(P, raw_q, pair_store, qs, qs2);
@@ -301,6 +345,9 @@
         constexpr int BUF = decltype(bufc)::value;
         constexpr int AO = BUF * BM * BK * 4, BO = BUF * BN * BK * 4, RO = 32 * BK * 4;
         if (it + NSTG - 1 < nK) issue_stage((BUF + NSTG - 1) % NSTG);
+        const bool src1 = DUAL && it0 + it >= cpt0;
+        H2Scale sxc = sx, swc = sw;
+        if (src1) { sxc = sx1; swc = sw1; }
         f32x4 af[X3 ? NS : 2][TM], bf[X3 ? NS : 2][TN];
         auto read_s = [&](int s, int pp) {
             lds_read128<AO>(af[pp][0], aaddr[s]);
@@ -321,9 +368,9 @@
                 if constexpr (H2) {
                     f16x8 ah[TM], al[TM], bh[TN], bl[TN];
 #pragma unroll
-                    for (int i = 0; i < TM; ++i) split2_f16(af[2 * g][i], af[2 * g + 1][i], sx, ah[i], al[i]);
-#pragma unroll
-                    for (int j = 0; j < TN; ++j) split2_f16(bf[2 * g][j], bf[2 * g + 1][j], sw, bh[j], bl[j]);
+                    for (int i = 0; i < TM; ++i) split2_f16(af[2 * g][i], af[2 * g + 1][i], sxc, ah[i], al[i]);
+#pragma unroll
+                    for (int j = 0; j < TN; ++j) split2_f16(bf[2 * g][j], bf[2 * g + 1][j], swc, bh[j], bl[j]);
 #pragma unroll
                     for (int i = 0; i < TM; ++i)
 #pragma unroll
@@ -436,10 +483,12 @@
 #pragma unroll
                     for (int j = 0; j < TNA; ++j) { bh[j] = __builtin_bit_cast(f16x8, fb[PP][0][j]); bl[j] = __builtin_bit_cast(f16x8, fb[PP][1][j]); }
                 } else {
-#pragma unroll
-                for (int i = 0; i < TMA; ++i) split2_f16(fa[PP][0][i], fa[PP][1][i], sx, ah[i], al[i]);
-#pragma unroll
-                for (int j = 0; j < TNA; ++j) split2_f16(fb[PP][0][j], fb[PP][1][j], sw, bh[j], bl[j]);
+                H2Scale sxc = sx, swc = sw;
+                if (DUAL && it0 + it >= cpt0) { sxc = sx1; swc = sw1; }
+#pragma unroll
+                for (int i = 0; i < TMA; ++i) split2_f16(fa[PP][0][i], fa[PP][1][i], sxc, ah[i], al[i]);
+#pragma unroll
+                for (int j = 0; j < TNA; ++j) split2_f16(fb[PP][0][j], fb[PP][1][j], swc, bh[j], bl[j]);
                 }
 #pragma unroll
                 for (int i = 0; i < TMA; ++i)
@@ -591,7 +640,7 @@
 #pragma unroll
         for (int i = 0; i < TMA; ++i)
 #pragma unroll
-            for (int j = 0; j < TNA; ++j) h2_combine(acc[i][j], acc1[i][j], sx.inv, sw.inv);
+            for (int j = 0; j < TNA; ++j) h2_combine(acc[i][j], acc1[i][j], cinv_a, cinv_b);
     }
     if constexpr (SK) {
         cur += nK;
@@ -636,15 +685,24 @@
             }
         }
         __syncthreads();
-        igemm_store<BM, BN, WM, WN>(epi, P, out, m0, n0, nsplit, ctile, zsplit, kg / TNA, nh * TNA + kg % TNA, li, lh,
-                                    reinterpret_cast<volatile int*>(&As[0][0]));
+        igemm_store<BM, BN, WM, WN, DUAL>(epi, P, out, m0, n0, nsplit, ctile, zsplit, kg / TNA, nh * TNA + kg % TNA, li, lh,
+                                          reinterpret_cast<volatile int*>(&As[0][0]));
         cur = end_it;
     } else {
-        igemm_store<BM, BN, WM, WN>(epi, P, acc, m0, n0, nsplit, ctile, zsplit, wm, wn, li, lh,
-                                    reinterpret_cast<volatile int*>(&As[0][0]));
+        igemm_store<BM, BN, WM, WN, DUAL>(epi, P, acc, m0, n0, nsplit, ctile, zsplit, wm, wn, li, lh,
+                                          reinterpret_cast<volatile int*>(&As[0][0]));
         cur = end_it;
     }
   } while (SK && cur < end_it);
+}
+
+template <int BM, int BN, int WM, int WN, int TAG, int BK, int NSTG = 2, bool SK = false>
+__global__ __launch_bounds__(WM * WN * 64) void conv_igemmg_kernel(const ConvArgs a) {
+    conv_igemmg_body<BM, BN, WM, WN, TAG, BK, NSTG, SK, false>(a);
+}
+template <int BM, int BN, int WM, int WN, int TAG, int BK, int NSTG = 2>
+__global__ __launch_bounds__(WM * WN * 64) void conv_igemmg_dual_kernel(const ConvArgs a) {
+    conv_igemmg_body<BM, BN, WM, WN, TAG, BK, NSTG, false, true>(a);
 }
 
 
diff --git a/radet_amd/csrc/tape_thunks.c b/radet_amd/csrc/tape_thunks.c
--- a/radet_amd/csrc/tape_thunks.c
+++ b/radet_amd/csrc/tape_thunks.c
@@ -28,6 +28,7 @@
 static int t_radet_conv2d_igemm(const uint64_t* a) { return radet_conv2d_igemm((void*)(uintptr_t)a[0], (void*)(uintptr_t)a[1], (void*)(uintptr_t)a[2], (void*)(uintptr_t)a[3], (void*)(uintptr_t)a[4], (void*)(uintptr_t)a[5], (void*)(uintptr_t)a[6], (int)(int64_t)a[7], (int)(int64_t)a[8], (int)(int64_t)a[9], (int)(int64_t)a[10], (int)(int64_t)a[11], (int)(int64_t)a[12], (int)(int64_t)a[13], (void*)(uintptr_t)a[14], (size_t)a[15], (void*)(uintptr_t)a[16]); }
 static int t_radet_conv2d_igemm_classes(const uint64_t* a) { return radet_conv2d_igemm_classes((void*)(uintptr_t)a[0], (void*)(uintptr_t)a[1], (void*)(uintptr_t)a[2], (void*)(uintptr_t)a[3], (void*)(uintptr_t)a[4], (void*)(uintptr_t)a[5], (void*)(uintptr_t)a[6], (void*)(uintptr_t)a[7], (void*)(uintptr_t)a[8], (void*)(uintptr_t)a[9], (int)(int64_t)a[10], (int)(int64_t)a[11], (int)(int64_t)a[12], (int)(int64_t)a[13], (int)(int64_t)a[14], (int)(int64_t)a[15], (void*)(uintptr_t)a[16], (size_t)a[17], (void*)(uintptr_t)a[18]); }
 static int t_radet_conv2d_igemm_classes_s(const uint64_t* a) { return radet_conv2d_igemm_classes_s((void*)(uintptr_t)a[0], (void*)(uintptr_t)a[1], (void*)(uintptr_t)a[2], (void*)(uintptr_t)a[3], (void*)(uintptr_t)a[4], (void*)(uintptr_t)a[5], (void*)(uintptr_t)a[6], (void*)(uintptr_t)a[7], (void*)(uintptr_t)a[8], (void*)(uintptr_t)a[9], (int)(int64_t)a[10], (int)(int64_t)a[11], (int)(int64_t)a[12], (int)(int64_t)a[13], (int)(int64_t)a[14], (int)(int64_t)a[15], (void*)(uintptr_t)a[16], (size_t)a[17], (void*)(uintptr_t)a[18], (void*)(uintptr_t)a[19]); }
+static int t_radet_conv2d_igemm_dual_s(const uint64_t* a) { return radet_conv2d_igemm_dual_s((void*)(uintptr_t)a[0], (void*)(uintptr_t)a[1], (void*)(uintptr_t)a[2], (void*)(uintptr_t)a[3], (int)(int64_t)a[4], (int)(int64_t)a[5], (void*)(uintptr_t)a[6], (void*)(uintptr_t)a[7], (void*)(uintptr_t)a[8], (void*)(uintptr_t)a[9], (int)(int64_t)a[10], (int)(int64_t)a[11], (void*)(uintptr_t)a[12], (int)(int64_t)a[13], (int)(int64_t)a[14], (int)(int64_t)a[15], (int)(int64_t)a[16], (void*)(uintptr_t)a[17], (size_t)a[18], (void*)(uintptr_t)a[19], (void*)(uintptr_t)a[20]); }
 static int t_radet_conv2d_igemm_pair(const uint64_t* a) { return radet_conv2d_igemm_pair((void*)(uintptr_t)a[0], (void*)(uintptr_t)a[1], (void*)(uintptr_t)a[2], (void*)(uintptr_t)a[3], (void*)(uintptr_t)a[4], (void*)(uintptr_t)a[5], (void*)(uintptr_t)a[6], (void*)(uintptr_t)a[7], (void*)(uintptr_t)a[8], (void*)(uintptr_t)a[9], (void*)(uintptr_t)a[10], (void*)(uintptr_t)a[11], (void*)(uintptr_t)a[12], (int)(int64_t)a[13], (int)(int64_t)a[14], (int)(int64_t)a[15], (int)(int64_t)a[16], (int)(int64_t)a[17], (int)(int64_t)a[18], (int)(int64_t)a[19], (void*)(uintptr_t)a[20], (size_t)a[21], (void*)(uintptr_t)a[22]); }
 static int t_radet_conv2d_igemm_pair_s(const uint64_t* a) { return radet_conv2d_igemm_pair_s((void*)(uintptr_t)a[0], (void*)(uintptr_t)a[1], (void*)(uintptr_t)a[2], (void*)(uintptr_t)a[3], (void*)(uintptr_t)a[4], (void*)(uintptr_t)a[5], (void*)(uintptr_t)a[6], (void*)(uintptr_t)a[7], (void*)(uintptr_t)a[8], (void*)(uintptr_t)a[9], (void*)(uintptr_t)a[10], (void*)(uintptr_t)a[11], (void*)(uintptr_t)a[12], (int)(int64_t)a[13], (int)(int64_t)a[14], (int)(int64_t)a[15], (int)(int64_t)a[16], (int)(int64_t)a[17], (int)(int64_t)a[18], (int)(int64_t)a[19], (void*)(uintptr_t)a[20], (size_t)a[21], (void*)(uintptr_t)a[22], (void*)(uintptr_t)a[23]); }
 static int t_radet_conv2d_igemm_s(const uint64_t* a) { return radet_conv2d_igemm_s((void*)(uintptr_t)a[0], (void*)(uintptr_t)a[1], (void*)(uintptr_t)a[2], (void*)(uintptr_t)a[3], (void*)(uintptr_t)a[4], (void*)(uintptr_t)a[5], (void*)(uintptr_t)a[6], (int)(int64_t)a[7], (int)(int64_t)a[8], (int)(int64_t)a[9], (int)(int64_t)a[10], (int)(int64_t)a[11], (int)(int64_t)a[12], (int)(int64_t)a[13], (void*)(uintptr_t)a[14], (size_t)a[15], (void*)(uintptr_t)a[16], (void*)(uintptr_t)a[17]); }
@@ -145,6 +146,7 @@
     {"radet_conv2d_igemm", t_radet_conv2d_igemm, 17},
     {"radet_conv2d_igemm_classes", t_radet_conv2d_igemm_classes, 19},
     {"radet_conv2d_igemm_classes_s", t_radet_conv2d_igemm_classes_s, 20},
+    {"radet_conv2d_igemm_dual_s", t_radet_conv2d_igemm_dual_s, 21},
     {"radet_conv2d_igemm_pair", t_radet_conv2d_igemm_pair, 23},
     {"radet_conv2d_igemm_pair_s", t_radet_conv2d_igemm_pair_s, 24},
     {"radet_conv2d_igemm_s", t_radet_conv2d_igemm_s, 18},
@@ -237,4 +239,4 @@
     {"radet_upsample_add_h", t_radet_upsample_add_h, 9},
     {"radet_warp_affine_u8", t_radet_warp_affine_u8, 9},
 };
-const int radet_tape_nthunks = 114;
+const int radet_tape_nthunks = 115;
diff --git a/radet_amd/engine.py b/radet_amd/engine.py
--- a/radet_amd/engine.py
+++ b/radet_amd/engine.py
@@ -52,6 +52,8 @@
         self.po = self.h2 and not self.pairs and os.environ.get("RADET_PAIRS_ONLY", "0") == "1"
         self.po_max_planes = int(os.environ.get("RADET_PAIRS_ONLY_MAX", "512"))
         self.pairs_from = int(os.environ.get("RADET_PAIRS_FROM", "2"))
+        self.fused_shortcut = (os.environ.get("RADET_FUSED_SHORTCUT", "1") != "0" and not self.pairs and not self.h16
+                               and not self.math and (self.h2 or not self.x3))
         if self.x3 and "RADET_TOWER_MODE" not in os.environ:
             self.tower_mode = "pairbwd"
         self.p3 = self.x3 and self.tower_mode == "pairbwd" and feat % 32 == 0 and os.environ.get("RADET_P3", "1") != "0"
@@ -135,6 +137,8 @@
                 if b == 0:
                     blk["ds"] = self._add(Conv(pfx + ".downsample.0", inpl, planes * 4, 1, stride, 0, bn=pfx + ".downsample.1",
                                                trainable=train, dgrad=in_dgrad))
+                blk["fs"] = (blk["ds"] is not None and self.fused_shortcut and not blk["po"]
+                             and planes % 32 == 0 and inpl % 32 == 0)
                 inpl = planes * 4
                 blocks.append(blk)
             self.stages.append(blocks)
@@ -326,7 +330,8 @@
                 blk["c3"].geom = ConvGeom(lo, blk["c3"].cin, blk["c3"].cout, 1, 1, 0)
                 if blk["ds"] is not None:
                     blk["ds"].geom = ConvGeom(lv, blk["ds"].cin, blk["ds"].cout, 1, blk["stride"], 0)
-                    new(pfx + ".idt", lo.rows, blk["ds"].cout, prefix=fz)
+                    if not blk["fs"]:
+                        new(pfx + ".idt", lo.rows, blk["ds"].cout, prefix=fz)
                 blk["lout"] = lo
                 tw = li + 1 >= self.pairs_from
                 new(pfx + ".o1", lv.rows, blk["c1"].cout, prefix=fz, twin=tw, only=blk["po"])
@@ -442,6 +447,10 @@
                 if c is not self.stem and c.geom is not None and (self.math or c not in towers):
                     K.autotune(c.geom, need_dgrad=c.need_dgrad)
             K.save_tune_cache()
+        for st in self.stages:
+            for blk in st:
+                if blk["fs"]:
+                    blk["c3"].geom.dual_tile = K.autotune_dual(blk["c3"].geom, blk["ds"].geom)
 
     wgrad_group = os.environ.get("RADET_WGRAD_GROUP", "0") == "1"
     wgrad_group_tile = int(os.environ.get("RADET_WGRAD_GROUP_TILE", "128"))
@@ -622,6 +631,9 @@
         else:
             K.conv_fwd(blk["c1"].geom, x, blk["c1"].wf, blk["c1"].bias_f, o1, relu=True)
             K.conv_fwd(blk["c2"].geom, o1, blk["c2"].wf, blk["c2"].bias_f, o2, relu=True)
+        if blk["fs"]:
+            K.conv_fwd_dual(c3.geom, ds.geom, o2, c3.wf, c3.bias_f, x, ds.wf, ds.bias_f, out, relu=True)
+            return out
         if blk["ds"] is not None:
             idt = b[pfx + ".idt"]
             K.conv_fwd(blk["ds"].geom, x, blk["ds"].wf, blk["ds"].bias_f, idt)
diff --git a/radet_amd/kernels.py b/radet_amd/kernels.py
--- a/radet_amd/kernels.py
+++ b/radet_amd/kernels.py
@@ -778,6 +778,110 @@
                   g.lout.rows, g.cin, g.cout, g.k, g.k, int(relu), tile, _ptr(ws), C.c_size_t(ws.numel() if splitk else 0),
                   _stream(), sc)
     _timed(lambda: _igemm_key(tile, x), 2.0 * g.lout.rows * g.cout * g.cin * g.k * g.k, launch, _conv_bytes(g), geom=g)
+
+
+def _dual_key(t):
+    tid = tile_id(t)
+    if tid == 0:
+        return "conv_igemmg_dual_kernel<launcher heuristic>"
+    if t & H2:
+        if tid >= 7:
+            nst = 2 if tid == 7 else (4 if t & STAGES4 else (3 if t & STAGES3 else 2))
+            return f"conv_igemmg_dual_kernel<{_TILES[tid]}, {TAG_X3 | TAG_H2 | TAG_KDIV}, {64 if tid == 7 else 32}, {nst}>"
+        return f"conv_igemmg_dual_kernel<{_TILES.get(tid, '?')}, {TAG_X3 | TAG_H2}, 32, {3 if t & (STAGES3 | STAGES4) else 2}>"
+    return f"conv_igemmg_dual_kernel<{_TILES.get(tid, '?')}, 0, {32 if t & BK32 else 16}, 2>"
+
+
+def dual_supported(g3, gd):
+    if g3.math or g3.h16 or g3.k != 1 or gd.k != 1 or g3.stride != 1 or g3.lout.rows != gd.lout.rows or g3.cout != gd.cout:
+        return False
+    if getattr(g3, "x3", False):
+        return bool(g3.h2) and g3.cin % 32 == 0 and gd.cin % 32 == 0
+    return g3.cin % 16 == 0 and gd.cin % 16 == 0
+
+
+def _dual_tune_key(g3, gd):
+    return ("dual", g3._key, gd._key, g3.cin, gd.cin, g3.cout, g3.math, g3.h16) + (("x3",) if getattr(g3, "x3", False) else ()) + _h2key(g3)
+
+
+def _dual_cands(g3, gd):
+    m, n, kdim = g3.lout.rows, g3.cout, g3.cin + gd.cin
+    h2 = bool(_h2key(g3))
+    tiles = [4] if n <= 32 else [1, 2, 3]
+    if h2:
+        c = list(tiles) + [t | STAGES3 for t in tiles]
+        if n > 32:
+            c += ([7] if g3.cin % 64 == 0 and gd.cin % 64 == 0 else []) + [8] + ([8 | STAGES3, 8 | STAGES4] if KW_DEEP else [])
+    else:
+        c = list(tiles) + ([t | BK32 for t in tiles] if g3.cin % 32 == 0 and gd.cin % 32 == 0 else [])
+    out = list(c)
+    for t in c:
+        out += _splitk_cands(t, m, n, kdim // (64 if tile_id(t) == 7 else (32 if (h2 or t & BK32) else 16)))
+    return out
+
+
+def autotune_dual(g3, gd, measure=False):
+    global _TUNE_DIRTY, TUNE_RUNS
+    load_tune_cache()
+    key = _dual_tune_key(g3, gd)
+    if key not in _TUNE_CACHE and measure:
+        dev = torch.device("cuda", torch.cuda.current_device())
+        x0 = torch.randn(g3.lin.rows, g3.cin, device=dev)
+        x1 = torch.randn(gd.lin.rows, gd.cin, device=dev)
+        w0 = torch.randn(g3.cout * g3.cin, device=dev) * 0.05
+        w1 = torch.randn(gd.cout * gd.cin, device=dev) * 0.05
+        y = torch.empty(g3.lout.rows, g3.cout, device=dev)
+        tmp_keys = _tune_slots(g3, x0, w0, x1, w1, outputs=(y,))
+        cands = _dual_cands(g3, gd)
+        for t in cands:
+            conv_fwd_dual(g3, gd, x0, w0, None, x1, w1, None, y, relu=True, tile=t)
+        torch.cuda.synchronize()
+        best = [float("inf")] * len(cands)
+        for _ in range(TUNE_REPS):
+            for i, t in enumerate(cands):
+                s, e = torch.cuda.Event(enable_timing=True), torch.cuda.Event(enable_timing=True)
+                s.record()
+                for _b in range(TUNE_BURST):
+                    conv_fwd_dual(g3, gd, x0, w0, None, x1, w1, None, y, relu=True, tile=t)
+                e.record()
+                e.synchronize()
+                best[i] = min(best[i], s.elapsed_time(e) / TUNE_BURST)
+        i = min(range(len(cands)), key=lambda j: (best[j], j))
+        _TUNE_CACHE[key] = (cands[i], 0)
+        _TUNE_DIRTY = True
+        TUNE_RUNS += 1
+        unregister_amax(tmp_keys)
+        if os.environ.get("RADET_TUNE_LOG"):
+            print(f"[tune dual] M={g3.lout.rows} {g3.cin}+{gd.cin}->{g3.cout} s{gd.stride}: tile={cands[i]:#x} {best[i] * 1e3:.1f} us")
+    if key in _TUNE_CACHE:
+        return _TUNE_CACHE[key][0]
+    t = g3.fwd_tile & ~(STREAMK_MASK | SYMBOL)
+    tid = tile_id(t)
+    h2 = bool(_h2key(g3))
+    if tid > 4 and (not h2 or tid not in (7, 8) or (tid == 7 and (g3.cin % 64 or gd.cin % 64))):
+        t = with_tile(t, 3)
+    if h2:
+        t &= ~BK32
+    elif g3.cin % 32 or gd.cin % 32:
+        t &= ~BK32
+    return t
+
+
+def conv_fwd_dual(g3, gd, x0, w0, bias0, x1, w1, bias1, y, relu=True, tile=0, splitk=True):
+    assert dual_supported(g3, gd)
+    t = (tile or getattr(g3, "dual_tile", 0) or autotune_dual(g3, gd)) & ~(MATH_BF16 | STORE_BF16 | P3 | X3 | H2)
+    if getattr(g3, "x3", False):
+        t = (t & ~BK32) | X3 | H2
+    ws = splitk_ws() if splitk else None
+    t0, t1 = g3.fwd_table, gd.fwd_table
+    sc = _scales(x0, w0, y, x1=x1, w1=w1, need=bool(t & H2))
+
+    def launch():
+        _lib.call("radet_conv2d_igemm_dual_s", _ptr(x0), _ptr(w0), _ptr(bias0), _ptr(t0), g3.cin, g3.lin.rows,
+                  _ptr(x1), _ptr(w1), _ptr(bias1), _ptr(t1), gd.cin, gd.lin.rows, _ptr(y), g3.lout.rows, g3.cout, int(relu), t,
+                  _ptr(ws), C.c_size_t(ws.numel() if splitk else 0), _stream(), sc)
+    nbytes = 4.0 * (g3.lin.rows * g3.cin + gd.lout.rows * gd.cin + g3.cout * (g3.cin + gd.cin) + g3.lout.rows * g3.cout)
+    _timed(lambda: _dual_key(t), 2.0 * g3.lout.rows * g3.cout * (g3.cin + gd.cin), launch, nbytes, geom=g3)
 
 
 def _pred_tiles(lv):
```
